# totokunda/apex-studio

Measured on AMD Instinct MI355X. Metric: denoise_steps_per_sec, higher is better.
Workload: dtype bf16; 1 GPU; flux-dev-1024x1024 denoise step (19 double + 38 single MM-DiT blocks, S_img 4096 + S_txt 512, B=1, no CFG) + FlowMatch-Euler step; clips_in_flight=1, parallelism=clip-per-gpu x1

## Files before the change

### apex-studio_amd/build.py

```python
from __future__ import annotations

import hashlib
import os
import shutil
import subprocess
import sys

PKG_DIR = os.path.dirname(os.path.abspath(__file__))
CSRC = os.path.join(PKG_DIR, "csrc")
LIB_NAME = "libapex_mi355.so"
LIB_PATH = os.path.join(PKG_DIR, LIB_NAME)
SOURCES = ["runtime.hip", "gemm.hip", "attention.hip", "attention_masked.hip", "attention_varlen.hip", "attention_dual.hip", "attention_wide.hip", "elementwise.hip", "dequant_gguf.hip",
           "conv.hip", "gemm_fp8.hip", "gemm_mxfp4.hip", "gemm_mxfp6.hip"]
ARCH = "gfx950"


def _hipcc() -> str:
    for cand in (os.environ.get("HIPCC"), shutil.which("hipcc"), "/opt/rocm/bin/hipcc"):
        if cand and os.path.exists(cand):
            return cand
    raise RuntimeError("hipcc not found (set HIPCC or install ROCm)")


FLAGS = ["-O3", "-std=c++17", "-fPIC", "-Wno-unused-result"]
if os.environ.get("APEXMI_DEBUG", "0") not in ("", "0"):
    FLAGS.append("-DAPEXMI_DEBUG")


NO_SPILL = {"attention.hip": ["attn_fwd_d128_w64_kernel", "attn_fwd_d128_w64r_kernel", "attn_fwd_d128_w64_band_kernel"],
            "attention_masked.hip": ["attn_masked_kernel", "attn_window_map_kernel"],
            "attention_varlen.hip": ["attn_varlen_kernel", "attn_varlen_vt_kernel"], "attention_dual.hip": ["attn_dual_kernel"], "attention_wide.hip": ["attn_wide_kernel"],
            "gemm_fp8.hip": ["gemm_fp8_kernel"], "gemm_mxfp4.hip": ["gemm_mxfp4_kernel"], "gemm_mxfp6.hip": ["gemm_mxfp6_kernel"],
            "elementwise.hip": ["ln_modulate_quant_kernel", "ln_modulate_wave_quant_kernel"]}
REMARKS = "-Rpass-analysis=kernel-resource-usage"


def parse_resource_remarks(text: str) -> dict:
    import re
    out, cur = {}, None
    for line in text.splitlines():
        m = re.search(r"remark:\s+Function Name: (\S+)", line)
        if m:
            cur = out.setdefault(m.group(1), {})
            continue
        m = re.search(r"remark:\s+([A-Za-z ]+?)(?: \[[^\]]*\])?: (\d+)", line)
        if m and cur is not None:
            cur[m.group(1).strip()] = int(m.group(2))
    return out


def check_no_spill(src: str, remarks: str, complete: bool = False) -> None:
    res = parse_resource_remarks(remarks)
    wanted = NO_SPILL.get(src, [])
    found = [want for want in wanted if any(want in k for k in res)]
    for want in wanted:
        hits = {k: v for k, v in res.items() if want in k}
        if not hits:
            if found and not complete:
                continue
            raise RuntimeError(f"build: no resource remark for kernel '{want}' of {src} — the spill check cannot run")
        for k, v in hits.items():
            bad = {f: v.get(f, -1) for f in ("ScratchSize", "SGPRs Spill", "VGPRs Spill") if v.get(f, -1) != 0}
            if bad:
                raise RuntimeError(f"build: {k} ({src}) has a hand-fixed register map and must not spill, but the compiler "
                                   f"reports {bad} (VGPRs {v.get('VGPRs')}, AGPRs {v.get('AGPRs')}, SGPRs {v.get('TotalSGPRs')}): "
                                   f"this hipcc allocates differently from the one the map was written against")


def _digest(paths: list[str], extra: str = "") -> str:
    h = hashlib.sha256(extra.encode())
    for p in paths:
        with open(p, "rb") as f:
            h.update(hashlib.sha256(f.read()).digest())
    return h.hexdigest()


def _stale(target: str, digest: str) -> bool:
    stamp = target + ".sha256"
    if not (os.path.exists(target) and os.path.exists(stamp)):
        return True
    with open(stamp) as f:
        return f.read().strip() != digest


def _stamp(target: str, digest: str) -> None:
    with open(target + ".sha256", "w") as f:
        f.write(digest + "\n")


def build(force: bool = False, verbose: bool = True) -> str:
    hipcc = _hipcc()
    headers = [os.path.join(CSRC, "common.h"),
               os.path.join(PKG_DIR, "..", "include", "apexmi.h")]
    headers += sorted(os.path.join(CSRC, f) for f in os.listdir(CSRC) if f.endswith((".inc", ".h")) and f != "common.h")
    objs = []
    jobs = []
    for src in SOURCES:
        sp = os.path.join(CSRC, src)
        op = os.path.join(CSRC, src.replace(".hip", ".o"))
        objs.append(op)
        dg = _digest([sp] + headers, " ".join(FLAGS + ([REMARKS + ":checked"] if src in NO_SPILL else []) + [ARCH]))
        if force or _stale(op, dg):
            cmd = [hipcc, f"--offload-arch={ARCH}", *FLAGS, *([REMARKS] if src in NO_SPILL else []), "-c", sp, "-o", op]
            if verbose:
                print("[build]", " ".join(cmd), flush=True)
            jobs.append((subprocess.Popen(cmd, stderr=subprocess.PIPE if src in NO_SPILL else None, text=True), cmd, op, dg, src))
    for proc, cmd, op, dg, src in jobs:
        err = proc.communicate()[1]
        if err:
            rest = [l for l in err.splitlines() if "kernel-resource-usage" not in l and not l.lstrip().startswith(("|", "^"))
                    and not l.strip()[:1].isdigit() and not l.startswith("In file included from")]
            if rest and verbose:
                print("\n".join(rest), file=sys.stderr, flush=True)
        if proc.returncode != 0:
            if err:
                print(err[-4000:], file=sys.stderr)
            raise subprocess.CalledProcessError(proc.returncode, cmd)
        if src in NO_SPILL:
            check_no_spill(src, err or "", complete=True)
        _stamp(op, dg)
    dg = _digest(objs, ARCH)
    if force or _stale(LIB_PATH, dg):
        cmd = [hipcc, f"--offload-arch={ARCH}", "-shared", "-fPIC", "-o", LIB_PATH] + objs
        if verbose:
            print("[build]", " ".join(cmd), flush=True)
        subprocess.check_call(cmd)
        _stamp(LIB_PATH, dg)
    return LIB_PATH


if __name__ == "__main__":
    build(force="--force" in sys.argv)
    print(LIB_PATH)
```

### apex-studio_amd/csrc/gemm.hip

```cpp
#include "common.h"

#include <cstring>
#include <type_traits>

namespace {

#ifndef APEXMI_GEMM_TRACE
#define APEXMI_GEMM_TRACE 0
#endif
#define PP_BAR()                               \
    do {                                       \
        __builtin_amdgcn_sched_barrier(0);     \
        __builtin_amdgcn_s_barrier();          \
        __builtin_amdgcn_sched_barrier(0);     \
    } while (0)
#define PP_SYNC()                                                                   \
    do {                                                                            \
        asm volatile("s_waitcnt lgkmcnt(0)" ::: "memory");                          \
        PP_BAR();                                                                   \
    } while (0)
#define VMCNT(n) asm volatile("s_waitcnt vmcnt(" #n ")" ::: "memory")
constexpr int BK = 64;
constexpr int GROUP_M = 6;
constexpr int EPI_GATE_RES_F32 = 7;
constexpr int MAX_GROUPS = 4;

struct GemmProblem {
    const bf16_t* A;
    const bf16_t* W;
    const bf16_t* bias;
    bf16_t* C;
    const float* gate;
    const bf16_t* R;
    int64_t lda, ldw, ldc, ldr;
    int M, N, nm, nn, tile0, gelu;
    int qkv, row0;
    const bf16_t* nq;
    const bf16_t* nk;
};
struct QkvShared {
    bf16_t* qo;
    bf16_t* ko;
    bf16_t* vt;
    const float* rope;
    int S_out, Skp, inner;
    float eps;
    const float* rope_pairs;
};
struct GemmGroup {
    GemmProblem p[MAX_GROUPS];
    int count, K, total, group_m;
    int batch;
    int64_t bsA, bsW, bsC_bytes;
    QkvShared qs;
    unsigned long long* clk;
#if APEXMI_GEMM_TRACE
    unsigned long long* trace;
#endif
    int wpacked;
};

template <int BM_, int BN_, int WM_, int WN_, int SCHED_>
struct Cfg {
    static constexpr int BM = BM_, BN = BN_, WM = WM_, WN = WN_;
    static constexpr int SCHED = SCHED_;
    static constexpr bool PP = SCHED_ == 1;
    static constexpr int NW = WM * WN, NT = NW * 64;
    static constexpr int TM = BM / WM / 32, TN = BN / WN / 32;
    static constexpr int A_BYTES = BM * BK * 2, W_BYTES = BN * BK * 2;
    static constexpr int STAGE = A_BYTES + W_BYTES;
    static constexpr int LDS = SCHED_ == 8 ? 5 * 32768 : 2 * STAGE;
    static constexpr int A_LD = BM * 8 / NT, W_LD = BN * 8 / NT;
    static constexpr int OCC = (LDS <= 80 * 1024 && NT == 256) ? 2 : (NT == 512 ? 2 : 1);
};
using CFG_128 = Cfg<128, 128, 2, 2, 0>;
using CFG_256 = Cfg<256, 256, 2, 4, 0>;
using CFG_128E = Cfg<128, 128, 2, 4, 0>;
using CFG_256P = Cfg<256, 256, 2, 4, 1>;
using CFG_256W = Cfg<256, 256, 2, 2, 4>;
using CFG_256P16 = Cfg<256, 256, 2, 4, 5>;
using CFG_256R = Cfg<256, 256, 2, 4, 7>;
using CFG_256R5 = Cfg<256, 256, 2, 4, 8>;

APEXMI_DEVICE float act_f(float x, int mode) {
    if (mode == 1) return gelu_tanh_f(x);
    if (mode == 2) return 0.5f * x * (1.0f + erff(x * 0.70710678118654752f));
    if (mode == 4) return x_sigmoid_log2(x, (1.702f * 1.4426950408889634f) * x);
    return silu_f(x);
}
template <int ACT>
APEXMI_DEVICE float act_c(float x) {
    if constexpr (ACT == 0) return x;
    else return act_f(x, ACT);
}
#define APEXMI_ACT_DISPATCH(mode, ...)                                    \
    switch (mode) {                                                       \
        case 1: { constexpr int ACT = 1; __VA_ARGS__; } break;            \
        case 2: { constexpr int ACT = 2; __VA_ARGS__; } break;            \
        case 3: { constexpr int ACT = 3; __VA_ARGS__; } break;            \
        case 4: { constexpr int ACT = 4; __VA_ARGS__; } break;            \
        default: { constexpr int ACT = 0; __VA_ARGS__; } break;           \
    }
inline int act_mode(int epilogue) {
    return epilogue == APEXMI_EPI_BIAS_GELU ? 1 : epilogue == APEXMI_EPI_BIAS_GELU_ERF ? 2 : epilogue == APEXMI_EPI_BIAS_SILU ? 3 : epilogue == APEXMI_EPI_BIAS_QUICK_GELU ? 4 : 0;
}

APEXMI_DEVICE void swap_pair(u32x2& a, u32x2& b) {
#pragma unroll
    for (int i = 0; i < 2; ++i) {
        auto r = __builtin_amdgcn_permlane32_swap(a[i], b[i], false, false);
        a[i] = r[0];
        b[i] = r[1];
    }
}

template <int EPI, int TM, int ACT = 0>
APEXMI_DEVICE void store_ntile(const f32x16 (&acc)[TM], const GemmProblem& P, int N, const int (&m)[TM],
                               int nbase, int hi) {
    float bs[4][4];
    f32x4 gt[4];
#pragma unroll
    for (int g = 0; g < 4; ++g) {
        const int n = min(nbase + 8 * g + 4 * hi, N - 4);
        u32x2 b = {0u, 0u};
        if (P.bias != nullptr) b = *(const u32x2*)(P.bias + n);
        bs[g][0] = bf16_lo(b[0]);
        bs[g][1] = bf16_hi(b[0]);
        bs[g][2] = bf16_lo(b[1]);
        bs[g][3] = bf16_hi(b[1]);
        if (EPI == APEXMI_EPI_BIAS_GATE_RES || EPI == EPI_GATE_RES_F32) gt[g] = *(const f32x4*)(P.gate + n);
    }
    if (EPI == APEXMI_EPI_BIAS_F32 || EPI == EPI_GATE_RES_F32) {
        float* Cf = (float*)P.C;
        const float* Rf = (const float*)P.R;
#pragma unroll
        for (int mt = 0; mt < TM; ++mt)
#pragma unroll
            for (int g = 0; g < 4; ++g) {
                const int n = nbase + 8 * g + 4 * hi;
                if (m[mt] >= 0 && n < N) {
                    float o[4];
#pragma unroll
                    for (int j = 0; j < 4; ++j) {
                        o[j] = acc[mt][4 * g + j] + bs[g][j];
                        o[j] = act_c<ACT>(o[j]);
                    }
                    if (EPI == EPI_GATE_RES_F32) {
                        const f32x4 r = *(const f32x4*)(Rf + (int64_t)m[mt] * P.ldr + n);
#pragma unroll
                        for (int j = 0; j < 4; ++j) o[j] = r[j] + gt[g][j] * o[j];
                    }
                    *(f32x4*)(Cf + (int64_t)m[mt] * P.ldc + n) = f32x4{o[0], o[1], o[2], o[3]};
                }
            }
        return;
    }
    u32x4 rr[TM][2];
    if (EPI == APEXMI_EPI_BIAS_GATE_RES) {
#pragma unroll
        for (int mt = 0; mt < TM; ++mt)
#pragma unroll
            for (int pr = 0; pr < 2; ++pr) {
                const int nst = min(nbase + 8 * (2 * pr + hi), N - 8);
                rr[mt][pr] = *(const u32x4*)(P.R + (int64_t)max(m[mt], 0) * P.ldr + nst);
            }
    }
#pragma unroll
    for (int mt = 0; mt < TM; ++mt)
#pragma unroll
        for (int pr = 0; pr < 2; ++pr) {
            const int g0 = 2 * pr;
            const int nst = nbase + 8 * (g0 + hi);
            float v[2][4];
#pragma unroll
            for (int q = 0; q < 2; ++q)
#pragma unroll
                for (int j = 0; j < 4; ++j) {
                    v[q][j] = acc[mt][4 * (g0 + q) + j] + bs[g0 + q][j];
                    v[q][j] = act_c<ACT>(v[q][j]);
                }
            if (EPI == APEXMI_EPI_BIAS_GATE_RES) {
                u32x2 ra = {rr[mt][pr][0], rr[mt][pr][1]}, rb = {rr[mt][pr][2], rr[mt][pr][3]};
                swap_pair(ra, rb);
#pragma unroll
                for (int q = 0; q < 2; ++q) {
                    const u32x2 r2 = q ? rb : ra;
                    v[q][0] = bf16_lo(r2[0]) + gt[g0 + q][0] * v[q][0];
                    v[q][1] = bf16_hi(r2[0]) + gt[g0 + q][1] * v[q][1];
                    v[q][2] = bf16_lo(r2[1]) + gt[g0 + q][2] * v[q][2];
                    v[q][3] = bf16_hi(r2[1]) + gt[g0 + q][3] * v[q][3];
                }
            }
            u32x2 oa = {pack_bf16(v[0][0], v[0][1]), pack_bf16(v[0][2], v[0][3])};
            u32x2 ob = {pack_bf16(v[1][0], v[1][1]), pack_bf16(v[1][2], v[1][3])};
            swap_pair(oa, ob);
            if (m[mt] >= 0 && nst < N) {
                const u32x4 o = {oa[0], oa[1], ob[0], ob[1]};
                *(u32x4*)(P.C + (int64_t)m[mt] * P.ldc + nst) = o;
            }
        }
}


typedef __attribute__((ext_vector_type(4))) float f32x4_t;

APEXMI_DEVICE float sum_xor16(float x) {
    auto r = __builtin_amdgcn_permlane16_swap(__float_as_uint(x), __float_as_uint(x), false, false);
    return __uint_as_float(r[0]) + __uint_as_float(r[1]);
}
APEXMI_DEVICE void swap16(uint32_t& a, uint32_t& b) {
    auto r = __builtin_amdgcn_permlane16_swap(a, b, false, false);
    a = r[0];
    b = r[1];
}

template <int EPI, int MT, int ACT = 0>
APEXMI_DEVICE void store_slab16(const f32x4_t (&x)[MT], const f32x4_t (&y)[MT], const GemmProblem& P, int N,
                                const int (&m)[MT], int nbase, int g, const u32x4* rr_pre = nullptr) {
    float bs[2][4];
    f32x4 gt[2];
#pragma unroll
    for (int t = 0; t < 2; ++t) {
        const int n = min(nbase + 16 * t + 4 * g, N - 4);
        u32x2 b = {0u, 0u};
        if (P.bias != nullptr) b = *(const u32x2*)(P.bias + n);
        bs[t][0] = bf16_lo(b[0]);
        bs[t][1] = bf16_hi(b[0]);
        bs[t][2] = bf16_lo(b[1]);
        bs[t][3] = bf16_hi(b[1]);
        if (EPI == APEXMI_EPI_BIAS_GATE_RES || EPI == EPI_GATE_RES_F32) gt[t] = *(const f32x4*)(P.gate + n);
    }
    if (EPI == APEXMI_EPI_BIAS_F32 || EPI == EPI_GATE_RES_F32) {
        float* Cf = (float*)P.C;
        const float* Rf = (const float*)P.R;
        constexpr int CH = MT < 4 ? MT : 4;
#pragma unroll
        for (int m0 = 0; m0 < MT; m0 += CH) {
            f32x4 rr[CH][2];
            if (EPI == EPI_GATE_RES_F32) {
#pragma unroll
                for (int c = 0; c < CH; ++c)
#pragma unroll
                    for (int t = 0; t < 2; ++t)
                        if (m0 + c < MT)
                            rr[c][t] = *(const f32x4*)(Rf + (int64_t)max(m[m0 + c < MT ? m0 + c : 0], 0) * P.ldr + min(nbase + 16 * t + 4 * g, N - 4));
            }
#pragma unroll
            for (int c = 0; c < CH; ++c)
#pragma unroll
                for (int t = 0; t < 2; ++t) {
                    if (m0 + c >= MT) continue;
                    const int mt = m0 + c < MT ? m0 + c : 0;
                    const int n = nbase + 16 * t + 4 * g;
                    const f32x4_t& a = t ? y[mt] : x[mt];
                    if (m[mt] >= 0 && n < N) {
                        float o[4];
#pragma unroll
                        for (int j = 0; j < 4; ++j) {
                            o[j] = a[j] + bs[t][j];
                            o[j] = act_c<ACT>(o[j]);
                        }
                        if (EPI == EPI_GATE_RES_F32) {
#pragma unroll
                            for (int j = 0; j < 4; ++j) o[j] = rr[c][t][j] + gt[t][j] * o[j];
                        }
                        *(f32x4*)(Cf + (int64_t)m[mt] * P.ldc + n) = f32x4{o[0], o[1], o[2], o[3]};
                    }
                }
        }
        return;
    }
    const int nst = nbase + 16 * (g & 1) + 8 * (g >> 1);
    u32x4 rr[MT];
    if (EPI == APEXMI_EPI_BIAS_GATE_RES) {
#pragma unroll
        for (int mt = 0; mt < MT; ++mt)
            rr[mt] = rr_pre ? rr_pre[mt] : *(const u32x4*)(P.R + (int64_t)max(m[mt], 0) * P.ldr + min(nst, N - 8));
    }
#pragma unroll
    for (int mt = 0; mt < MT; ++mt) {
        float v[2][4];
#pragma unroll
        for (int j = 0; j < 4; ++j) {
            v[0][j] = x[mt][j] + bs[0][j];
            v[1][j] = y[mt][j] + bs[1][j];
            v[0][j] = act_c<ACT>(v[0][j]);
            v[1][j] = act_c<ACT>(v[1][j]);
        }
        if (EPI == APEXMI_EPI_BIAS_GATE_RES) {
            uint32_t r0 = rr[mt][0], r1 = rr[mt][1], r2 = rr[mt][2], r3 = rr[mt][3];
            swap16(r0, r2);
            swap16(r1, r3);
            const uint32_t ra[2][2] = {{r0, r1}, {r2, r3}};
#pragma unroll
            for (int t = 0; t < 2; ++t) {
                v[t][0] = bf16_lo(ra[t][0]) + gt[t][0] * v[t][0];
                v[t][1] = bf16_hi(ra[t][0]) + gt[t][1] * v[t][1];
                v[t][2] = bf16_lo(ra[t][1]) + gt[t][2] * v[t][2];
                v[t][3] = bf16_hi(ra[t][1]) + gt[t][3] * v[t][3];
            }
        }
        uint32_t x0 = pack_bf16(v[0][0], v[0][1]), x1 = pack_bf16(v[0][2], v[0][3]);
        uint32_t y0 = pack_bf16(v[1][0], v[1][1]), y1 = pack_bf16(v[1][2], v[1][3]);
        swap16(x0, y0);
        swap16(x1, y1);
        if (m[mt] >= 0 && nst < N) {
            const u32x4 o = {x0, x1, y0, y1};
            *(u32x4*)(P.C + (int64_t)m[mt] * P.ldc + nst) = o;
        }
    }
}

#ifndef APEXMI_QK_ABL
#define APEXMI_QK_ABL 0
#endif
template <int MT = 8, int WROWS = 128>
APEXMI_DEVICE void qkv_epilogue16(f32x4_t (&acc16)[4][MT], const GemmProblem& P, const QkvShared& Q, int M, int m0, int n0,
                                  int wave, int wm, int wn, int lane, char* smem) {
    const int g = lane >> 4, c = lane & 15;
    const int which = n0 / Q.inner;
    const int ncol0 = n0 - which * Q.inner;
    float bs[2][4];
    auto load_bias = [&](int p) {
#pragma unroll
        for (int t = 0; t < 2; ++t) {
            u32x2 b = {0u, 0u};
            if (P.bias != nullptr) b = *(const u32x2*)(P.bias + n0 + wn * 64 + p * 32 + 16 * t + 4 * g);
            bs[t][0] = bf16_lo(b[0]);
            bs[t][1] = bf16_hi(b[0]);
            bs[t][2] = bf16_lo(b[1]);
            bs[t][3] = bf16_hi(b[1]);
        }
    };
    auto rounded = [&](int p, int mt) -> u32x4 {
        const f32x4_t& x = acc16[2 * p][mt];
        const f32x4_t& y = acc16[2 * p + 1][mt];
        uint32_t x0 = pack_bf16(x[0] + bs[0][0], x[1] + bs[0][1]), x1 = pack_bf16(x[2] + bs[0][2], x[3] + bs[0][3]);
        uint32_t y0 = pack_bf16(y[0] + bs[1][0], y[1] + bs[1][1]), y1 = pack_bf16(y[2] + bs[1][2], y[3] + bs[1][3]);
        swap16(x0, y0);
        swap16(x1, y1);
        return u32x4{x0, x1, y0, y1};
    };
    const int cw = 16 * (g & 1) + 8 * (g >> 1);
    __syncthreads();
    if (which == 2) {
        constexpr int NPASS = (2 * WROWS * 512 > 160 * 1024) ? 2 : 1;
        constexpr int ROWS = NPASS == 1 ? 2 * WROWS : WROWS;
        bf16_t* tile = (bf16_t*)smem;
        const int tid = wave * 64 + lane;
#pragma unroll
        for (int pass = 0; pass < NPASS; ++pass) {
            if (NPASS == 2 && pass == 1) __syncthreads();
            if (NPASS == 1 || wm == pass) {
#pragma unroll
                for (int p = 0; p < 2; ++p) {
                    load_bias(p);
#pragma unroll
                    for (int mt = 0; mt < MT; ++mt) {
                        const int r = (NPASS == 1 ? wm * WROWS : 0) + mt * 16 + c;
                        const int dch = (wn * 64 + p * 32 + cw) >> 3;
                        *(u32x4*)(tile + r * 256 + (((dch + (r >> 3) + 4 * (r & 7)) & 31) << 3)) = rounded(p, mt);
                    }
                }
            }
            __syncthreads();
            const int mp = m0 + (NPASS == 1 ? 0 : pass * WROWS);
            if (((P.row0 | M) & 7) != 0) {
                for (int i = 0; i < ROWS / 2; ++i) {
                    const int idx = i * 512 + tid;
                    const int r = idx % ROWS, d = idx / ROWS;
                    const bf16_t e = tile[r * 256 + ((((d >> 3) + (r >> 3) + 4 * (r & 7)) & 31) << 3) + (d & 7)];
                    const int h = (ncol0 + d) >> 7, dd = (ncol0 + d) & 127;
                    if (mp + r < M) Q.vt[((int64_t)h * 128 + dd) * Q.Skp + P.row0 + mp + r] = e;
                }
                continue;
            }
#pragma unroll 4
            for (int i = 0; i < ROWS / 16; ++i) {
                const int idx = i * 512 + tid;
                const int sc = idx & 7, d = (idx >> 3) & 255, sc_hi = idx >> 11;
                const int s8 = (sc_hi * 8 + sc) * 8;
                uint32_t w[4];
#pragma unroll
                for (int j = 0; j < 8; ++j) {
                    const int r = s8 + j;
                    const uint32_t e = tile[r * 256 + ((((d >> 3) + (r >> 3) + 4 * (r & 7)) & 31) << 3) + (d & 7)];
                    if (j & 1) w[j >> 1] |= e << 16;
                    else w[j >> 1] = e;
                }
                const int h = (ncol0 + d) >> 7, dd = (ncol0 + d) & 127;
                if (mp + s8 < M)
                    *(u32x4*)(Q.vt + ((int64_t)h * 128 + dd) * Q.Skp + P.row0 + mp + s8) = u32x4{w[0], w[1], w[2], w[3]};
            }
        }
        return;
    }
    float* red = (float*)smem;
#pragma unroll
    for (int p = 0; p < ((APEXMI_QK_ABL & 4) ? 0 : 2); ++p) {
        load_bias(p);
#pragma unroll
        for (int mt = 0; mt < MT; ++mt) {
            float x[8];
            unpack8(rounded(p, mt), x);
            float sq = 0.0f;
#pragma unroll
            for (int j = 0; j < 8; ++j) sq += x[j] * x[j];
            red[(wave * 2 * MT + p * MT + mt) * 64 + lane] = sq;
        }
    }
    __syncthreads();
    const bf16_t* nw = which ? P.nk : P.nq;
    const int h = (ncol0 >> 7) + (wn >> 1);
    bf16_t* dst_base = (which ? Q.ko : Q.qo) + (int64_t)h * Q.S_out * 128;
    auto rinv_of = [&](int mt) -> float {
        const float a0 = red[(wave * 2 * MT + mt) * 64 + lane] + red[((wave ^ 1) * 2 * MT + mt) * 64 + lane];
        const float a1 = red[(wave * 2 * MT + MT + mt) * 64 + lane] + red[((wave ^ 1) * 2 * MT + MT + mt) * 64 + lane];
        float sq = a0 + a1;
        sq = sum_xor16(sq);
        sq = sum_xor32(sq);
        return rsqrtf(sq * (1.0f / 128) + Q.eps);
    };
    float rinv[MT > 8 ? 1 : MT];
    if constexpr (MT <= 8) {
#pragma unroll
        for (int mt = 0; mt < MT; ++mt) rinv[mt] = rinv_of(mt);
    }
    if constexpr (!(APEXMI_QK_ABL & 64)) {
        if (Q.rope_pairs != nullptr) {
            constexpr int NIT = 2 * MT, NS = 5;
            constexpr int RED_BYTES = 8 * 2 * MT * 64 * 4;
            char* ring = smem + RED_BYTES + wave * (NS * 2048);
            const unsigned ring_lane = (unsigned)(uintptr_t)(__attribute__((address_space(3))) char*)ring + (unsigned)lane * 16u;
            auto issue = [&](int it) {
                const int p = it / MT, mt = it % MT;
                const int d = (wn & 1) * 64 + p * 32 + cw;
                int m = m0 + wm * WROWS + mt * 16 + c;
                asm volatile("" : "+v"(m));
                const int srow = P.row0 + min(m, M - 1);
                const float* cp = Q.rope_pairs + (int64_t)srow * 64 + (d >> 1);
                char* dst = ring + (it % NS) * 2048;
                glds16(cp, dst);
                glds16(cp + (int64_t)Q.S_out * 64, dst + 1024);
            };
#pragma unroll
            for (int it = 0; it < NS - 1; ++it) issue(it);
            float* wtab = (float*)(smem + RED_BYTES + 8 * NS * 2048) + wave * 1024 + lane * 8;
            float wv[MT > 8 ? 1 : 8];
            if constexpr (MT > 8) {
                if (nw != nullptr) {
#pragma unroll
                    for (int p = 0; p < 2; ++p) {
                        float w8[8];
                        unpack8(*(const u32x4*)(nw + (wn & 1) * 64 + p * 32 + cw), w8);
                        *(f32x4*)(wtab + p * 512) = f32x4{w8[0], w8[1], w8[2], w8[3]};
                        *(f32x4*)(wtab + p * 512 + 4) = f32x4{w8[4], w8[5], w8[6], w8[7]};
                    }
                }
            }
            auto body = [&](auto IT) {
                constexpr int it = decltype(IT)::value;
                if constexpr (it < NIT) {
                    constexpr int p = it / MT, mt = it % MT;
                    constexpr int later = (NIT - 1 - it) < (NS - 1) ? (NIT - 1 - it) : (NS - 1);
                    if constexpr (it + NS - 1 < NIT) issue(it + NS - 1);
                    const int d = (wn & 1) * 64 + p * 32 + cw;
                    if constexpr (mt == 0) {
                        load_bias(p);
                        if constexpr (MT <= 8) {
                            if (nw != nullptr) unpack8(*(const u32x4*)(nw + d), wv);
                        }
                    }
                    float x[8], y[8];
                    unpack8(rounded(p, mt), x);
                    if (nw != nullptr) {
                        if constexpr (MT > 8) {
                            const float ri = rinv_of(mt);
                            const f32x4 w0 = *(const f32x4*)(wtab + p * 512), w1 = *(const f32x4*)(wtab + p * 512 + 4);
#pragma unroll
                            for (int j = 0; j < 4; ++j) {
                                x[j] = x[j] * ri * w0[j];
                                x[j + 4] = x[j + 4] * ri * w1[j];
                            }
                        } else {
                            const float ri = rinv[MT > 8 ? 0 : mt];
#pragma unroll
                            for (int j = 0; j < 8; ++j) x[j] = x[j] * ri * wv[MT > 8 ? 0 : j];
                        }
                    }
                    f32x4 cq, sq4;
                    asm volatile("s_waitcnt vmcnt(%3)\n\t"
                                 "ds_read_b128 %0, %2 offset:%4\n\t"
                                 "ds_read_b128 %1, %2 offset:%5\n\t"
                                 "s_waitcnt lgkmcnt(0)"
                                 : "=&v"(cq), "=&v"(sq4)
                                 : "v"(ring_lane), "n"(2 * later), "n"((it % NS) * 2048), "n"((it % NS) * 2048 + 1024)
                                 : "memory");
#pragma unroll
                    for (int q = 0; q < 4; ++q) {
                        y[2 * q] = fmaf(x[2 * q], cq[q], -(x[2 * q + 1] * sq4[q]));
                        y[2 * q + 1] = fmaf(x[2 * q + 1], cq[q], x[2 * q] * sq4[q]);
                    }
                    int m = m0 + wm * WROWS + mt * 16 + c;
                    asm volatile("" : "+v"(m));
                    const int srow = P.row0 + min(m, M - 1);
                    if (m < M)
                        *(u32x4*)(dst_base + (int64_t)srow * 128 + d) =
                            u32x4{pack_bf16(y[0], y[1]), pack_bf16(y[2], y[3]), pack_bf16(y[4], y[5]), pack_bf16(y[6], y[7])};
                    __builtin_amdgcn_sched_barrier(0);
                }
            };
#define APEXMI_QK_IT(i) body(std::integral_constant<int, (i)>{});
            APEXMI_QK_IT(0) APEXMI_QK_IT(1) APEXMI_QK_IT(2) APEXMI_QK_IT(3) APEXMI_QK_IT(4) APEXMI_QK_IT(5)
            APEXMI_QK_IT(6) APEXMI_QK_IT(7) APEXMI_QK_IT(8) APEXMI_QK_IT(9) APEXMI_QK_IT(10) APEXMI_QK_IT(11)
            APEXMI_QK_IT(12) APEXMI_QK_IT(13) APEXMI_QK_IT(14) APEXMI_QK_IT(15) APEXMI_QK_IT(16) APEXMI_QK_IT(17)
            APEXMI_QK_IT(18) APEXMI_QK_IT(19) APEXMI_QK_IT(20) APEXMI_QK_IT(21) APEXMI_QK_IT(22) APEXMI_QK_IT(23)
#undef APEXMI_QK_IT
            static_assert(NIT <= 24, "the unrolled call list above covers 24 iterations");
            static_assert(MT > 8 ? RED_BYTES + 8 * NS * 2048 + 8 * 4096 <= 160 * 1024 : RED_BYTES + 8 * NS * 2048 <= 128 * 1024,
                          "sums + ring (+ weights) must fit the tile's LDS");
            return;
        }
    }
#pragma unroll
    for (int p = 0; p < ((APEXMI_QK_ABL & 32) ? 0 : 2); ++p) {
        const int d = (wn & 1) * 64 + p * 32 + cw;
        load_bias(p);
        float wv[8];
        if (nw != nullptr) unpack8(*(const u32x4*)(nw + d), wv);
#pragma unroll
        for (int mt = 0; mt < MT; ++mt) {
            const int m = m0 + wm * WROWS + mt * 16 + c;
            const int srow = P.row0 + min(m, M - 1);
            float x[8], y[8];
            unpack8(rounded(p, mt), x);
            if (nw != nullptr) {
                const float ri = (APEXMI_QK_ABL & 8) ? 1.0f : MT > 8 ? rinv_of(mt) : rinv[MT > 8 ? 0 : mt];
#pragma unroll
                for (int j = 0; j < 8; ++j) x[j] = x[j] * ri * wv[j];
            }
            const float* cp = Q.rope + (int64_t)srow * 128 + d;
            const float* sp = Q.rope + (int64_t)Q.S_out * 128 + (int64_t)srow * 128 + d;
            float cs[8], sn[8];
            if constexpr (APEXMI_QK_ABL & 1) {
#pragma unroll
                for (int j = 0; j < 8; ++j) cs[j] = 1.f, sn[j] = 0.5f;
            } else {
                const f32x4 c0 = *(const f32x4*)cp, c1 = *(const f32x4*)(cp + 4);
                const f32x4 s0 = *(const f32x4*)sp, s1 = *(const f32x4*)(sp + 4);
#pragma unroll
                for (int j = 0; j < 4; ++j) {
                    cs[j] = c0[j];
                    cs[j + 4] = c1[j];
                    sn[j] = s0[j];
                    sn[j + 4] = s1[j];
                }
            }
#pragma unroll
            for (int q = 0; q < 4; ++q) {
                y[2 * q] = fmaf(x[2 * q], cs[2 * q], -(x[2 * q + 1] * sn[2 * q]));
                y[2 * q + 1] = fmaf(x[2 * q + 1], cs[2 * q + 1], x[2 * q] * sn[2 * q + 1]);
            }
            if ((APEXMI_QK_ABL & 2) ? (y[0] + y[3] + y[5] == 12345.678f) : (m < M))
                *(u32x4*)(dst_base + (int64_t)srow * 128 + d) =
                    u32x4{pack_bf16(y[0], y[1]), pack_bf16(y[2], y[3]), pack_bf16(y[4], y[5]), pack_bf16(y[6], y[7])};
            if (!(APEXMI_QK_ABL & 16) && (MT > 8 || (mt & 1))) __builtin_amdgcn_sched_barrier(0);
        }
    }
}

#if APEXMI_GEMM_TRACE
#define APEXMI_TRACE_END()                                                                                   \
    do {                                                                                                     \
        if (G.trace != nullptr) {                                                                            \
            __builtin_amdgcn_sched_barrier(0);                                                               \
            const unsigned long long t_st = __builtin_amdgcn_s_memrealtime();                                \
            asm volatile("s_waitcnt vmcnt(0)" ::: "memory");                                                 \
            const unsigned long long t_ack = __builtin_amdgcn_s_memrealtime();                               \
            if (tid == 0) {                                                                                  \
                unsigned long long* o = G.trace + (size_t)blockIdx.x * 8;                                    \
                o[0] = __builtin_amdgcn_s_getreg((31 << 11) | (0 << 6) | 4);               \
                o[1] = __builtin_amdgcn_s_getreg((31 << 11) | (0 << 6) | 20);             \
                o[2] = tr_in;                                                                                \
                o[3] = tr_l0;                                                                                \
                o[4] = tr_l1;                                                                                \
                o[5] = t_st;                                                                                 \
                o[6] = t_ack;                                                                                \
                o[7] = (unsigned long long)s;                                                                \
            }                                                                                                \
        }                                                                                                    \
    } while (0)
#else
#define APEXMI_TRACE_END() do { } while (0)
#endif

struct TileCoord {
    int pm, pn;
};
__device__ __forceinline__ TileCoord tile_coord(int s, int nm, int nn, int group_m) {
    const int width = group_m * nn;
    const int first_m = (s / width) * group_m;
    const int gsz = min(nm - first_m, group_m);
    return TileCoord{first_m + (s % width) % gsz, (s % width) / gsz};
}

__device__ __forceinline__ const char* uniform_ptr(const char* p) {
    const uint64_t u = (uint64_t)p;
    const uint32_t hi = __builtin_amdgcn_readfirstlane((uint32_t)(u >> 32)), lo = __builtin_amdgcn_readfirstlane((uint32_t)u);
    return (const char*)(((uint64_t)hi << 32) | lo);
}
#pragma clang diagnostic push
#pragma clang diagnostic ignored "-Winline-asm"
__device__ __forceinline__ void glds16_s(const char* sbase, uint32_t voff, uint32_t la) {
    asm volatile("s_mov_b32 m0, %2\n\ts_nop 0\n\tglobal_load_lds_dwordx4 %0, %1"
                 :: "v"(voff), "s"(sbase), "s"(la) : "memory", "m0");
}
#pragma clang diagnostic pop

struct KRange {
    int kt0, kt1;
};
template <typename CFG, int EPI>
__device__ __forceinline__ void gemm_tile(const GemmGroup& G, char* smem, int s, const KRange& kr) {
    constexpr int BM = CFG::BM, BN = CFG::BN, TM = CFG::TM, TN = CFG::TN;

#if APEXMI_GEMM_TRACE
    unsigned long long tr_in = 0, tr_l0 = 0, tr_l1 = 0;
    if (G.trace != nullptr) tr_in = __builtin_amdgcn_s_memrealtime();
#endif
    int tid_ = threadIdx.x;
    asm volatile("" : "+v"(tid_));
    const int tid = tid_;
    const int lane = tid & 63;
    const int wave = __builtin_amdgcn_readfirstlane(tid >> 6);
    const int wm = wave / CFG::WN, wn = wave % CFG::WN;
    const int l31 = lane & 31, hi = lane >> 5;

    int gi = 0;
#pragma unroll
    for (int i = 1; i < MAX_GROUPS; ++i)
        if (i < G.count && s >= G.p[i].tile0) gi = i;
    GemmProblem P = G.p[gi];
    if (G.batch > 1) {
        const int64_t z = blockIdx.y;
        P.A += z * G.bsA;
        P.W += z * G.bsW;
        P.C = (bf16_t*)((char*)P.C + z * G.bsC_bytes);
    }
    s -= P.tile0;
    const int N = P.N, M = P.M;
    const TileCoord tc = tile_coord(s, P.nm, P.nn, G.group_m);
    const int pm = tc.pm, pn = tc.pn;
    const int m0 = pm * BM, n0 = pn * BN;

    const char* a_src[CFG::A_LD];
    const char* w_src[CFG::W_LD];
#pragma unroll
    for (int i = 0; i < CFG::A_LD; ++i) {
        const int p = (i * CFG::NW + wave) * 64 + lane;
        const int row = p >> 3, c = (p & 7) ^ ((row >> 1) & 7);
        a_src[i] = (const char*)(P.A + (int64_t)min(m0 + row, M - 1) * P.lda + c * 8);
    }
#pragma unroll
    for (int i = 0; i < CFG::W_LD; ++i) {
        const int p = (i * CFG::NW + wave) * 64 + lane;
        const int row = p >> 3, c = (p & 7) ^ ((row >> 1) & 7);
        w_src[i] = (const char*)(P.W + (int64_t)min(n0 + row, N - 1) * P.ldw + c * 8);
    }

    f32x16 acc[TN][TM];
#pragma unroll
    for (int i = 0; i < TN; ++i)
#pragma unroll
        for (int j = 0; j < TM; ++j)
#pragma unroll
            for (int r = 0; r < 16; ++r) acc[i][j][r] = 0.0f;

    f32x4_t acc16[4][8];
    if constexpr (CFG::SCHED == 5 || CFG::SCHED >= 7) {
#pragma unroll
        for (int i = 0; i < 4; ++i)
#pragma unroll
            for (int j = 0; j < 8; ++j) {
                acc16[i][j] = f32x4_t{0.f, 0.f, 0.f, 0.f};
                asm volatile("" : "+v"(acc16[i][j]));
            }
    }
    const int nkt_all = G.K / BK;
    const int nkt = (CFG::SCHED == 5) ? kr.kt1 - kr.kt0 : nkt_all;
    unsigned long long clk_c0 = 0, clk_r0 = 0;
    if (G.clk != nullptr) {
        clk_c0 = __builtin_readcyclecounter();
        clk_r0 = __builtin_amdgcn_s_memrealtime();
    }
#if APEXMI_GEMM_TRACE
    if (G.trace != nullptr) tr_l0 = __builtin_amdgcn_s_memrealtime();
#endif

    int a_off[TM], a_sw[TM], w_off[TN], w_sw[TN];
#pragma unroll
    for (int t = 0; t < TM; ++t) {
        const int r = wm * (BM / CFG::WM) + t * 32 + l31;
        a_off[t] = r * 128;
        a_sw[t] = (r >> 1) & 7;
    }
#pragma unroll
    for (int t = 0; t < TN; ++t) {
        const int r = wn * (BN / CFG::WN) + t * 32 + l31;
        w_off[t] = r * 128;
        w_sw[t] = (r >> 1) & 7;
    }

    if constexpr (CFG::SCHED == 0) {
        const char* const a_p = (const char*)(P.A + (int64_t)min(m0, M - 1) * P.lda);
        const char* const w_p = (const char*)(P.W + (int64_t)min(n0, N - 1) * P.ldw);
        const char* const a_u = uniform_ptr(a_p);
        const char* const w_u = uniform_ptr(w_p);
        uint32_t a_o[CFG::A_LD], w_o[CFG::W_LD];
#pragma unroll
        for (int i = 0; i < CFG::A_LD; ++i) a_o[i] = (uint32_t)(a_src[i] - a_u);
#pragma unroll
        for (int i = 0; i < CFG::W_LD; ++i) w_o[i] = (uint32_t)(w_src[i] - w_u);
        const uint32_t smem_lds0 = __builtin_amdgcn_readfirstlane((uint32_t)(uintptr_t)(__attribute__((address_space(3))) void*)smem);
        auto stage = [&](int buf, int kt) {
            const uint32_t base = smem_lds0 + buf * CFG::STAGE + wave * 1024;
            const char* ga = a_u + (int64_t)kt * (BK * 2);
            const char* gw = w_u + (int64_t)kt * (BK * 2);
#pragma unroll
            for (int i = 0; i < CFG::A_LD; ++i) glds16_s(ga, a_o[i], base + i * (CFG::NW * 1024));
#pragma unroll
            for (int i = 0; i < CFG::W_LD; ++i) glds16_s(gw, w_o[i], base + CFG::A_BYTES + i * (CFG::NW * 1024));
        };
        stage(0, 0);
        for (int kt = 0; kt < nkt; ++kt) {
            asm volatile("s_waitcnt vmcnt(0)" ::: "memory");
            __syncthreads();
            if (kt + 1 < nkt) stage((kt + 1) & 1, kt + 1);
            const char* As = smem + (kt & 1) * CFG::STAGE;
            const char* Ws = As + CFG::A_BYTES;
#pragma unroll
            for (int ks = 0; ks < 4; ++ks) {
                const int c = ks * 2 + hi;
                bf16x8 af[TM], wf[TN];
#pragma unroll
                for (int t = 0; t < TM; ++t) af[t] = *(const bf16x8*)(As + a_off[t] + ((c ^ a_sw[t]) << 4));
#pragma unroll
                for (int t = 0; t < TN; ++t) wf[t] = *(const bf16x8*)(Ws + w_off[t] + ((c ^ w_sw[t]) << 4));
#pragma unroll
                for (int nt = 0; nt < TN; ++nt)
#pragma unroll
                    for (int mt = 0; mt < TM; ++mt)
                        acc[nt][mt] = __builtin_amdgcn_mfma_f32_32x32x16_bf16(wf[nt], af[mt], acc[nt][mt], 0, 0, 0);
            }
        }
    } else if constexpr (CFG::SCHED == 4) {
        static_assert(CFG::SCHED != 4 || (TM == 4 && TN == 4 && CFG::NW == 4), "SCHED 4 is written for 2x2 waves of 128x128");
        bf16x8 fa[2][4], fw[2][4];
        const int rows_a = min(M - m0, BM), rows_w = min(N - n0, BN);
        auto rsrc_a = __builtin_amdgcn_make_buffer_rsrc((void*)(P.A + (int64_t)m0 * P.lda), 0,
                                                        (int)(((int64_t)(rows_a - 1) * P.lda + G.K) * 2), 0x00020000);
        auto rsrc_w = __builtin_amdgcn_make_buffer_rsrc((void*)(P.W + (int64_t)n0 * P.ldw), 0,
                                                        (int)(((int64_t)(rows_w - 1) * P.ldw + G.K) * 2), 0x00020000);
        const int sw_src = ((lane & 7) ^ (4 * (wave & 1) + (lane >> 4))) * 16;
        const int voff_a = (lane >> 3) * (int)P.lda * 2 + sw_src;
        const int voff_w = (lane >> 3) * (int)P.ldw * 2 + sw_src;
        const int sa = (int)P.lda * 2 * 8, sw = (int)P.ldw * 2 * 8;
        const int krot = (G.K * 2) % 8192 == 0 ? (int)(blockIdx.x & 7) * (nkt >> 3) : 0;
        auto dma1 = [&](int slot, int kt_, int i) {
            int kt = kt_ + krot;
            kt = kt >= nkt ? kt - nkt : kt;
            char* base = smem + slot * CFG::STAGE + wave * 1024;
            if (i < 8)
                __builtin_amdgcn_raw_ptr_buffer_load_lds(rsrc_a, (__attribute__((address_space(3))) void*)(base + i * 4096), 16, voff_a,
                                                         (i * 4 + wave) * sa + kt * (BK * 2), 0, 0);
            else
                __builtin_amdgcn_raw_ptr_buffer_load_lds(rsrc_w, (__attribute__((address_space(3))) void*)(base + CFG::A_BYTES + (i - 8) * 4096), 16,
                                                         voff_w, ((i - 8) * 4 + wave) * sw + kt * (BK * 2), 0, 0);
        };
        auto rd1 = [&](int slot, int ks, int b, int j) {
            const char* As = smem + slot * CFG::STAGE;
            const char* Ws = As + CFG::A_BYTES;
            const int c = ks * 2 + hi;
            if (j == 0) fw[b][0] = *(const bf16x8*)(Ws + w_off[0] + ((c ^ w_sw[0]) << 4));
            else if (j <= 4) fa[b][j - 1] = *(const bf16x8*)(As + a_off[j - 1] + ((c ^ a_sw[j - 1]) << 4));
            else fw[b][j - 4] = *(const bf16x8*)(Ws + w_off[j - 4] + ((c ^ w_sw[j - 4]) << 4));
        };
        auto mma1 = [&](int b, int i) {
            acc[i >> 2][i & 3] =
                __builtin_amdgcn_mfma_f32_32x32x16_bf16(fw[b][i >> 2], fa[b][i & 3], acc[i >> 2][i & 3], 0, 0, 0);
        };
#define W4_FENCE() __builtin_amdgcn_sched_barrier(0)
        constexpr int ROT = 0;
        constexpr int STEP = 2;
        auto period = [&](int kt, auto has_dma, auto has_next) {
            constexpr bool DMA = decltype(has_dma)::value, NEXT = decltype(has_next)::value;
            const int cur = kt & 1, nxt = cur ^ 1;
            asm volatile("s_waitcnt vmcnt(0) lgkmcnt(0)" ::: "memory");
            W4_FENCE();
            __builtin_amdgcn_s_barrier();
            W4_FENCE();
#pragma unroll
            for (int s = 0; s < (NEXT ? 64 : 16); ++s) {
                const int q = s >> 4, i = s & 15;
                mma1((q + 1) & 1, i);
                if (NEXT && i < 8) rd1(nxt, q, q & 1, i);
                if (DMA && s >= ROT && (s - ROT) % STEP == 0 && (s - ROT) / STEP < 16) dma1(cur, kt + 2, (s - ROT) / STEP);
                W4_FENCE();
            }
        };
#pragma unroll
        for (int i = 0; i < 16; ++i) dma1(0, 0, i);
        if (nkt > 1) {
#pragma unroll
            for (int i = 0; i < 16; ++i) dma1(1, 1, i);
            asm volatile("s_waitcnt vmcnt(16)" ::: "memory");
        } else {
            asm volatile("s_waitcnt vmcnt(0)" ::: "memory");
        }
        W4_FENCE();
        __builtin_amdgcn_s_barrier();
        W4_FENCE();
#pragma unroll
        for (int j = 0; j < 8; ++j) rd1(0, 0, 0, j);
        W4_FENCE();
#pragma unroll
        for (int s = 0; s < 48; ++s) {
            const int q = s >> 4, i = s & 15;
            mma1(q & 1, i);
            if (i < 8) rd1(0, q + 1, (q + 1) & 1, i);
            W4_FENCE();
        }
        int kt = 0;
        for (; kt + 2 < nkt; ++kt) period(kt, std::true_type{}, std::true_type{});
        if (kt + 1 < nkt) {
            period(kt, std::false_type{}, std::true_type{});
            ++kt;
        }
        period(kt, std::false_type{}, std::false_type{});
#undef W4_FENCE
    } else if constexpr (CFG::SCHED >= 7) {
        const int l15 = lane & 15, g4 = lane >> 4;
        const int swz = (g4 ^ (l15 >> 2)) << 4;
        const int rd_a = (wm * 128 + l15) * 64 + swz;
        const int rd_w = 16384 + (wn * 64 + l15) * 64 + swz;
        const char* base_a = (const char*)(P.A + (int64_t)m0 * P.lda);
        const char* base_w = (const char*)(P.W + (int64_t)n0 * P.ldw);
        unsigned off[4];
        int dst[4];
#pragma unroll
        for (int j = 0; j < 2; ++j) {
            const int pc = wave + 8 * j;
            const int row = pc * 16 + (lane >> 2);
            const int c = (lane & 3) ^ ((row >> 2) & 3);
            off[j] = (unsigned)((min(m0 + row, M - 1) - m0) * (int)P.lda * 2 + c * 16);
            off[2 + j] = (unsigned)((min(n0 + row, N - 1) - n0) * (int)P.ldw * 2 + c * 16);
            dst[j] = pc * 1024;
            dst[2 + j] = 16384 + pc * 1024;
        }
        constexpr int RD_ = CFG::SCHED == 8 ? 4 : 3;
        constexpr int NSLOT = RD_ + 1;
        auto dma = [&](int st, int slot) {
            char* base = smem + slot * 32768;
            const char* ka = base_a + (int64_t)st * 64;
            const char* kw = base_w + (int64_t)st * 64;
#pragma unroll
            for (int j = 0; j < 2; ++j) glds16(ka + off[j], base + dst[j]);
#pragma unroll
            for (int j = 2; j < 4; ++j) glds16(kw + off[j], base + dst[j]);
        };
        bf16x8 fa[2][8], fw[2][4];
#define RING_DSR(dstreg, addr, offs) asm volatile("ds_read_b128 %0, %1 offset:%2" : "=v"(dstreg) : "v"(addr), "i"(offs) : "memory")
#define RING_RD(slotidx, set)                              \
    do {                                                   \
        const int slot_ = (slotidx) * 32768;               \
        const int aw_ = slot_ + rd_w, aa_ = slot_ + rd_a;  \
        RING_DSR(fw[set][0], aw_, 0);                      \
        RING_DSR(fw[set][1], aw_, 1024);                   \
        RING_DSR(fw[set][2], aw_, 2048);                   \
        RING_DSR(fw[set][3], aw_, 3072);                   \
        RING_DSR(fa[set][0], aa_, 0);                      \
        RING_DSR(fa[set][1], aa_, 1024);                   \
        RING_DSR(fa[set][2], aa_, 2048);                   \
        RING_DSR(fa[set][3], aa_, 3072);                   \
        RING_DSR(fa[set][4], aa_, 4096);                   \
        RING_DSR(fa[set][5], aa_, 5120);                   \
        RING_DSR(fa[set][6], aa_, 6144);                   \
        RING_DSR(fa[set][7], aa_, 7168);                   \
    } while (0)
#define RING_WAIT(n, set)                                                                                                    \
    asm volatile("s_waitcnt lgkmcnt(" #n ")"                                                                                 \
                 : "+v"(fw[set][0]), "+v"(fw[set][1]), "+v"(fw[set][2]), "+v"(fw[set][3]), "+v"(fa[set][0]), "+v"(fa[set][1]), \
                   "+v"(fa[set][2]), "+v"(fa[set][3]), "+v"(fa[set][4]), "+v"(fa[set][5]), "+v"(fa[set][6]), "+v"(fa[set][7]) \
                 :                                                                                                           \
                 : "memory")
#define RING_MMA(set)                                                                                                      \
    do {                                                                                                                   \
        __builtin_amdgcn_s_setprio(1);                                                                                     \
        _Pragma("unroll") for (int u = 0; u < 4; ++u) _Pragma("unroll") for (int t = 0; t < 8; ++t) acc16[u][t] =          \
            __builtin_amdgcn_mfma_f32_16x16x32_bf16(fw[set][u], fa[set][t], acc16[u][t], 0, 0, 0);                         \
        __builtin_amdgcn_s_setprio(0);                                                                                     \
    } while (0)
#define RING_FENCE() __builtin_amdgcn_sched_barrier(0)
#define RING_VM(n) asm volatile("s_waitcnt vmcnt(" #n ")" ::: "memory")
#define RING_BAR() __builtin_amdgcn_s_barrier()
#define RING_STEP(st_, set, RD, DMA)                                        \
    do {                                                                    \
        RING_FENCE();                                                       \
        if (RD) RING_RD(s_rd, (set) ^ 1);                                   \
        RING_FENCE();                                                       \
        if (DMA) dma((st_) + RD_, s_dma);                                   \
        RING_FENCE();                                                       \
        if (DMA) {                                                          \
            if (RD_ == 3) RING_VM(4);                                       \
            else RING_VM(8);                                                \
        } else {                                                            \
            RING_VM(0);                                                     \
        }                                                                   \
        RING_FENCE();                                                       \
        RING_BAR();                                                         \
        RING_FENCE();                                                       \
        RING_MMA(set);                                                      \
        if (RD) RING_WAIT(0, (set) ^ 1);                                    \
        RING_FENCE();                                                       \
        RING_BAR();                                                         \
        RING_FENCE();                                                       \
        s_rd = s_rd + 1 == NSLOT ? 0 : s_rd + 1;                            \
        s_dma = s_dma + 1 == NSLOT ? 0 : s_dma + 1;                         \
    } while (0)
        const int ns = nkt * 2;
#pragma unroll
        for (int i = 0; i < RD_; ++i)
            if (i < ns) dma(i, i);
        if (ns >= 4 && RD_ == 4) RING_VM(8);
        else if (ns >= 3) RING_VM(4);
        else RING_VM(0);
        RING_FENCE();
        __builtin_amdgcn_s_barrier();
        RING_FENCE();
        RING_RD(0, 0);
        RING_WAIT(0, 0);
        RING_FENCE();
        if (wm == 1) RING_BAR();
        RING_FENCE();
        int s_rd = 1, s_dma = RD_ % NSLOT;
        int st = 0;
        for (; st + 1 + RD_ < ns; st += 2) {
            RING_STEP(st, 0, true, true);
            RING_STEP(st + 1, 1, true, true);
        }
        if (st + 4 <= ns) {
            if constexpr (RD_ == 3) RING_STEP(st, 0, true, true);
            else RING_STEP(st, 0, true, false);
            RING_STEP(st + 1, 1, true, false);
            st += 2;
        }
        RING_STEP(st, 0, true, false);
        RING_STEP(st + 1, 1, false, false);
        RING_FENCE();
        if (wm == 0) RING_BAR();
        RING_FENCE();
#undef RING_VM
#undef RING_BAR
#undef RING_STEP
#undef RING_MMA
#undef RING_RD
#undef RING_FENCE
#undef RING_DSR
#undef RING_WAIT
    } else if constexpr (CFG::SCHED == 5) {
        const int l15 = lane & 15, g4 = lane >> 4;
        const int sw16 = (l15 >> 1) & 7;
        int a16[8], w16[4];
#pragma unroll
        for (int t = 0; t < 8; ++t) a16[t] = (wm * 128 + t * 16 + l15) * 128;
#pragma unroll
        for (int t = 0; t < 4; ++t) w16[t] = (wn * 64 + t * 16 + l15) * 128;
        const int ch16[2] = {((0 + g4) ^ sw16) << 4, ((4 + g4) ^ sw16) << 4};
        bf16x8 af[4][2], wf[2][2][2];
        auto rd_a = [&](const char* As, int half) {
#pragma unroll
            for (int t = 0; t < 4; ++t)
#pragma unroll
                for (int ks = 0; ks < 2; ++ks) af[t][ks] = *(const bf16x8*)(As + a16[half * 4 + t] + ch16[ks]);
        };
        auto rd_w = [&](const char* Ws, int nt) {
#pragma unroll
            for (int u = 0; u < 2; ++u)
#pragma unroll
                for (int ks = 0; ks < 2; ++ks) wf[nt][u][ks] = *(const bf16x8*)(Ws + w16[nt * 2 + u] + ch16[ks]);
        };
        auto mma = [&](int half, int nt) {
            __builtin_amdgcn_s_setprio(1);
#pragma unroll
            for (int ks = 0; ks < 2; ++ks)
#pragma unroll
                for (int u = 0; u < 2; ++u)
#pragma unroll
                    for (int t = 0; t < 4; ++t)
                        acc16[nt * 2 + u][half * 4 + t] = __builtin_amdgcn_mfma_f32_16x16x32_bf16(
                            wf[nt][u][ks], af[t][ks], acc16[nt * 2 + u][half * 4 + t], 0, 0, 0);
            __builtin_amdgcn_s_setprio(0);
        };
        const char* ra_src[2][2];
        const char* rw_src[2][2];
        int ra_row[2][2], rw_row[2][2];
#pragma unroll
        for (int reg = 0; reg < 2; ++reg)
#pragma unroll
            for (int j = 0; j < 2; ++j) {
                const int q = j * 8 + wave;
                const int ra0 = (q < 8 ? q * 8 : 128 + (q - 8) * 8) + reg * 64;
                const int rw0 = (q >> 2) * 64 + reg * 32 + (q & 3) * 8;
                const int ra = ra0 + (lane >> 3), rw = rw0 + (lane >> 3);
                ra_src[reg][j] = (G.wpacked & 2)
                    ? (const char*)(P.A + ((int64_t)pm * nkt_all * 256 + ra) * 64 + (((lane & 7) ^ ((ra >> 1) & 7)) * 8))
                    : (const char*)(P.A + (int64_t)min(m0 + ra, M - 1) * P.lda + (((lane & 7) ^ ((ra >> 1) & 7)) * 8));
                rw_src[reg][j] = (G.wpacked & 1)
                    ? (const char*)(P.W + ((int64_t)pn * nkt_all * 256 + rw) * 64 + (((lane & 7) ^ ((rw >> 1) & 7)) * 8))
                    : (const char*)(P.W + (int64_t)min(n0 + rw, N - 1) * P.ldw + (((lane & 7) ^ ((rw >> 1) & 7)) * 8));
                ra_row[reg][j] = ra0;
                rw_row[reg][j] = rw0;
            }
        const int64_t w_kstep = (G.wpacked & 1) ? 256 * 128 : BK * 2;
        const int64_t a_kstep = (G.wpacked & 2) ? 256 * 128 : BK * 2;
        const char* const a_base_u = uniform_ptr((G.wpacked & 2) ? (const char*)(P.A + (int64_t)pm * nkt_all * 256 * 64)
                                                                 : (const char*)(P.A + (int64_t)min(m0, M - 1) * P.lda));
        const char* const w_base_u = uniform_ptr((G.wpacked & 1) ? (const char*)(P.W + (int64_t)pn * nkt_all * 256 * 64)
                                                                 : (const char*)(P.W + (int64_t)min(n0, N - 1) * P.ldw));
        uint32_t ra_off[2][2], rw_off[2][2];
#pragma unroll
        for (int reg = 0; reg < 2; ++reg)
#pragma unroll
            for (int j = 0; j < 2; ++j) {
                ra_off[reg][j] = (uint32_t)(ra_src[reg][j] - a_base_u);
                rw_off[reg][j] = (uint32_t)(rw_src[reg][j] - w_base_u);
            }
        const uint32_t smem_lds = __builtin_amdgcn_readfirstlane((uint32_t)(uintptr_t)(__attribute__((address_space(3))) void*)smem);
        auto stage_a = [&](int buf, int kt, int reg) {
            const uint32_t base = smem_lds + buf * CFG::STAGE;
            const char* gb = a_base_u + (int64_t)kt * a_kstep;
#pragma unroll
            for (int j = 0; j < 2; ++j) glds16_s(gb, ra_off[reg][j], base + ra_row[reg][j] * 128);
        };
        auto stage_w = [&](int buf, int kt, int reg) {
            const uint32_t base = smem_lds + buf * CFG::STAGE + CFG::A_BYTES;
            const char* gb = w_base_u + (int64_t)kt * w_kstep;
#pragma unroll
            for (int j = 0; j < 2; ++j) glds16_s(gb, rw_off[reg][j], base + rw_row[reg][j] * 128);
        };
        stage_a(0, 0, 0);
        stage_w(0, 0, 0);
        stage_w(0, 0, 1);
        stage_a(0, 0, 1);
        VMCNT(0);
        PP_BAR();
        if (wm == 1) PP_BAR();
        auto ktile = [&](int kt, auto more_c) {
            constexpr bool more = decltype(more_c)::value;
            const char* As = smem + (kt & 1) * CFG::STAGE;
            const char* Ws = As + CFG::A_BYTES;
            const int nb = (kt + 1) & 1;
            rd_a(As, 0);
            rd_w(Ws, 0);
            if constexpr (more) { stage_a(nb, kt + 1, 0); VMCNT(4); } else { VMCNT(2); }
            PP_SYNC();
            mma(0, 0);
            PP_BAR();
            rd_w(Ws, 1);
            if constexpr (more) { stage_w(nb, kt + 1, 0); VMCNT(4); } else { VMCNT(0); }
            PP_SYNC();
            mma(0, 1);
            PP_BAR();
            rd_a(As, 1);
            if constexpr (more) { stage_w(nb, kt + 1, 1); VMCNT(4); }
            PP_SYNC();
            mma(1, 1);
            PP_BAR();
            if constexpr (more) { stage_a(nb, kt + 1, 1); VMCNT(4); }
            PP_SYNC();
            mma(1, 0);
            PP_BAR();
        };
        for (int kt = 0; kt + 1 < nkt; ++kt) ktile(kt, std::true_type{});
        if (nkt > 0) ktile(nkt - 1, std::false_type{});
        if (wm == 0) PP_BAR();
    } else {
        static_assert(!CFG::PP || (TM == 4 && TN == 2), "ping-pong schedule is written for 128x64 wave tiles");
        bf16x8 af[2][4], wf[4];
        auto rd_a = [&](const char* As, int half) {
#pragma unroll
            for (int t = 0; t < 2; ++t)
#pragma unroll
                for (int ks = 0; ks < 4; ++ks)
                    af[t][ks] = *(const bf16x8*)(As + a_off[half * 2 + t] + (((ks * 2 + hi) ^ a_sw[half * 2 + t]) << 4));
        };
        auto rd_w = [&](const char* Ws, int nt) {
#pragma unroll
            for (int ks = 0; ks < 4; ++ks)
                wf[ks] = *(const bf16x8*)(Ws + w_off[nt] + (((ks * 2 + hi) ^ w_sw[nt]) << 4));
        };
        auto mma = [&](int half, int nt) {
            __builtin_amdgcn_s_setprio(1);
#pragma unroll
            for (int ks = 0; ks < 4; ++ks)
#pragma unroll
                for (int t = 0; t < 2; ++t)
                    acc[nt][half * 2 + t] =
                        __builtin_amdgcn_mfma_f32_32x32x16_bf16(wf[ks], af[t][ks], acc[nt][half * 2 + t], 0, 0, 0);
            __builtin_amdgcn_s_setprio(0);
        };

        const char* ra_src[2][2];
        const char* rw_src[2][2];
        int ra_lds[2][2], rw_lds[2][2];
#pragma unroll
        for (int reg = 0; reg < 2; ++reg)
#pragma unroll
            for (int j = 0; j < 2; ++j) {
                const int q = j * 8 + wave;
                const int ra0 = (q < 8 ? q * 8 : 128 + (q - 8) * 8) + reg * 64;
                const int rw0 = (q >> 2) * 64 + reg * 32 + (q & 3) * 8;
                const int ra = ra0 + (lane >> 3), rw = rw0 + (lane >> 3);
                ra_src[reg][j] = (const char*)(P.A + (int64_t)min(m0 + ra, M - 1) * P.lda + (((lane & 7) ^ ((ra >> 1) & 7)) * 8));
                rw_src[reg][j] = (const char*)(P.W + (int64_t)min(n0 + rw, N - 1) * P.ldw + (((lane & 7) ^ ((rw >> 1) & 7)) * 8));
                ra_lds[reg][j] = ra0 * 128;
                rw_lds[reg][j] = CFG::A_BYTES + rw0 * 128;
            }
        auto stage_a = [&](int buf, int kt, int reg) {
            char* base = smem + buf * CFG::STAGE;
            const int64_t koff = (int64_t)kt * (BK * 2);
#pragma unroll
            for (int j = 0; j < 2; ++j) glds16(ra_src[reg][j] + koff, base + ra_lds[reg][j]);
        };
        auto stage_w = [&](int buf, int kt, int reg) {
            char* base = smem + buf * CFG::STAGE;
            const int64_t koff = (int64_t)kt * (BK * 2);
#pragma unroll
            for (int j = 0; j < 2; ++j) glds16(rw_src[reg][j] + koff, base + rw_lds[reg][j]);
        };

        stage_a(0, 0, 0);
        stage_w(0, 0, 0);
        stage_w(0, 0, 1);
        stage_a(0, 0, 1);
        VMCNT(0);
        PP_BAR();
        if (wm == 1) PP_BAR();
        for (int kt = 0; kt < nkt; ++kt) {
            const char* As = smem + (kt & 1) * CFG::STAGE;
            const char* Ws = As + CFG::A_BYTES;
            const bool more = kt + 1 < nkt;
            const int nb = (kt + 1) & 1;
            rd_a(As, 0);
            rd_w(Ws, 0);
            if (more) stage_a(nb, kt + 1, 0);
            if (more) { VMCNT(4); } else { VMCNT(2); }
            PP_SYNC();
            mma(0, 0);
            PP_BAR();
            rd_w(Ws, 1);
            if (more) stage_w(nb, kt + 1, 0);
            if (more) { VMCNT(4); } else { VMCNT(0); }
            PP_SYNC();
            mma(0, 1);
            PP_BAR();
            rd_a(As, 1);
            if (more) stage_w(nb, kt + 1, 1);
            if (more) VMCNT(4);
            PP_SYNC();
            mma(1, 1);
            PP_BAR();
            rd_w(Ws, 0);
            if (more) stage_a(nb, kt + 1, 1);
            if (more) VMCNT(4);
            PP_SYNC();
            mma(1, 0);
            PP_BAR();
        }
        if (wm == 0) PP_BAR();
    }

#if APEXMI_GEMM_TRACE
    if (G.trace != nullptr) {
        __builtin_amdgcn_sched_barrier(0);
        tr_l1 = __builtin_amdgcn_s_memrealtime();
        __builtin_amdgcn_sched_barrier(0);
    }
#endif
    if (G.clk != nullptr) {
        const unsigned long long c1 = __builtin_readcyclecounter(), r1 = __builtin_amdgcn_s_memrealtime();
        if (tid == 0) {
            atomicAdd(G.clk, c1 - clk_c0);
            atomicAdd(G.clk + 1, r1 - clk_r0);
        }
    }

    if constexpr (CFG::SCHED == 5 || CFG::SCHED >= 7) {
        if constexpr (EPI == APEXMI_EPI_BIAS) {
            if (P.qkv) {
                qkv_epilogue16(acc16, P, G.qs, M, m0, n0, wave, wm, wn, lane, smem);
                APEXMI_TRACE_END();
                return;
            }
        }
        int mrow16[8];
#pragma unroll
        for (int mt = 0; mt < 8; ++mt) {
            mrow16[mt] = m0 + wm * 128 + mt * 16 + (lane & 15);
            if (mrow16[mt] >= M) mrow16[mt] = -1;
        }
        if constexpr (EPI == APEXMI_EPI_BIAS_GATE_RES) {
            u32x4 rr2[2][8];
            const int g = lane >> 4;
#pragma unroll
            for (int p = 0; p < 2; ++p) {
                const int nst = n0 + wn * 64 + p * 32 + 16 * (g & 1) + 8 * (g >> 1);
#pragma unroll
                for (int mt = 0; mt < 8; ++mt)
                    rr2[p][mt] = *(const u32x4*)(P.R + (int64_t)max(mrow16[mt], 0) * P.ldr + min(nst, N - 8));
            }
#pragma unroll
            for (int p = 0; p < 2; ++p)
                store_slab16<EPI, 8, 0>(acc16[2 * p], acc16[2 * p + 1], P, N, mrow16, n0 + wn * 64 + p * 32, g, rr2[p]);
        } else {
            APEXMI_ACT_DISPATCH((EPI == APEXMI_EPI_BIAS || EPI == APEXMI_EPI_BIAS_F32) ? P.gelu : 0,
                                _Pragma("unroll") for (int p = 0; p < 2; ++p)
                                    store_slab16<EPI, 8, ACT>(acc16[2 * p], acc16[2 * p + 1], P, N, mrow16, n0 + wn * 64 + p * 32, lane >> 4));
        }
        APEXMI_TRACE_END();
        return;
    }
    int mrow[TM];
#pragma unroll
    for (int mt = 0; mt < TM; ++mt) {
        mrow[mt] = m0 + wm * (BM / CFG::WM) + mt * 32 + l31;
        if (mrow[mt] >= M) mrow[mt] = -1;
    }
    APEXMI_ACT_DISPATCH((EPI == APEXMI_EPI_BIAS || EPI == APEXMI_EPI_BIAS_F32) ? P.gelu : 0,
                        _Pragma("unroll") for (int nt = 0; nt < TN; ++nt)
                            store_ntile<EPI, TM, ACT>(acc[nt], P, N, mrow, n0 + wn * (BN / CFG::WN) + nt * 32, hi));
}

template <typename CFG, int EPI>
__global__ __launch_bounds__(CFG::NT, CFG::OCC) void gemm_bf16_kernel(const GemmGroup G) {
    extern __shared__ __attribute__((aligned(16))) char smem[];
    const int nkt = G.K / BK;
    const KRange kr{0, nkt};
    gemm_tile<CFG, EPI>(G, smem, xcd_remap(blockIdx.x, G.total), kr);
}

__global__ __launch_bounds__(256) void split_bf16x3_kernel(const float* __restrict__ x, int64_t ldx, int64_t M, int K,
                                                            bf16_t* __restrict__ out, int64_t ldo) {
    const int kc = K >> 3;
    const int64_t idx = (int64_t)blockIdx.x * 256 + threadIdx.x;
    if (idx >= M * kc) return;
    const int64_t m = idx / kc;
    const int c = (int)(idx % kc) * 8;
    float v[8], h[8], md[8], lo[8];
    load8<float>(x + m * ldx + c, v);
#pragma unroll
    for (int j = 0; j < 8; ++j) {
        h[j] = bf16_to_f32(f32_to_bf16(v[j]));
        const float r1 = v[j] - h[j];
        md[j] = bf16_to_f32(f32_to_bf16(r1));
        lo[j] = r1 - md[j];
    }
    bf16_t* o = out + m * ldo + c;
    store8<bf16_t>(o, h);
    store8<bf16_t>(o + K, md);
    store8<bf16_t>(o + 2 * (int64_t)K, lo);
}

constexpr int XBM = 288, XBN = 192;
constexpr int X_A_BYTES = XBM * BK * 2, X_W_BYTES = XBN * BK * 2, X_STAGE = X_A_BYTES + X_W_BYTES, X_LDS = 2 * X_STAGE;

template <int EPI, int MT, int ACT = 0>
APEXMI_DEVICE void store_single16(const f32x4_t (&x)[MT], const GemmProblem& P, int N, const int (&m)[MT], int nb, int g,
                                  const u32x2* rr_pre) {
    const int nl = min(nb + 4 * g, N - 4);
    float bs[4] = {0.f, 0.f, 0.f, 0.f};
    if (P.bias != nullptr) {
        const u32x2 b = *(const u32x2*)(P.bias + nl);
        bs[0] = bf16_lo(b[0]);
        bs[1] = bf16_hi(b[0]);
        bs[2] = bf16_lo(b[1]);
        bs[3] = bf16_hi(b[1]);
    }
    f32x4 gt = {0.f, 0.f, 0.f, 0.f};
    if (EPI == APEXMI_EPI_BIAS_GATE_RES) gt = *(const f32x4*)(P.gate + nl);
#pragma unroll
    for (int mt = 0; mt < MT; ++mt) {
        float v[4];
#pragma unroll
        for (int j = 0; j < 4; ++j) v[j] = act_c<ACT>(x[mt][j] + bs[j]);
        if (EPI == APEXMI_EPI_BIAS_GATE_RES) {
            const u32x2 r = rr_pre[mt];
            v[0] = bf16_lo(r[0]) + gt[0] * v[0];
            v[1] = bf16_hi(r[0]) + gt[1] * v[1];
            v[2] = bf16_lo(r[1]) + gt[2] * v[2];
            v[3] = bf16_hi(r[1]) + gt[3] * v[3];
        }
        if (m[mt] >= 0 && nb + 4 * g < N)
            *(u32x2*)(P.C + (int64_t)m[mt] * P.ldc + nb + 4 * g) = u32x2{pack_bf16(v[0], v[1]), pack_bf16(v[2], v[3])};
    }
}

template <int EPI>
__global__ __launch_bounds__(512, 2) void gemm_bf16_x288_kernel(const GemmGroup G) {
    extern __shared__ __attribute__((aligned(16))) char smem[];
    const int tid = threadIdx.x;
    const int lane = tid & 63;
    const int wave = __builtin_amdgcn_readfirstlane(tid >> 6);
    const int wm = wave >> 2, wn = wave & 3;

    int s = xcd_remap(blockIdx.x, G.total);
    int gi = 0;
#pragma unroll
    for (int i = 1; i < MAX_GROUPS; ++i)
        if (i < G.count && s >= G.p[i].tile0) gi = i;
    const GemmProblem P = G.p[gi];
    s -= P.tile0;
    const int N = P.N, M = P.M;
    const TileCoord tc = tile_coord(s, P.nm, P.nn, G.group_m);
    const int m0 = tc.pm * XBM, n0 = tc.pn * XBN;

    const char* src[8];
    int dst[8];
#pragma unroll
    for (int j = 0; j < 8; ++j) {
        int row0;
        bool isw = false;
        if (j < 3) {
            isw = true;
            row0 = (j * 8 + wave) * 8;
        } else if (j < 5) {
            const int q = (j - 3) * 8 + wave;
            row0 = q < 6 ? q * 8 : q < 12 ? 144 + (q - 6) * 8 : (q - 12) * 8;
        } else {
            const int q = (j - 5) * 8 + wave;
            row0 = q < 6 ? 48 + q * 8 : q < 12 ? 192 + (q - 6) * 8 : q < 18 ? 96 + (q - 12) * 8 : 240 + (q - 18) * 8;
        }
        const int row = row0 + (lane >> 3);
        const int c = (lane & 7) ^ ((row >> 1) & 7);
        src[j] = isw ? (const char*)(P.W + (int64_t)min(n0 + row, N - 1) * P.ldw + c * 8)
                     : (const char*)(P.A + (int64_t)min(m0 + row, M - 1) * P.lda + c * 8);
        dst[j] = (isw ? X_A_BYTES : 0) + row0 * 128;
    }
    auto stage = [&](int buf, int kt, int j) { glds16(src[j] + (int64_t)kt * (BK * 2), smem + buf * X_STAGE + dst[j]); };

    f32x4_t acc[3][9];
#pragma unroll
    for (int i = 0; i < 3; ++i)
#pragma unroll
        for (int j = 0; j < 9; ++j) acc[i][j] = f32x4_t{0.f, 0.f, 0.f, 0.f};

    const int nkt = G.K / BK;
    unsigned long long clk_c0 = 0, clk_r0 = 0;
    if (G.clk != nullptr) {
        clk_c0 = __builtin_readcyclecounter();
        clk_r0 = __builtin_amdgcn_s_memrealtime();
    }

    const int l15 = lane & 15, g4 = lane >> 4;
    const int sw16 = (l15 >> 1) & 7;
    const int a_base = (wm * 144 + l15) * 128, w_base = X_A_BYTES + (wn * 48 + l15) * 128;
    const int ch16[2] = {((0 + g4) ^ sw16) << 4, ((4 + g4) ^ sw16) << 4};
    bf16x8 af[3][2], wf[3][2];
    auto rd_a = [&](const char* St, int grp) {
#pragma unroll
        for (int t = 0; t < 3; ++t)
#pragma unroll
            for (int ks = 0; ks < 2; ++ks) af[t][ks] = *(const bf16x8*)(St + a_base + (grp * 3 + t) * 2048 + ch16[ks]);
    };
    auto rd_w = [&](const char* St) {
#pragma unroll
        for (int t = 0; t < 3; ++t)
#pragma unroll
            for (int ks = 0; ks < 2; ++ks) wf[t][ks] = *(const bf16x8*)(St + w_base + t * 2048 + ch16[ks]);
    };
    auto mma = [&](int grp) {
        __builtin_amdgcn_s_setprio(1);
#pragma unroll
        for (int ks = 0; ks < 2; ++ks)
#pragma unroll
            for (int nt = 0; nt < 3; ++nt)
#pragma unroll
                for (int t = 0; t < 3; ++t)
                    acc[nt][grp * 3 + t] =
                        __builtin_amdgcn_mfma_f32_16x16x32_bf16(wf[nt][ks], af[t][ks], acc[nt][grp * 3 + t], 0, 0, 0);
        __builtin_amdgcn_s_setprio(0);
    };
#pragma unroll
    for (int j = 0; j < 8; ++j) stage(0, 0, j);
    VMCNT(0);
    PP_BAR();
    if (wm == 1) PP_BAR();
    for (int kt = 0; kt < nkt; ++kt) {
        const char* St = smem + (kt & 1) * X_STAGE;
        const bool more = kt + 1 < nkt;
        const int nb = (kt + 1) & 1;
        rd_w(St);
        rd_a(St, 0);
        if (more) {
            stage(nb, kt + 1, 0);
            stage(nb, kt + 1, 1);
            stage(nb, kt + 1, 2);
            VMCNT(4);
        } else {
            VMCNT(1);
        }
        PP_SYNC();
        mma(0);
        PP_BAR();
        rd_a(St, 1);
        if (more) {
            stage(nb, kt + 1, 3);
            stage(nb, kt + 1, 4);
            stage(nb, kt + 1, 5);
            VMCNT(6);
        } else {
            VMCNT(0);
        }
        PP_SYNC();
        mma(1);
        PP_BAR();
        rd_a(St, 2);
        if (more) {
            stage(nb, kt + 1, 6);
            stage(nb, kt + 1, 7);
            VMCNT(3);
        }
        PP_SYNC();
        mma(2);
        PP_BAR();
    }
    if (wm == 0) PP_BAR();

    if (G.clk != nullptr) {
        const unsigned long long c1 = __builtin_readcyclecounter(), r1 = __builtin_amdgcn_s_memrealtime();
        if (tid == 0) {
            atomicAdd(G.clk, c1 - clk_c0);
            atomicAdd(G.clk + 1, r1 - clk_r0);
        }
    }

    int mrow[9];
#pragma unroll
    for (int mt = 0; mt < 9; ++mt) {
        mrow[mt] = m0 + wm * 144 + mt * 16 + l15;
        if (mrow[mt] >= M) mrow[mt] = -1;
    }
    const int nbase = n0 + wn * 48;
    if constexpr (EPI == APEXMI_EPI_BIAS_GATE_RES) {
        u32x4 rr[9];
        u32x2 r1[9];
        const int nst = nbase + 16 * (g4 & 1) + 8 * (g4 >> 1);
#pragma unroll
        for (int mt = 0; mt < 9; ++mt) {
            const bf16_t* row = P.R + (int64_t)max(mrow[mt], 0) * P.ldr;
            rr[mt] = *(const u32x4*)(row + min(nst, N - 8));
            r1[mt] = *(const u32x2*)(row + min(nbase + 32 + 4 * g4, N - 4));
        }
        store_slab16<EPI, 9, 0>(acc[0], acc[1], P, N, mrow, nbase, g4, rr);
        store_single16<EPI, 9, 0>(acc[2], P, N, mrow, nbase + 32, g4, r1);
    } else {
        APEXMI_ACT_DISPATCH(P.gelu, store_slab16<EPI, 9, ACT>(acc[0], acc[1], P, N, mrow, nbase, g4);
                            store_single16<EPI, 9, ACT>(acc[2], P, N, mrow, nbase + 32, g4, nullptr));
    }
}

constexpr int YBM = 384, YBN = 256;
constexpr int Y_A_BYTES = YBM * BK * 2, Y_W_BYTES = YBN * BK * 2, Y_STAGE = Y_A_BYTES + Y_W_BYTES, Y_LDS = 2 * Y_STAGE;

template <int EPI, int DIST = 1, int QKV = 0>
__global__ __launch_bounds__(512, 2) void gemm_bf16_x384_kernel(const GemmGroup G) {
    extern __shared__ __attribute__((aligned(16))) char smem[];
    const int tid = threadIdx.x;
    const int lane = tid & 63;
    const int wave = __builtin_amdgcn_readfirstlane(tid >> 6);
    const int wm = wave >> 2, wn = wave & 3;

    int s = xcd_remap(blockIdx.x, G.total);
    int gi = 0;
#pragma unroll
    for (int i = 1; i < MAX_GROUPS; ++i)
        if (i < G.count && s >= G.p[i].tile0) gi = i;
    const GemmProblem P = G.p[gi];
    s -= P.tile0;
    const int N = P.N, M = P.M;
    const TileCoord tc = tile_coord(s, P.nm, P.nn, G.group_m);
    const int m0 = tc.pm * YBM, n0 = tc.pn * YBN;

    const int rows_a = min(M - m0, YBM), rows_w = min(N - n0, YBN);
    auto rsrc_a = __builtin_amdgcn_make_buffer_rsrc((void*)(P.A + (int64_t)m0 * P.lda), 0,
                                                    (int)(((int64_t)(rows_a - 1) * P.lda + G.K) * 2), 0x00020000);
    auto rsrc_w = __builtin_amdgcn_make_buffer_rsrc((void*)(P.W + (int64_t)n0 * P.ldw), 0,
                                                    (int)(((int64_t)(rows_w - 1) * P.ldw + G.K) * 2), 0x00020000);
    const int par = wave & 1, widx = wave >> 1;
    const int sw_src = ((lane & 7) ^ (4 * par + (lane >> 4))) * 16;
    const int voff_a = (lane >> 3) * (int)P.lda * 2 + sw_src;
    const int voff_w = (lane >> 3) * (int)P.ldw * 2 + sw_src;
    const int lda8 = (int)P.lda * 16, ldw8 = (int)P.ldw * 16;
    auto piece_of = [&](int j) -> int {
        if (j < 4) return 2 * (4 * j + widx) + par;
        const int e = 3 * widx + (j < 7 ? j - 4 : j - 7);
        return (e < 6 ? 0 : 24) + (j < 7 ? 0 : 12) + 2 * (e % 6) + par;
    };
    auto stage = [&](int buf, int kt, int j) {
        const int pc = piece_of(j);
        char* dst = smem + buf * Y_STAGE + (j < 4 ? Y_A_BYTES : 0) + pc * 1024;
        if (j < 4)
            __builtin_amdgcn_raw_ptr_buffer_load_lds(rsrc_w, (__attribute__((address_space(3))) void*)dst, 16, voff_w, pc * ldw8 + kt * (BK * 2), 0, 0);
        else
            __builtin_amdgcn_raw_ptr_buffer_load_lds(rsrc_a, (__attribute__((address_space(3))) void*)dst, 16, voff_a, pc * lda8 + kt * (BK * 2), 0, 0);
    };

    f32x4_t acc[4][12];
#pragma unroll
    for (int i = 0; i < 4; ++i)
#pragma unroll
        for (int j = 0; j < 12; ++j) acc[i][j] = f32x4_t{0.f, 0.f, 0.f, 0.f};

    const int nkt = G.K / BK;
    unsigned long long clk_c0 = 0, clk_r0 = 0;
    if (G.clk != nullptr) {
        clk_c0 = __builtin_readcyclecounter();
        clk_r0 = __builtin_amdgcn_s_memrealtime();
    }
#if APEXMI_GEMM_TRACE
    const unsigned long long y_t_in = G.trace != nullptr ? __builtin_amdgcn_s_memrealtime() : 0;
    unsigned long long y_t_loop = 0;
#define Y_TRACE_END(kind)                                                                                   \
    do {                                                                                                    \
        if (G.trace != nullptr) {                                                                           \
            asm volatile("s_waitcnt vmcnt(0)" ::: "memory");                                                \
            __syncthreads();                                                                                \
            if (tid == 0) {                                                                                 \
                unsigned long long* o = G.trace + (size_t)blockIdx.x * 4;                                   \
                o[0] = (unsigned long long)(kind);                                                          \
                o[1] = y_t_in;                                                                              \
                o[2] = y_t_loop;                                                                            \
                o[3] = __builtin_amdgcn_s_memrealtime();                                                    \
            }                                                                                               \
        }                                                                                                   \
    } while (0)
#else
#define Y_TRACE_END(kind) do { } while (0)
#endif

    const int l15 = lane & 15, g4 = lane >> 4;
    const int sw16 = (l15 >> 1) & 7;
    const int a_base = (wm * 192 + l15) * 128, w_base = Y_A_BYTES + (wn * 64 + l15) * 128;
    const int ch16[2] = {((0 + g4) ^ sw16) << 4, ((4 + g4) ^ sw16) << 4};
    bf16x8 af[6], wf[4];
    auto rd_a = [&](const char* St, int h, int ks) {
#pragma unroll
        for (int t = 0; t < 6; ++t) af[t] = *(const bf16x8*)(St + a_base + (h * 6 + t) * 2048 + ch16[ks]);
    };
    auto rd_w = [&](const char* St, int ks) {
#pragma unroll
        for (int t = 0; t < 4; ++t) wf[t] = *(const bf16x8*)(St + w_base + t * 2048 + ch16[ks]);
    };
    auto mma = [&](int h) {
        __builtin_amdgcn_s_setprio(1);
#pragma unroll
        for (int nt = 0; nt < 4; ++nt)
#pragma unroll
            for (int t = 0; t < 6; ++t)
                acc[nt][h * 6 + t] = __builtin_amdgcn_mfma_f32_16x16x32_bf16(wf[nt], af[t], acc[nt][h * 6 + t], 0, 0, 0);
        __builtin_amdgcn_s_setprio(0);
    };
#pragma unroll
    for (int j = 0; j < 10; ++j) stage(0, 0, j);
    VMCNT(0);
    PP_BAR();
    if (wm == 1) PP_BAR();
    auto ktile = [&](int kt, auto more_c) {
        constexpr bool more = decltype(more_c)::value;
        const char* St = smem + (kt & 1) * Y_STAGE;
        const int nb = (kt + 1) & 1;
        rd_w(St, 0);
        rd_a(St, 0, 0);
        if constexpr (more) {
            stage(nb, kt + 1, 0);
            stage(nb, kt + 1, 1);
            if (DIST == 0) {
                stage(nb, kt + 1, 2);
                VMCNT(3);
            } else {
                VMCNT(2);
            }
        } else {
            VMCNT(0);
        }
        PP_SYNC();
        mma(0);
        PP_BAR();
        rd_a(St, 1, 0);
        if constexpr (more) {
            if (DIST != 0) stage(nb, kt + 1, 2);
            stage(nb, kt + 1, 3);
            stage(nb, kt + 1, 4);
            if (DIST == 0) stage(nb, kt + 1, 5);
        }
        PP_SYNC();
        mma(1);
        PP_BAR();
        rd_w(St, 1);
        rd_a(St, 0, 1);
        if constexpr (more) {
            if (DIST != 0) stage(nb, kt + 1, 5);
            stage(nb, kt + 1, 6);
            if (DIST == 0) stage(nb, kt + 1, 7);
        }
        PP_SYNC();
        mma(0);
        PP_BAR();
        rd_a(St, 1, 1);
        if constexpr (more) {
            if (DIST != 0) stage(nb, kt + 1, 7);
            stage(nb, kt + 1, 8);
            stage(nb, kt + 1, 9);
            VMCNT(3);
        }
        PP_SYNC();
        mma(1);
        PP_BAR();
    };
    for (int kt = 0; kt + 1 < nkt; ++kt) ktile(kt, std::true_type{});
    if (nkt > 0) ktile(nkt - 1, std::false_type{});
    if (wm == 0) PP_BAR();

    if (G.clk != nullptr) {
        const unsigned long long c1 = __builtin_readcyclecounter(), r1 = __builtin_amdgcn_s_memrealtime();
        if (tid == 0) {
            atomicAdd(G.clk, c1 - clk_c0);
            atomicAdd(G.clk + 1, r1 - clk_r0);
        }
    }

#if APEXMI_GEMM_TRACE
    if (G.trace != nullptr) y_t_loop = __builtin_amdgcn_s_memrealtime();
#endif
    if constexpr (EPI == APEXMI_EPI_BIAS && QKV == 1) {
        if (P.qkv) {
            qkv_epilogue16<12, 192>(acc, P, G.qs, M, m0, n0, wave, wm, wn, lane, smem);
            Y_TRACE_END(n0 / G.qs.inner);
            return;
        }
    }
    constexpr int MTC = EPI == APEXMI_EPI_BIAS_GATE_RES ? 3 : EPI == EPI_GATE_RES_F32 ? 2 : 6;
#pragma unroll
    for (int h = 0; h < 12 / MTC; ++h) {
        int mrow[MTC];
#pragma unroll
        for (int mt = 0; mt < MTC; ++mt) {
            mrow[mt] = m0 + wm * 192 + (h * MTC + mt) * 16 + l15;
            if (mrow[mt] >= M) mrow[mt] = -1;
        }
#pragma unroll
        for (int p = 0; p < 2; ++p) {
            const int nbase = n0 + wn * 64 + p * 32;
            const f32x4_t(&x)[MTC] = *(const f32x4_t(*)[MTC]) & acc[2 * p][h * MTC];
            const f32x4_t(&y)[MTC] = *(const f32x4_t(*)[MTC]) & acc[2 * p + 1][h * MTC];
            if constexpr (EPI == APEXMI_EPI_BIAS_GATE_RES) {
                u32x4 rr[MTC];
                const int nst = nbase + 16 * (g4 & 1) + 8 * (g4 >> 1);
#pragma unroll
                for (int mt = 0; mt < MTC; ++mt) rr[mt] = *(const u32x4*)(P.R + (int64_t)max(mrow[mt], 0) * P.ldr + min(nst, N - 8));
                store_slab16<EPI, MTC, 0>(x, y, P, N, mrow, nbase, g4, rr);
            } else {
                APEXMI_ACT_DISPATCH(P.gelu, store_slab16<EPI, MTC, ACT>(x, y, P, N, mrow, nbase, g4));
            }
        }
    }
    Y_TRACE_END(3);
}
#undef Y_TRACE_END

int g_group_m = GROUP_M;
#if APEXMI_GEMM_TRACE
uintptr_t g_gemm_trace = 0;
#endif
int g_large_cfg = 7;
int g_force_cfg = 0;
int g_wpacked = 0;
int g_tail_max = 96;
int g_x288 = 0;
int g_x384_group_m = 3;
int g_x384_dist = -1;
int g_x384_qkv = 1;
int g_x384 = 1;
int g_small_max = 112;
int g_tail_split = 2;

int number_tiles(GemmGroup& G, const int* Ms, int BM, int BN) {
    int t = 0;
    for (int i = 0; i < G.count; ++i) {
        G.p[i].M = Ms[i];
        G.p[i].nm = (Ms[i] + BM - 1) / BM;
        G.p[i].nn = (G.p[i].N + BN - 1) / BN;
        G.p[i].tile0 = t;
        t += G.p[i].nm * G.p[i].nn;
    }
    G.total = t;
    G.clk = apexmi_clk_ptr();
#if APEXMI_GEMM_TRACE
    G.trace = (unsigned long long*)g_gemm_trace;
#endif
    G.wpacked = 0;
    return t;
}

template <typename CFG, int EPI>
int launch_cfg(GemmGroup& G, const int* Ms, hipStream_t stream) {
    if constexpr (CFG::SCHED == 0 || CFG::SCHED == 5) {
        for (int i = 0; i < G.count; ++i)
            if (G.p[i].lda > (1 << 22) || G.p[i].ldw > (1 << 22)) {
                apexmi_set_error("gemm_bf16: leading dimensions above 2^22 elements are not supported (lda %lld, ldw %lld)",
                                 (long long)G.p[i].lda, (long long)G.p[i].ldw);
                return 1;
            }
    }
    static uint64_t attr_set = 0;
    APEXMI_SET_ATTR_ONCE(attr_set,
        (void)hipFuncSetAttribute((const void*)gemm_bf16_kernel<CFG, EPI>,
                                  hipFuncAttributeMaxDynamicSharedMemorySize, CFG::LDS));
    const int t = number_tiles(G, Ms, CFG::BM, CFG::BN);
    G.group_m = g_group_m;
    if (CFG::SCHED == 5) G.wpacked = g_wpacked;
    hipLaunchKernelGGL((gemm_bf16_kernel<CFG, EPI>), dim3(t, G.batch), dim3(CFG::NT), CFG::LDS, stream, G);
    return apexmi_check_launch("gemm_bf16");
}

template <int EPI>
int launch_x288(GemmGroup& G, const int* Ms, hipStream_t stream) {
    static uint64_t attr_set = 0;
    APEXMI_SET_ATTR_ONCE(attr_set,
        (void)hipFuncSetAttribute((const void*)gemm_bf16_x288_kernel<EPI>, hipFuncAttributeMaxDynamicSharedMemorySize, X_LDS));
    const int t = number_tiles(G, Ms, XBM, XBN);
    G.group_m = g_group_m;
    hipLaunchKernelGGL((gemm_bf16_x288_kernel<EPI>), dim3(t, 1), dim3(512), X_LDS, stream, G);
    return apexmi_check_launch("gemm_bf16 (288x192)");
}

template <int EPI>
int launch_x384(GemmGroup& G, const int* Ms, hipStream_t stream) {
    static uint64_t attr_set = 0;
    APEXMI_SET_ATTR_ONCE(attr_set,
        (void)hipFuncSetAttribute((const void*)gemm_bf16_x384_kernel<EPI, 0>, hipFuncAttributeMaxDynamicSharedMemorySize, Y_LDS);
        (void)hipFuncSetAttribute((const void*)gemm_bf16_x384_kernel<EPI, 1>, hipFuncAttributeMaxDynamicSharedMemorySize, Y_LDS);
        if constexpr (EPI == APEXMI_EPI_BIAS)
            (void)hipFuncSetAttribute((const void*)gemm_bf16_x384_kernel<EPI, 1, 1>, hipFuncAttributeMaxDynamicSharedMemorySize, Y_LDS));
    const int t = number_tiles(G, Ms, YBM, YBN);
    G.group_m = g_x384_group_m;
    bool any_qkv = false;
    for (int i = 0; i < G.count; ++i) any_qkv |= G.p[i].qkv != 0;
    if constexpr (EPI == APEXMI_EPI_BIAS) {
        if (any_qkv) {
            hipLaunchKernelGGL((gemm_bf16_x384_kernel<EPI, 1, 1>), dim3(t, 1), dim3(512), Y_LDS, stream, G);
            return apexmi_check_launch("gemm_bf16 (384x256, fused q/k/v)");
        }
    }
    const int dist = g_x384_dist >= 0 ? g_x384_dist : (t >= 2048 ? 0 : 1);
    if (dist == 0) hipLaunchKernelGGL((gemm_bf16_x384_kernel<EPI, 0>), dim3(t, 1), dim3(512), Y_LDS, stream, G);
    else hipLaunchKernelGGL((gemm_bf16_x384_kernel<EPI, 1>), dim3(t, 1), dim3(512), Y_LDS, stream, G);
    return apexmi_check_launch("gemm_bf16 (384x256)");
}

inline bool x288_pays(const GemmGroup& G, const int* Ms) {
    int64_t t256 = 0, t288 = 0;
    for (int i = 0; i < G.count; ++i) {
        if (G.p[i].qkv) return false;
        t256 += (int64_t)((Ms[i] + 255) / 256) * ((G.p[i].N + 255) / 256);
        t288 += (int64_t)((Ms[i] + XBM - 1) / XBM) * ((G.p[i].N + XBN - 1) / XBN);
    }
    const double c256 = (double)((t256 + 255) / 256) * 65536.0;
    const double c288 = (double)((t288 + 255) / 256) * (XBM * XBN) * 1.04;
    return c288 < 0.95 * c256;
}

inline bool use_x288(const GemmGroup& G, const int* Ms) {
    if (g_x288 == 0 || G.batch != 1 || G.K % BK != 0 || !(g_force_cfg == 0 || g_force_cfg == 7) || g_large_cfg != 7) return false;
    int64_t mtot = 0;
    int nmax = 0;
    for (int i = 0; i < G.count; ++i) {
        if (G.p[i].qkv) return false;
        mtot += Ms[i];
        nmax = G.p[i].N > nmax ? G.p[i].N : nmax;
    }
    if (g_x288 == 2) return true;
    return G.K >= 256 && mtot >= 1024 && nmax >= 1024 && x288_pays(G, Ms);
}

inline bool x384_pays(const GemmGroup& G, const int* Ms) {
    int64_t t = 0;
    for (int i = 0; i < G.count; ++i) {
        const int64_t nm = (Ms[i] + YBM - 1) / YBM;
        if ((nm * YBM - Ms[i]) * 200 > 3 * (int64_t)Ms[i]) return false;
        t += nm * ((G.p[i].N + YBN - 1) / YBN);
    }
    const int64_t rem = t % 256;
    return t >= 3 * 256 && (rem == 0 || rem >= 154 || t >= 8 * 256);
}
inline bool use_x384(const GemmGroup& G, const int* Ms) {
    if (g_x384 == 0 || G.batch != 1 || G.K % BK != 0 || !(g_force_cfg == 0 || g_force_cfg == 7) || g_large_cfg != 7) return false;
    for (int i = 0; i < G.count; ++i)
        if (G.p[i].qkv || G.p[i].lda > (1 << 21) || G.p[i].ldw > (1 << 21)) return false;
    return g_x384 == 2 || x384_pays(G, Ms);
}

template <int EPI>
int launch_epi(GemmGroup& G, const int* Ms, hipStream_t stream) {
    int cfg = g_force_cfg;
    if constexpr (EPI == APEXMI_EPI_BIAS || EPI == APEXMI_EPI_BIAS_GATE_RES) {
        if (use_x288(G, Ms)) return launch_x288<EPI>(G, Ms, stream);
        if (use_x384(G, Ms)) return launch_x384<EPI>(G, Ms, stream);
    }
    if constexpr (EPI == APEXMI_EPI_BIAS_F32 || EPI == EPI_GATE_RES_F32) {
        if (G.batch == 1 && !use_x288(G, Ms) && use_x384(G, Ms)) return launch_x384<EPI>(G, Ms, stream);
    }
    if (cfg == 0) {
        int64_t mtot = 0;
        int nmax = 0;
        for (int i = 0; i < G.count; ++i) {
            mtot += Ms[i];
            nmax = G.p[i].N > nmax ? G.p[i].N : nmax;
        }
        cfg = (mtot >= 1024 && nmax >= 1024 && G.K >= 256) ? g_large_cfg : 1;
        if ((EPI == APEXMI_EPI_BIAS_GATE_RES || EPI == EPI_GATE_RES_F32) && cfg == 7 && G.batch == 1 && g_small_max > 0) {
            int64_t t256 = 0;
            bool any_qkv = false;
            for (int i = 0; i < G.count; ++i) {
                t256 += (int64_t)((Ms[i] + 255) / 256) * ((G.p[i].N + 255) / 256);
                any_qkv |= G.p[i].qkv != 0;
            }
            if (!any_qkv && t256 <= g_small_max) cfg = 1;
        }
        if (cfg == 6 && G.K % 12288 == 0) cfg = 7;
        if ((cfg == 7 || cfg == 9 || cfg == 10) && g_tail_split && G.count >= 2 && G.batch == 1) {
            int64_t lead = 0;
            for (int i = 0; i + 1 < G.count; ++i)
                lead += (int64_t)((Ms[i] + 255) / 256) * ((G.p[i].N + 255) / 256);
            const int li = G.count - 1;
            const int64_t last = (int64_t)((Ms[li] + 255) / 256) * ((G.p[li].N + 255) / 256);
            if (lead >= 256 && lead % 256 == 0 && last <= g_tail_max) {
                GemmGroup T = G;
                T.count = 1;
                T.p[0] = G.p[li];
                G.count = li;
                if (int rc = (cfg == 9    ? launch_cfg<CFG_256R, EPI>(G, Ms, stream)
                              : cfg == 10 ? launch_cfg<CFG_256R5, EPI>(G, Ms, stream)
                                          : launch_cfg<CFG_256P16, EPI>(G, Ms, stream)))
                    return rc;
                if (g_tail_split == 2) return launch_cfg<CFG_128E, EPI>(T, Ms + li, stream);
                return launch_cfg<CFG_128, EPI>(T, Ms + li, stream);
            }
        }
    }
    switch (cfg) {
        case 1: return launch_cfg<CFG_128, EPI>(G, Ms, stream);
        case 2: return launch_cfg<CFG_256, EPI>(G, Ms, stream);
        case 8: return launch_cfg<CFG_128E, EPI>(G, Ms, stream);
        case 6: return launch_cfg<CFG_256W, EPI>(G, Ms, stream);
        case 7: return launch_cfg<CFG_256P16, EPI>(G, Ms, stream);
        case 9: return launch_cfg<CFG_256R, EPI>(G, Ms, stream);
        case 10: return launch_cfg<CFG_256R5, EPI>(G, Ms, stream);
        default:
            return launch_cfg<CFG_256P, EPI>(G, Ms, stream);
    }
}

int launch_group(GemmGroup& G, const int* Ms, int kind, hipStream_t stream) {
    switch (kind) {
        case APEXMI_EPI_BIAS_GATE_RES: return launch_epi<APEXMI_EPI_BIAS_GATE_RES>(G, Ms, stream);
        case APEXMI_EPI_BIAS_F32: return launch_epi<APEXMI_EPI_BIAS_F32>(G, Ms, stream);
        case EPI_GATE_RES_F32: return launch_epi<EPI_GATE_RES_F32>(G, Ms, stream);
        default: return launch_epi<APEXMI_EPI_BIAS>(G, Ms, stream);
    }
}

int epi_base(int epilogue) { return epilogue & ~APEXMI_EPI_F32_IO; }
bool epi_f32(int epilogue) { return (epilogue & APEXMI_EPI_F32_IO) != 0 || epi_base(epilogue) == APEXMI_EPI_BIAS_F32; }
int epi_kind(int epilogue) {
    const int b = epi_base(epilogue);
    if (epilogue & APEXMI_EPI_F32_IO) return b == APEXMI_EPI_BIAS_GATE_RES ? EPI_GATE_RES_F32 : APEXMI_EPI_BIAS_F32;
    return act_mode(b) ? APEXMI_EPI_BIAS : b;
}

int check_problem(const void* A, int64_t lda, const void* W, int64_t ldw, void* C, int64_t ldc, int M,
                  int N, int K, int epilogue, const float* gate, const void* R, int64_t ldr) {
    APEXMI_REQUIRE(A && W && C, "gemm_bf16: null operand");
    APEXMI_REQUIRE(M > 0 && N > 0 && K > 0, "gemm_bf16: empty problem M=%d N=%d K=%d", M, N, K);
    APEXMI_REQUIRE(K % BK == 0, "gemm_bf16: K=%d must be a multiple of %d", K, BK);
    APEXMI_REQUIRE(N % 8 == 0, "gemm_bf16: N=%d must be a multiple of 8", N);
    APEXMI_REQUIRE(lda % 8 == 0 && ldw % 8 == 0 && ldc % 4 == 0,
                   "gemm_bf16: leading dimensions must keep rows 16-byte aligned");
    APEXMI_REQUIRE(((uintptr_t)A % 16) == 0 && ((uintptr_t)W % 16) == 0 && ((uintptr_t)C % 8) == 0,
                   "gemm_bf16: operands must be 16-byte aligned");
    APEXMI_REQUIRE(epi_base(epilogue) >= 0 && epi_base(epilogue) <= 6 && (epilogue & ~(APEXMI_EPI_F32_IO | 7)) == 0,
                   "gemm_bf16: unknown epilogue %d", epilogue);
    APEXMI_REQUIRE(!epi_f32(epilogue) || ((uintptr_t)C % 16) == 0, "gemm_bf16: f32 output must be 16-byte aligned");
    if (epi_base(epilogue) == APEXMI_EPI_BIAS_GATE_RES) {
        APEXMI_REQUIRE(gate && R, "gemm_bf16: gate/residual epilogue needs gate and R");
        APEXMI_REQUIRE(ldr % 4 == 0 && ((uintptr_t)gate % 16) == 0 && ((uintptr_t)R % (epi_f32(epilogue) ? 16 : 8)) == 0,
                       "gemm_bf16: gate/R alignment");
    }
    return 0;
}

}

extern "C" int apexmi_gemm_bf16(const void* A, int64_t lda, const void* W, int64_t ldw,
                                const void* bias, void* C, int64_t ldc, int M, int N, int K,
                                int epilogue, const float* gate, const void* R, int64_t ldr,
                                apexmi_stream_t stream_) {
    hipStream_t stream = (hipStream_t)stream_;
    if (int rc = check_problem(A, lda, W, ldw, C, ldc, M, N, K, epilogue, gate, R, ldr)) return rc;
    GemmGroup G;
    G.count = 1;
    G.K = K;
    G.batch = 1;
    G.bsA = G.bsW = G.bsC_bytes = 0;
    G.p[0] = GemmProblem{(const bf16_t*)A, (const bf16_t*)W, (const bf16_t*)bias, (bf16_t*)C, gate,
                         (const bf16_t*)R, lda, ldw, ldc, ldr, M, N, 0, 0, 0,
                         act_mode(epi_base(epilogue))};
    ApexmiProfScope prof(0, stream, 2.0 * M * N * (double)K,
                         2.0 * ((double)M * K + (double)N * K + (double)M * N));
    return launch_group(G, &M, epi_kind(epilogue), stream);
}

extern "C" int apexmi_gemm_bf16_batched(const void* A, int64_t lda, int64_t stride_a, const void* W, int64_t ldw,
                                        int64_t stride_w, void* C, int64_t ldc, int64_t stride_c, int batch, int M,
                                        int N, int K, int epilogue, apexmi_stream_t stream_) {
    hipStream_t stream = (hipStream_t)stream_;
    if (int rc = check_problem(A, lda, W, ldw, C, ldc, M, N, K, epilogue, nullptr, nullptr, 0)) return rc;
    APEXMI_REQUIRE(epilogue == APEXMI_EPI_BIAS || epilogue == APEXMI_EPI_BIAS_F32,
                   "gemm_bf16_batched: epilogue %d unsupported (plain bf16 or f32 output only)", epilogue);
    APEXMI_REQUIRE(batch >= 1 && batch <= 65535, "gemm_bf16_batched: batch=%d not in [1, 65535]", batch);
    const int esz = epilogue == APEXMI_EPI_BIAS_F32 ? 4 : 2;
    APEXMI_REQUIRE(stride_a % 8 == 0 && stride_w % 8 == 0 && (stride_c * esz) % 16 == 0,
                   "gemm_bf16_batched: batch strides must keep every element 16-byte aligned");
    APEXMI_REQUIRE(epilogue != APEXMI_EPI_BIAS_F32 || ((uintptr_t)C % 16) == 0, "gemm_bf16_batched: f32 output must be 16-byte aligned");
    GemmGroup G;
    G.count = 1;
    G.K = K;
    G.batch = batch;
    G.bsA = stride_a;
    G.bsW = stride_w;
    G.bsC_bytes = stride_c * esz;
    G.p[0] = GemmProblem{(const bf16_t*)A, (const bf16_t*)W, nullptr, (bf16_t*)C, nullptr, nullptr, lda, ldw, ldc, 0,
                         M, N, 0, 0, 0, 0};
    ApexmiProfScope prof(0, stream, 2.0 * batch * M * N * (double)K,
                         2.0 * batch * ((double)M * K + (double)N * K + (double)M * N));
    return launch_group(G, &M, epi_kind(epilogue), stream);
}

extern "C" int apexmi_gemm_bf16_grouped(int count, const void* const* A, const int64_t* lda,
                                        const void* const* W, const int64_t* ldw,
                                        const void* const* bias, void* const* C, const int64_t* ldc,
                                        const int* M, const int* N, int K, const int* epilogue,
                                        const float* const* gate, const void* const* R,
                                        const int64_t* ldr, apexmi_stream_t stream_) {
    hipStream_t stream = (hipStream_t)stream_;
    APEXMI_REQUIRE(count >= 1 && count <= MAX_GROUPS, "gemm_bf16_grouped: count=%d not in [1,%d]", count, MAX_GROUPS);
    GemmGroup G;
    G.count = count;
    G.K = K;
    G.batch = 1;
    G.bsA = G.bsW = G.bsC_bytes = 0;
    double flops = 0, bytes = 0;
    const int kind = epi_kind(epilogue[0]);
    for (int i = 0; i < count; ++i) {
        APEXMI_REQUIRE(epi_kind(epilogue[i]) == kind,
                       "gemm_bf16_grouped: gate/residual (or float / bf16 output) problems cannot be mixed with the others");
        const float* g = gate ? gate[i] : nullptr;
        const void* r = R ? R[i] : nullptr;
        const int64_t lr = ldr ? ldr[i] : 0;
        if (int rc = check_problem(A[i], lda[i], W[i], ldw[i], C[i], ldc[i], M[i], N[i], K, epilogue[i], g, r, lr))
            return rc;
        G.p[i] = GemmProblem{(const bf16_t*)A[i], (const bf16_t*)W[i], (const bf16_t*)(bias ? bias[i] : nullptr),
                             (bf16_t*)C[i], g, (const bf16_t*)r, lda[i], ldw[i], ldc[i], lr, M[i], N[i], 0, 0, 0,
                             act_mode(epi_base(epilogue[i]))};
        flops += 2.0 * M[i] * N[i] * (double)K;
        bytes += 2.0 * ((double)M[i] * K + (double)N[i] * K + (double)M[i] * N[i]);
    }
    ApexmiProfScope prof(0, stream, flops, bytes);
    return launch_group(G, M, kind, stream);
}

extern "C" int apexmi_gemm_uses_x288(int M, int N, int K) {
    GemmGroup G;
    memset(&G, 0, sizeof(G));
    G.count = 1;
    G.K = K;
    G.batch = 1;
    G.p[0].N = N;
    return (M > 0 && N > 0 && K > 0 && use_x288(G, &M)) ? 1 : 0;
}

extern "C" int apexmi_gemm_qkv_fusable(int64_t m_total, int n_max, int K) {
    return (g_force_cfg == 0 || g_force_cfg == 7 || g_force_cfg == 9 || g_force_cfg == 10) &&
           (g_large_cfg == 7 || g_large_cfg == 9 || g_large_cfg == 10) && m_total >= 1024 && n_max >= 1024 && K >= 256 && K % BK == 0;
}

extern "C" int apexmi_gemm_bf16_grouped_qkv(int count, const void* const* A, const int64_t* lda, const void* const* W,
                                            const int64_t* ldw, const void* const* bias, void* const* C, const int64_t* ldc,
                                            const int* M, const int* N, int K, const int* epilogue, const int* is_qkv,
                                            const void* const* norm_q, const void* const* norm_k, const int* row0, int H,
                                            float eps, const float* rope, void* q_out, void* k_out, void* vt_out, int S_out,
                                            int Skp, apexmi_stream_t stream_) {
    return apexmi_gemm_bf16_grouped_qkv_pairs(count, A, lda, W, ldw, bias, C, ldc, M, N, K, epilogue, is_qkv, norm_q, norm_k, row0, H,
                                              eps, rope, nullptr, q_out, k_out, vt_out, S_out, Skp, stream_);
}

extern "C" int apexmi_gemm_bf16_grouped_qkv_pairs(int count, const void* const* A, const int64_t* lda, const void* const* W,
                                                  const int64_t* ldw, const void* const* bias, void* const* C, const int64_t* ldc,
                                                  const int* M, const int* N, int K, const int* epilogue, const int* is_qkv,
                                                  const void* const* norm_q, const void* const* norm_k, const int* row0, int H,
                                                  float eps, const float* rope, const float* rope_pairs, void* q_out, void* k_out,
                                                  void* vt_out, int S_out, int Skp, apexmi_stream_t stream_) {
    hipStream_t stream = (hipStream_t)stream_;
    APEXMI_REQUIRE(((uintptr_t)rope_pairs % 16) == 0, "gemm_bf16_grouped_qkv: rope_pairs must be 16-byte aligned");
    APEXMI_REQUIRE(count >= 1 && count <= MAX_GROUPS, "gemm_bf16_grouped_qkv: count=%d not in [1,%d]", count, MAX_GROUPS);
    APEXMI_REQUIRE(is_qkv && row0 && rope && q_out && k_out && vt_out && H > 0, "gemm_bf16_grouped_qkv: null argument");
    APEXMI_REQUIRE(H % 2 == 0 && S_out > 0 && Skp >= S_out && Skp % 8 == 0, "gemm_bf16_grouped_qkv: H=%d must be even, Skp=%d a multiple of 8 >= S_out=%d",
                   H, Skp, S_out);
    APEXMI_REQUIRE(((uintptr_t)rope % 16) == 0 && ((uintptr_t)q_out % 16) == 0 && ((uintptr_t)k_out % 16) == 0 && ((uintptr_t)vt_out % 16) == 0,
                   "gemm_bf16_grouped_qkv: rope / outputs must be 16-byte aligned");
    GemmGroup G;
    G.count = count;
    G.K = K;
    G.batch = 1;
    G.bsA = G.bsW = G.bsC_bytes = 0;
    G.qs = QkvShared{(bf16_t*)q_out, (bf16_t*)k_out, (bf16_t*)vt_out, rope, S_out, Skp, H * 128, eps, rope_pairs};
    double flops = 0, bytes = 0;
    int64_t mtot = 0;
    int nmax = 0;
    for (int i = 0; i < count; ++i) {
        APEXMI_REQUIRE(epi_kind(epilogue[i]) == APEXMI_EPI_BIAS, "gemm_bf16_grouped_qkv: bias-class epilogues only (got %d)", epilogue[i]);
        void* c = is_qkv[i] ? q_out : C[i];
        const int64_t lc = is_qkv[i] ? 128 : ldc[i];
        if (int rc = check_problem(A[i], lda[i], W[i], ldw[i], c, lc, M[i], N[i], K, epilogue[i], nullptr, nullptr, 0)) return rc;
        G.p[i] = GemmProblem{(const bf16_t*)A[i], (const bf16_t*)W[i], (const bf16_t*)(bias ? bias[i] : nullptr), (bf16_t*)c,
                             nullptr, nullptr, lda[i], ldw[i], lc, 0, M[i], N[i], 0, 0, 0, act_mode(epi_base(epilogue[i]))};
        if (is_qkv[i]) {
            APEXMI_REQUIRE(N[i] == 3 * H * 128 && epi_base(epilogue[i]) == APEXMI_EPI_BIAS,
                           "gemm_bf16_grouped_qkv: a fused problem has N = 3 H 128 = %d (got %d) and the plain bias epilogue", 3 * H * 128, N[i]);
            APEXMI_REQUIRE(row0[i] >= 0 && row0[i] + M[i] <= S_out,
                           "gemm_bf16_grouped_qkv: rows [%d, %d) must lie inside S_out=%d", row0[i], row0[i] + M[i], S_out);
            const void* nq = norm_q ? norm_q[i] : nullptr;
            const void* nk = norm_k ? norm_k[i] : nullptr;
            APEXMI_REQUIRE(((uintptr_t)nq % 16) == 0 && ((uintptr_t)nk % 16) == 0, "gemm_bf16_grouped_qkv: norm weights must be 16-byte aligned");
            G.p[i].qkv = 1;
            G.p[i].row0 = row0[i];
            G.p[i].nq = (const bf16_t*)nq;
            G.p[i].nk = (const bf16_t*)nk;
        }
        mtot += M[i];
        nmax = N[i] > nmax ? N[i] : nmax;
        flops += 2.0 * M[i] * N[i] * (double)K;
        bytes += 2.0 * ((double)M[i] * K + (double)N[i] * K + (double)M[i] * N[i]);
    }
    APEXMI_REQUIRE(apexmi_gemm_qkv_fusable(mtot, nmax, K),
                   "gemm_bf16_grouped_qkv: needs the 256x256 v_mfma_f32_16x16x32 tiling (gemm.config / gemm.large = 7, >= 1024 rows)");
    ApexmiProfScope prof(0, stream, flops, bytes);
    bool ld_ok = true;
    for (int i = 0; i < count; ++i) ld_ok &= lda[i] <= (1 << 21) && ldw[i] <= (1 << 21);
    if (g_x384 && g_x384_qkv && ld_ok && g_large_cfg == 7 && (g_force_cfg == 0 || g_force_cfg == 7) && (g_x384 == 2 || x384_pays(G, M)))
        return launch_x384<APEXMI_EPI_BIAS>(G, M, stream);
    if (g_large_cfg == 9 || g_force_cfg == 9) return launch_cfg<CFG_256R, APEXMI_EPI_BIAS>(G, M, stream);
    if (g_large_cfg == 10 || g_force_cfg == 10) return launch_cfg<CFG_256R5, APEXMI_EPI_BIAS>(G, M, stream);
    return launch_cfg<CFG_256P16, APEXMI_EPI_BIAS>(G, M, stream);
}

extern "C" int apexmi_split_bf16x3(const float* x, int64_t ldx, int64_t M, int K, void* out, int64_t ldo,
                                   apexmi_stream_t stream_) {
    hipStream_t stream = (hipStream_t)stream_;
    APEXMI_REQUIRE(x && out && M > 0 && K > 0, "split_bf16x3: bad arguments");
    APEXMI_REQUIRE(K % 8 == 0 && ldx % 4 == 0 && ldo % 8 == 0 && ldo >= 3 * (int64_t)K && ((uintptr_t)x % 16) == 0 &&
                       ((uintptr_t)out % 16) == 0,
                   "split_bf16x3: K=%d must be a multiple of 8 and rows 16-byte aligned", K);
    const int64_t n = M * (K / 8);
    ApexmiProfScope prof(5, stream, 0.0, 10.0 * (double)M * K);
    hipLaunchKernelGGL(split_bf16x3_kernel, dim3((unsigned)((n + 255) / 256)), dim3(256), 0, stream, x, ldx, M, K,
                       (bf16_t*)out, ldo);
    return apexmi_check_launch("split_bf16x3");
}

int apexmi_set_gemm_key(const char* key, int value) {
    if (!strcmp(key, "gemm.tail")) g_tail_split = value;
    else if (!strcmp(key, "gemm.tail_max")) g_tail_max = value;
    else if (!strcmp(key, "gemm.group_m")) g_group_m = value > 0 ? value : GROUP_M;
    else if (!strcmp(key, "gemm.large")) g_large_cfg = value;
    else if (!strcmp(key, "gemm.config")) g_force_cfg = value;
    else if (!strcmp(key, "gemm.wpacked")) g_wpacked = value;
    else if (!strcmp(key, "gemm.x288")) g_x288 = value;
    else if (!strcmp(key, "gemm.small_max")) g_small_max = value;
    else if (!strcmp(key, "gemm.x384")) g_x384 = value;
    else if (!strcmp(key, "gemm.x384_dist")) g_x384_dist = value;
    else if (!strcmp(key, "gemm.x384_group_m")) g_x384_group_m = value > 0 ? value : 3;
    else if (!strcmp(key, "gemm.x384_qkv")) g_x384_qkv = value;
#if APEXMI_GEMM_TRACE
    else if (!strcmp(key, "gemm.trace_lo")) g_gemm_trace = (g_gemm_trace & ~(uintptr_t)0xffffffffu) | (uint32_t)value;
    else if (!strcmp(key, "gemm.trace_hi")) g_gemm_trace = (g_gemm_trace & (uintptr_t)0xffffffffu) | ((uintptr_t)(uint32_t)value << 32);
#endif
    else return 1;
    return 0;
}
```

### apex-studio_amd/lib.py

```python
from __future__ import annotations

import ctypes as C
import os

_PKG_DIR = os.path.dirname(os.path.abspath(__file__))
LIB_PATH = os.environ.get("APEX_MI355_LIB") or os.path.join(_PKG_DIR, "libapex_mi355.so")

_lib = None

c_i64p = C.POINTER(C.c_int64)
c_f32p = C.c_void_p
vp = C.c_void_p

SIGNATURES = {
    "apexmi_version": (C.c_int, []),
    "apexmi_last_error": (C.c_char_p, []),
    "apexmi_attn_workspace_bytes": (C.c_size_t, [C.c_int] * 6),
    "apexmi_attn_fwd": (C.c_int, [vp, vp, vp, vp, C.c_int, C.c_int, C.c_int, C.c_int, C.c_int,
                                  c_i64p, c_i64p, c_i64p, c_i64p, C.c_float, C.c_int, vp,
                                  C.c_size_t, vp]),
    "apexmi_attn_fwd_prepared": (C.c_int, [vp, vp, vp, vp, C.c_int, C.c_int, C.c_int, C.c_int,
                                           C.c_int, c_i64p, C.c_float, vp]),
    "apexmi_attn_prepared_workspace_bytes": (C.c_size_t, [C.c_int] * 4),
    "apexmi_attn_fwd_prepared_ws": (C.c_int, [vp, vp, vp, vp, C.c_int, C.c_int, C.c_int, C.c_int,
                                              C.c_int, c_i64p, C.c_float, vp, C.c_size_t, vp]),
    "apexmi_attn_w64_fallbacks": (C.c_int, [C.POINTER(C.c_uint64)]),
    "apexmi_attn_framecausal_workspace_bytes": (C.c_size_t, [C.c_int, C.c_int]),
    "apexmi_attn_fwd_framecausal": (C.c_int, [vp, vp, vp, vp, C.c_int, C.c_int, C.c_int, C.c_int, C.c_int,
                                              c_i64p, c_i64p, c_i64p, c_i64p, C.c_float, vp, C.c_size_t, vp]),
    "apexmi_attn_wide_workspace_bytes": (C.c_size_t, [C.c_int] * 4),
    "apexmi_attn_fwd_wide": (C.c_int, [vp, vp, vp, vp] + [C.c_int] * 5 + [c_i64p] * 4 + [C.c_float, C.c_int, C.c_int, vp, C.c_size_t, vp]),
    "apexmi_attn_wide_auto_splits": (C.c_int, [C.c_int] * 3),
    "apexmi_attn_wide_split_workspace_bytes": (C.c_size_t, [C.c_int] * 6),
    "apexmi_attn_fwd_wide_split": (C.c_int, [vp, vp, vp, vp] + [C.c_int] * 5 + [c_i64p] * 4 + [C.c_float, C.c_int, C.c_int, vp, c_i64p,
                                                                                            C.c_int, vp, C.c_size_t, vp]),
    "apexmi_attn_masked_workspace_bytes": (C.c_size_t, [C.c_int] * 6),
    "apexmi_attn_fwd_masked": (C.c_int, [vp, vp, vp, vp] + [C.c_int] * 6 + [c_i64p] * 4 + [vp, C.c_int, c_i64p, C.c_int,
                                                                                        C.c_float, C.c_int, vp, C.c_size_t, vp]),
    "apexmi_attn_fwd_masked_lse": (C.c_int, [vp, vp, vp, vp, vp] + [C.c_int] * 6 + [c_i64p] * 5 + [vp, C.c_int, c_i64p, C.c_int,
                                                                                                C.c_float, C.c_int, vp, C.c_size_t, vp]),
    "apexmi_attn_merge": (C.c_int, [C.c_int, C.POINTER(vp), C.POINTER(vp), vp, vp] + [C.c_int] * 4 + [c_i64p, c_i64p, C.c_int, vp]),
    "apexmi_attn_varlen_workspace_bytes": (C.c_size_t, [C.c_int] * 4),
    "apexmi_attn_fwd_varlen": (C.c_int, [vp] * 7 + [C.c_int] * 8 + [c_i64p] * 5 + [C.c_int, C.c_float, C.c_int, vp, C.c_size_t, vp]),
    "apexmi_attn_window_map_bytes": (C.c_size_t, [C.c_int, C.c_int]),
    "apexmi_attn_window_map": (C.c_int, [vp, vp] + [C.c_int] * 5 + [vp, C.c_size_t, vp]),
    "apexmi_attn_fwd_window": (C.c_int, [vp, vp, vp, vp] + [C.c_int] * 6 + [c_i64p] * 4 + [vp, vp, C.c_int, C.c_int, C.c_int, vp,
                                                                                        C.c_float, C.c_int, vp, C.c_size_t, vp]),
    "apexmi_attn_fwd_prepared_window": (C.c_int, [vp, vp, vp, vp] + [C.c_int] * 5 + [c_i64p, vp, vp, C.c_int, C.c_int, C.c_int, vp,
                                                                                     C.c_float, vp]),
    "apexmi_attn_fwd_prepared_band": (C.c_int, [vp, vp, vp, vp] + [C.c_int] * 5 + [c_i64p, vp, C.c_int, C.c_float, vp]),
    "apexmi_attn_band_workspace_bytes": (C.c_size_t, [C.c_int] * 4),
    "apexmi_attn_fwd_band": (C.c_int, [vp, vp, vp, vp] + [C.c_int] * 5 + [c_i64p] * 4 + [vp, C.c_int, C.c_float, C.c_int, vp,
                                                                                      C.c_size_t, vp]),
    "apexmi_attn_fwd_prepared_dual": (C.c_int, [vp, vp, vp, C.c_int, C.c_int, vp, vp, C.c_int, C.c_int, vp, C.c_int, C.c_int,
                                                C.c_int, c_i64p, C.c_float, vp]),
    "apexmi_gemm_bf16": (C.c_int, [vp, C.c_int64, vp, C.c_int64, vp, vp, C.c_int64, C.c_int, C.c_int,
                                   C.c_int, C.c_int, vp, vp, C.c_int64, vp]),
    "apexmi_gemm_bf16_grouped": (C.c_int, [C.c_int, C.POINTER(vp), c_i64p, C.POINTER(vp), c_i64p,
                                           C.POINTER(vp), C.POINTER(vp), c_i64p, C.POINTER(C.c_int),
                                           C.POINTER(C.c_int), C.c_int, C.POINTER(C.c_int), C.POINTER(vp),
                                           C.POINTER(vp), c_i64p, vp]),
    "apexmi_gemm_bf16_grouped_qkv": (C.c_int, [C.c_int, C.POINTER(vp), c_i64p, C.POINTER(vp), c_i64p, C.POINTER(vp),
                                               C.POINTER(vp), c_i64p, C.POINTER(C.c_int), C.POINTER(C.c_int), C.c_int,
                                               C.POINTER(C.c_int), C.POINTER(C.c_int), C.POINTER(vp), C.POINTER(vp),
                                               C.POINTER(C.c_int), C.c_int, C.c_float, vp, vp, vp, vp, C.c_int, C.c_int, vp]),
    "apexmi_gemm_bf16_grouped_qkv_pairs": (C.c_int, [C.c_int, C.POINTER(vp), c_i64p, C.POINTER(vp), c_i64p, C.POINTER(vp),
                                                     C.POINTER(vp), c_i64p, C.POINTER(C.c_int), C.POINTER(C.c_int), C.c_int,
                                                     C.POINTER(C.c_int), C.POINTER(C.c_int), C.POINTER(vp), C.POINTER(vp),
                                                     C.POINTER(C.c_int), C.c_int, C.c_float, vp, vp, vp, vp, vp, C.c_int, C.c_int, vp]),
    "apexmi_rope_pairs": (C.c_int, [vp, C.c_int, C.c_int, vp, vp, vp]),
    "apexmi_gemm_qkv_fusable": (C.c_int, [C.c_int64, C.c_int, C.c_int]),
    "apexmi_gemm_uses_x288": (C.c_int, [C.c_int, C.c_int, C.c_int]),
    "apexmi_qk_rms_rope_rows": (C.c_int, [vp, vp, vp, C.c_int64, C.c_int, C.c_int, vp, vp, C.c_float, vp, C.c_int, vp, vp, vp,
                                          C.c_int, C.c_int, C.c_int, vp]),
    "apexmi_qk_rms_rope_rows_f32": (C.c_int, [vp, vp, vp, C.c_int64, C.c_int, C.c_int, vp, vp, C.c_float, vp, C.c_int, vp, vp, vp,
                                              C.c_int, C.c_int, C.c_int, vp]),
    "apexmi_gemm_bf16_batched": (C.c_int, [vp, C.c_int64, C.c_int64, vp, C.c_int64, C.c_int64, vp, C.c_int64, C.c_int64,
                                           C.c_int, C.c_int, C.c_int, C.c_int, C.c_int, vp]),
    "apexmi_attn_bias_workspace_bytes": (C.c_size_t, [C.c_int] * 4),
    "apexmi_attn_fwd_bias": (C.c_int, [vp, C.c_int64, vp, C.c_int64, vp, C.c_int64, vp, C.c_int64, C.c_int, C.c_int,
                                       C.c_int, C.c_int, C.c_int, C.c_float, vp, vp, vp, C.c_int, vp, C.c_size_t, vp]),
    "apexmi_rope_half": (C.c_int, [vp, C.c_int64, C.c_int64, C.c_int, C.c_int, C.c_int, vp, vp, vp]),
    "apexmi_rope_half_f32": (C.c_int, [vp, C.c_int64, C.c_int64, C.c_int, C.c_int, C.c_int, vp, vp, vp]),
    "apexmi_tune_set": (C.c_int, [C.c_char_p, C.c_int]),
    "apexmi_gemv": (C.c_int, [vp, C.c_int64, vp, vp, C.c_int64, vp, C.c_int64, C.c_int, C.c_int,
                              C.c_int, C.c_int, vp]),
    "apexmi_ln_modulate": (C.c_int, [vp, C.c_int64, vp, C.c_int64, C.c_int, C.c_int, vp, vp, vp, vp,
                                     C.c_float, C.c_int, vp]),
    "apexmi_ln_modulate2": (C.c_int, [vp, C.c_int64, vp, C.c_int64, C.c_int, C.c_int, vp, vp, vp, vp,
                                      C.c_float, C.c_int, C.c_int, vp, vp, vp]),
    "apexmi_qkv_prepare": (C.c_int, [vp, vp, vp, C.c_int64, C.c_int, C.c_int, C.c_int, C.c_int, vp, vp,
                                     vp, vp, C.c_float, vp, C.c_int, vp, vp, vp, C.c_int, C.c_int,
                                     C.c_int, vp]),
    "apexmi_v_transpose": (C.c_int, [vp, C.c_int64, C.c_int64, C.c_int, C.c_int, C.c_int, vp, C.c_int,
                                     C.c_int, vp]),
    "apexmi_conv3d_cl": (C.c_int, [vp, vp, vp, vp, vp, vp] + [C.c_int] * 9 + [vp]),
    "apexmi_conv3d_cl_replicate": (C.c_int, [vp, vp, vp, vp, vp, vp] + [C.c_int] * 9 + [vp]),
    "apexmi_conv3d_cl_clips": (C.c_int, [vp, vp, vp, vp, vp, vp] + [C.c_int] * 11 + [vp]),
    "apexmi_conv3d_cl_strided": (C.c_int, [vp, vp, vp, vp, vp, vp] + [C.c_int] * 15 + [vp]),
    "apexmi_conv3d_cl_frames": (C.c_int, [vp, vp, vp, vp, vp, vp] + [C.c_int] * 9 + [vp]),
    "apexmi_conv3d_cl_up2": (C.c_int, [vp, vp, vp, vp, vp, vp] + [C.c_int] * 10 + [vp]),
    "apexmi_conv3d_cl_norm_fusable": (C.c_int, [C.c_int] * 6),
    "apexmi_conv3d_cl_family": (C.c_int, [C.c_int] * 23 + [vp]),
    "apexmi_conv3d_cl_norm": (C.c_int, [vp, vp, vp, vp, vp, vp, vp, C.c_int, vp] + [C.c_int] * 11 + [vp]),
    "apexmi_add_bf16": (C.c_int, [vp, vp, vp, C.c_int64, vp]),
    "apexmi_add_f32": (C.c_int, [vp, vp, vp, C.c_int64, vp]),
    "apexmi_group_mean_bf16": (C.c_int, [vp, vp, C.c_int64, C.c_int, C.c_int, vp]),
    "apexmi_group_mean_f32": (C.c_int, [vp, vp, C.c_int64, C.c_int, C.c_int, vp]),
    "apexmi_rmsnorm_cl": (C.c_int, [vp, vp, vp, C.c_int64, C.c_int, C.c_int, vp]),
    "apexmi_upsample2x_cl": (C.c_int, [vp, vp, C.c_int, C.c_int, C.c_int, C.c_int, vp]),
    "apexmi_time_interleave_cl": (C.c_int, [vp, vp, C.c_int, C.c_int64, C.c_int, vp]),
    "apexmi_conv3d_cl_act": (C.c_int, [vp, vp, vp, vp, vp, vp] + [C.c_int] * 12 + [C.c_float, vp]),
    "apexmi_conv3d_cl_tstrided": (C.c_int, [vp, vp, vp, vp, vp, vp] + [C.c_int] * 12 + [vp]),
    "apexmi_tanh_clamp": (C.c_int, [vp, vp, C.c_int64, C.c_float, vp]),
    "apexmi_pixel_shuffle_clamp": (C.c_int, [vp, vp] + [C.c_int] * 7 + [C.c_float, C.c_float, vp]),
    "apexmi_tanh_clamp_f32": (C.c_int, [vp, vp, C.c_int64, C.c_float, vp]),
    "apexmi_pixel_shuffle_clamp_f32": (C.c_int, [vp, vp] + [C.c_int] * 7 + [C.c_float, C.c_float, vp]),
    "apexmi_groupnorm_workspace_bytes": (C.c_size_t, [C.c_int64, C.c_int]),
    "apexmi_groupnorm_cl": (C.c_int, [vp, vp, vp, vp, C.c_int64, C.c_int, C.c_int, C.c_float, C.c_int, vp,
                                      C.c_size_t, vp]),
    "apexmi_crossfade": (C.c_int, [vp, vp, C.c_int64, C.c_int, C.c_int64, C.c_int64, C.c_int64, C.c_int64,
                                   C.c_int64, vp]),
    "apexmi_timestep_embedding": (C.c_int, [vp, vp, C.c_int, C.c_int, C.c_float, C.c_int, C.c_float,
                                            vp, vp]),
    "apexmi_rope_table_axes": (C.c_int, [vp, C.c_int, C.c_int, C.POINTER(C.c_int), C.c_float, vp, vp]),
    "apexmi_add_bcast_f32": (C.c_int, [vp, vp, vp, C.c_int64, C.c_int64, vp]),
    "apexmi_add_rowvec_bf16": (C.c_int, [vp, C.c_int64, vp, vp, C.c_int64, C.c_int64, C.c_int, vp]),
    "apexmi_add_rowvec_f32": (C.c_int, [vp, C.c_int64, vp, vp, C.c_int64, C.c_int64, C.c_int, vp]),
    "apexmi_frames_to_u8": (C.c_int, [vp, C.c_int64, C.c_int64, C.c_int64, C.c_int64, C.c_int, C.c_int, C.c_int, C.c_int,
                                      vp, vp]),
    "apexmi_mul_bf16": (C.c_int, [vp, vp, vp, C.c_int64, vp]),
    "apexmi_mul_f32": (C.c_int, [vp, vp, vp, C.c_int64, vp]),
    "apexmi_gather_rows_f32": (C.c_int, [vp, C.c_int64, C.c_int64, vp, vp, C.c_int64, C.c_int, vp, C.c_int64,
                                         C.c_int64, C.c_int, vp]),
    "apexmi_attn_fwd_bias_f32": (C.c_int, [vp, C.c_int64, vp, C.c_int64, vp, C.c_int64, vp, C.c_int64, C.c_int, C.c_int,
                                           C.c_int, C.c_int, C.c_int, C.c_float, vp, vp, vp, C.c_int, vp]),
    "apexmi_gather_rows_bf16": (C.c_int, [vp, C.c_int64, C.c_int64, vp, vp, C.c_int64, C.c_int, vp, C.c_int64,
                                          C.c_int64, C.c_int, vp]),
    "apexmi_relpos_bias": (C.c_int, [vp, C.c_int, C.c_int, vp, C.c_int, C.c_int, vp, vp]),
    "apexmi_cast_f32_to_bf16": (C.c_int, [vp, vp, C.c_int64, vp]),
    "apexmi_cast_bf16_to_f32": (C.c_int, [vp, vp, C.c_int64, vp]),
    "apexmi_dequant_fp8_scaled": (C.c_int, [vp, C.c_int, vp, C.c_int64, C.c_int64, C.c_int64, vp, C.c_int64, vp]),
    "apexmi_quant_rows_fp8": (C.c_int, [vp, C.c_int64, C.c_int, C.c_int, vp, C.c_int64, vp, vp]),
    "apexmi_ln_modulate_quant_fp8": (C.c_int, [vp, C.c_int64, C.c_int, vp, C.c_int64, vp, C.c_int64, vp, C.c_int, C.c_int, vp, vp, vp,
                                               vp, C.c_float, C.c_int, C.c_int, vp, vp, vp]),
    "apexmi_gemm_fp8": (C.c_int, [vp, C.c_int64, vp, vp, C.c_int64, C.c_int, vp, C.c_int64, vp, vp, C.c_int64, C.c_int, C.c_int,
                                  C.c_int, C.c_int, vp, vp, C.c_int64, vp]),
    "apexmi_gemm_fp8_lora": (C.c_int, [vp, C.c_int64, vp, vp, C.c_int64, C.c_int, vp, C.c_int64, vp, vp, C.c_int64, C.c_int, C.c_int,
                                       C.c_int, C.c_int, vp, vp, C.c_int64, vp, C.c_int64, vp, C.c_int64, C.c_int, vp]),
    "apexmi_gemm_fp8_grouped": (C.c_int, [C.c_int, C.POINTER(vp), c_i64p, C.POINTER(vp), C.POINTER(vp), c_i64p, C.POINTER(C.c_int),
                                          C.POINTER(vp), c_i64p, C.POINTER(vp), C.POINTER(vp), c_i64p, C.POINTER(C.c_int),
                                          C.POINTER(C.c_int), C.c_int, C.POINTER(C.c_int), C.POINTER(vp), C.POINTER(vp), c_i64p, vp]),
    "apexmi_gemm_fp8_grouped_qkv": (C.c_int, [C.c_int, C.POINTER(vp), c_i64p, C.POINTER(vp), C.POINTER(vp), c_i64p, C.POINTER(C.c_int),
                                              C.POINTER(vp), c_i64p, C.POINTER(vp), C.POINTER(vp), c_i64p, C.POINTER(C.c_int),
                                              C.POINTER(C.c_int), C.c_int, C.POINTER(C.c_int), C.POINTER(vp), C.POINTER(vp), c_i64p,
                                              C.POINTER(C.c_int), C.POINTER(vp), C.POINTER(vp), C.POINTER(C.c_int), C.c_int, C.c_float,
                                              vp, vp, vp, vp, C.c_int, C.c_int, vp]),
    "apexmi_gemm_fp8_grouped_lora": (C.c_int, [C.c_int, C.POINTER(vp), c_i64p, C.POINTER(vp), C.POINTER(vp), c_i64p, C.POINTER(C.c_int),
                                               C.POINTER(vp), c_i64p, C.POINTER(vp), C.POINTER(vp), c_i64p, C.POINTER(C.c_int),
                                               C.POINTER(C.c_int), C.c_int, C.POINTER(C.c_int), C.POINTER(vp), C.POINTER(vp), c_i64p,
                                               C.POINTER(vp), c_i64p, C.POINTER(vp), c_i64p, C.POINTER(C.c_int), vp]),
    "apexmi_gemm_fp8_grouped_qkv_lora": (C.c_int, [C.c_int, C.POINTER(vp), c_i64p, C.POINTER(vp), C.POINTER(vp), c_i64p,
                                                   C.POINTER(C.c_int), C.POINTER(vp), c_i64p, C.POINTER(vp), C.POINTER(vp), c_i64p,
                                                   C.POINTER(C.c_int), C.POINTER(C.c_int), C.c_int, C.POINTER(C.c_int), C.POINTER(vp),
                                                   C.POINTER(vp), c_i64p, C.POINTER(C.c_int), C.POINTER(vp), C.POINTER(vp),
                                                   C.POINTER(C.c_int), C.c_int, C.c_float, vp, vp, vp, vp, C.c_int, C.c_int,
                                                   C.POINTER(vp), c_i64p, C.POINTER(vp), c_i64p, C.POINTER(C.c_int), vp]),
    "apexmi_quant_blocks_mxfp8": (C.c_int, [vp, C.c_int64, C.c_int, C.c_int, vp, C.c_int64, vp, C.c_int64, vp]),
    "apexmi_gemm_fp8_mx": (C.c_int, [vp, C.c_int64, vp, vp, C.c_int64, vp, C.c_int64, C.c_int, vp, C.c_int64, vp, vp, C.c_int64, vp,
                                     C.c_int64, vp, C.c_int64, C.c_int, C.c_int, C.c_int, C.c_int, vp, vp, C.c_int64, vp]),
    "apexmi_gemm_fp8_grouped_mx": (C.c_int, [C.c_int, C.POINTER(vp), c_i64p, C.POINTER(vp), C.POINTER(vp), c_i64p, C.POINTER(C.c_int),
                                             C.POINTER(vp), c_i64p, C.POINTER(vp), C.POINTER(vp), c_i64p, C.POINTER(C.c_int),
                                             C.POINTER(C.c_int), C.c_int, C.POINTER(C.c_int), C.POINTER(vp), C.POINTER(vp), c_i64p,
                                             C.POINTER(vp), c_i64p, C.POINTER(vp), c_i64p, C.POINTER(vp), c_i64p, vp]),
    "apexmi_quant_blocks_mxfp4": (C.c_int, [vp, C.c_int64, C.c_int, C.c_int, vp, C.c_int64, vp, C.c_int64, vp]),
    "apexmi_gemm_mxfp4": (C.c_int, [vp, C.c_int64, vp, C.c_int64, vp, C.c_int64, vp, C.c_int64, vp, vp, C.c_int64, C.c_int, C.c_int,
                                    C.c_int, C.c_int, vp, vp, C.c_int64, vp]),
    "apexmi_gemm_mxfp4_grouped": (C.c_int, [C.c_int, C.POINTER(vp), c_i64p, C.POINTER(vp), c_i64p, C.POINTER(vp), c_i64p, C.POINTER(vp),
                                            c_i64p, C.POINTER(vp), C.POINTER(vp), c_i64p, C.POINTER(C.c_int), C.POINTER(C.c_int), C.c_int,
                                            C.POINTER(C.c_int), C.POINTER(vp), C.POINTER(vp), c_i64p, vp]),
    "apexmi_gemm_mxfp4_grouped_qkv": (C.c_int, [C.c_int, C.POINTER(vp), c_i64p, C.POINTER(vp), c_i64p, C.POINTER(vp), c_i64p,
                                                C.POINTER(vp), c_i64p, C.POINTER(vp), C.POINTER(vp), c_i64p, C.POINTER(C.c_int),
                                                C.POINTER(C.c_int), C.c_int, C.POINTER(C.c_int), C.POINTER(vp), C.POINTER(vp), c_i64p,
                                                C.POINTER(C.c_int), C.POINTER(vp), C.POINTER(vp), C.POINTER(C.c_int), C.c_int, C.c_float,
                                                vp, vp, vp, vp, C.c_int, C.c_int, vp]),
    "apexmi_ln_modulate_quant_mxfp4": (C.c_int, [vp, C.c_int64, C.c_int, vp, C.c_int64, vp, C.c_int64, vp, C.c_int64, C.c_int, C.c_int, vp,
                                                 vp, vp, vp, C.c_float, C.c_int, C.c_int, vp, vp, vp]),
    "apexmi_gemm_mxfp4_mx": (C.c_int, [vp, C.c_int64, vp, C.c_int64, vp, C.c_int64, vp, C.c_int64, vp, vp, C.c_int64, vp, C.c_int64, vp,
                                       C.c_int64, C.c_int, C.c_int, C.c_int, C.c_int, vp, vp, C.c_int64, vp]),
    "apexmi_gemm_mxfp4_grouped_mx": (C.c_int, [C.c_int, C.POINTER(vp), c_i64p, C.POINTER(vp), c_i64p, C.POINTER(vp), c_i64p, C.POINTER(vp),
                                               c_i64p, C.POINTER(vp), C.POINTER(vp), c_i64p, C.POINTER(vp), c_i64p, C.POINTER(vp), c_i64p,
                                               C.POINTER(C.c_int), C.POINTER(C.c_int), C.c_int, C.POINTER(C.c_int), C.POINTER(vp),
                                               C.POINTER(vp), c_i64p, vp]),
    "apexmi_gemm_mxfp4_grouped_qkv_mx": (C.c_int, [C.c_int, C.POINTER(vp), c_i64p, C.POINTER(vp), c_i64p, C.POINTER(vp), c_i64p,
                                                   C.POINTER(vp), c_i64p, C.POINTER(vp), C.POINTER(vp), c_i64p, C.POINTER(vp), c_i64p,
                                                   C.POINTER(vp), c_i64p, C.POINTER(C.c_int), C.POINTER(C.c_int), C.c_int,
                                                   C.POINTER(C.c_int), C.POINTER(vp), C.POINTER(vp), c_i64p, C.POINTER(C.c_int),
                                                   C.POINTER(vp), C.POINTER(vp), C.POINTER(C.c_int), C.c_int, C.c_float, vp, vp, vp, vp,
                                                   C.c_int, C.c_int, vp]),
    "apexmi_quant_blocks_mxfp6": (C.c_int, [vp, C.c_int64, C.c_int, C.c_int, vp, C.c_int64, vp, C.c_int64, vp]),
    "apexmi_gemm_mxfp6": (C.c_int, [vp, C.c_int64, vp, C.c_int64, vp, C.c_int64, vp, C.c_int64, vp, vp, C.c_int64, C.c_int, C.c_int,
                                    C.c_int, C.c_int, vp, vp, C.c_int64, vp]),
    "apexmi_dequant_gguf": (C.c_int, [vp, C.c_int, C.c_int64, C.c_int64, vp, C.c_int64, vp]),
    "apexmi_euler_step": (C.c_int, [vp, vp, vp, C.c_int64, C.c_float, C.c_int, vp]),
    "apexmi_prof_enable": (C.c_int, [C.c_int]),
    "apexmi_prof_read": (C.c_int, [C.POINTER(C.c_double), C.POINTER(C.c_int64), C.POINTER(C.c_double),
                                   C.POINTER(C.c_double)]),
    "apexmi_prof_reset": (C.c_int, []),
    "apexmi_clk_enable": (C.c_int, [C.c_int]),
    "apexmi_clk_read": (C.c_int, [C.POINTER(C.c_uint64), C.POINTER(C.c_uint64)]),
}

for _name in ("apexmi_ln_modulate2", "apexmi_qkv_prepare", "apexmi_rmsnorm_cl", "apexmi_groupnorm_cl",
              "apexmi_time_interleave_cl", "apexmi_crossfade", "apexmi_frames_to_u8"):
    SIGNATURES[_name + "_f32"] = SIGNATURES[_name]
SIGNATURES["apexmi_ln_modulate_f32in"] = SIGNATURES["apexmi_ln_modulate"]
SIGNATURES["apexmi_ln_modulate2_f32in"] = SIGNATURES["apexmi_ln_modulate2"]
SIGNATURES["apexmi_attn_fwd_prepared_f32"] = SIGNATURES["apexmi_attn_fwd_prepared"]
SIGNATURES["apexmi_split_bf16x3"] = (C.c_int, [vp, C.c_int64, C.c_int64, C.c_int, vp, C.c_int64, vp])
SIGNATURES["apexmi_conv3d_cl_f32"] = (C.c_int, [vp, vp, vp, vp, vp, vp] + [C.c_int] * 20 + [C.c_float, vp])

NCLASS = 6
PROF_CLASSES = ("gemm", "attention", "gemv", "ln_modulate", "qkv_prepare", "other")

BF16, F16, F32 = 0, 1, 2
MASK_BOOL = 3
EPI_BIAS, EPI_BIAS_GELU, EPI_BIAS_GATE_RES, EPI_BIAS_F32, EPI_BIAS_GELU_ERF, EPI_BIAS_SILU, EPI_BIAS_QUICK_GELU = 0, 1, 2, 3, 4, 5, 6
EPI_F32_IO = 0x100
GEMV_PRE_SILU, GEMV_POST_SILU, GEMV_POST_GELU, GEMV_ACCUM = 1, 2, 4, 8
ROPE_INTERLEAVED, ROPE_COMPLEX, ROPE_NONE = 0, 1, 2


class ApexMIError(RuntimeError):
    pass


def load():
    global _lib
    if _lib is not None:
        return _lib
    if not os.path.exists(LIB_PATH):
        raise ApexMIError(
            f"{LIB_PATH} is missing: the HIP extension has not been built "
            "(run `python __graft_entry__.py` or apex_studio_amd.build.build()). "
            "There is no CPU fallback for the product path."
        )
    import torch
    if torch.cuda.is_available():
        torch.cuda.init()
    lib = C.CDLL(LIB_PATH)
    for name, (res, args) in SIGNATURES.items():
        fn = getattr(lib, name)
        fn.restype = res
        fn.argtypes = args
    _lib = lib
    return lib


def check(rc: int, what: str = "") -> None:
    if rc != 0:
        msg = load().apexmi_last_error().decode("utf-8", "replace")
        raise ApexMIError(f"{what or 'apexmi'} failed (rc={rc}): {msg}")


def i64x2(vals):
    return (C.c_int64 * 2)(*[int(v) for v in vals])


def i64x3(vals):
    return (C.c_int64 * 3)(*[int(v) for v in vals])


def i64x4(vals):
    return (C.c_int64 * 4)(*[int(v) for v in vals])


def tune_set(key: str, value: int) -> None:
    check(load().apexmi_tune_set(key.encode(), int(value)), "tune_set")


def attn_w64_fallbacks() -> int:
    n = C.c_uint64(0)
    check(load().apexmi_attn_w64_fallbacks(C.byref(n)), "attn_w64_fallbacks")
    return int(n.value)


def prof_enable(on: bool) -> None:
    check(load().apexmi_prof_enable(1 if on else 0))


def clk_enable(on: bool) -> None:
    check(load().apexmi_clk_enable(1 if on else 0), "clk_enable")


def clk_read() -> dict:
    c, r = C.c_uint64(0), C.c_uint64(0)
    check(load().apexmi_clk_read(C.byref(c), C.byref(r)), "clk_read")
    return {"cycles": int(c.value), "ref_ticks": int(r.value), "ghz": (0.1 * c.value / r.value) if r.value else None}


def prof_reset() -> None:
    check(load().apexmi_prof_reset())


def prof_read() -> dict:
    ms = (C.c_double * NCLASS)()
    n = (C.c_int64 * NCLASS)()
    fl = (C.c_double * NCLASS)()
    by = (C.c_double * NCLASS)()
    check(load().apexmi_prof_read(ms, n, fl, by), "prof_read")
    return {
        PROF_CLASSES[i]: {"ms": ms[i], "launches": int(n[i]), "flops": fl[i], "bytes": by[i]}
        for i in range(NCLASS)
    }
```

### include/apexmi.h

```cpp
#ifndef APEXMI_H
#define APEXMI_H

#include <stdint.h>
#include <stddef.h>

#ifdef __cplusplus
extern "C" {
#endif

typedef void* apexmi_stream_t;

#define APEXMI_BF16 0
#define APEXMI_F16 1
#define APEXMI_F32 2
#define APEXMI_MASK_BOOL 3

#define APEXMI_EPI_BIAS 0
#define APEXMI_EPI_BIAS_GELU 1
#define APEXMI_EPI_BIAS_GATE_RES 2
#define APEXMI_EPI_BIAS_GELU_ERF 4
#define APEXMI_EPI_BIAS_QUICK_GELU 6
#define APEXMI_EPI_BIAS_SILU 5
#define APEXMI_EPI_BIAS_F32 3

#define APEXMI_EPI_F32_IO 0x100

#define APEXMI_GEMV_PRE_SILU 1
#define APEXMI_GEMV_POST_SILU 2
#define APEXMI_GEMV_POST_GELU 4
#define APEXMI_GEMV_ACCUM 8

#define APEXMI_ROPE_INTERLEAVED 0
#define APEXMI_ROPE_COMPLEX 1
#define APEXMI_ROPE_NONE 2

int apexmi_version(void);
const char* apexmi_last_error(void);

size_t apexmi_attn_workspace_bytes(int B, int H, int Sq, int Sk, int D, int dtype);
int apexmi_attn_fwd(const void* q, const void* k, const void* v, void* out,
                    int B, int H, int Sq, int Sk, int D,
                    const int64_t q_strides[3], const int64_t k_strides[3],
                    const int64_t v_strides[3], const int64_t o_strides[3],
                    float softmax_scale, int dtype,
                    void* workspace, size_t workspace_bytes, apexmi_stream_t stream);

int apexmi_attn_fwd_prepared(const void* q, const void* k, const void* vt, void* out,
                             int B, int H, int Sq, int Sk, int Skp,
                             const int64_t o_strides[3], float softmax_scale,
                             apexmi_stream_t stream);

size_t apexmi_attn_prepared_workspace_bytes(int B, int H, int Sq, int Sk);
int apexmi_attn_fwd_prepared_ws(const void* q, const void* k, const void* vt, void* out, int B, int H, int Sq, int Sk,
                                int Skp, const int64_t o_strides[3], float softmax_scale, void* workspace,
                                size_t workspace_bytes, apexmi_stream_t stream);

int apexmi_attn_w64_fallbacks(uint64_t* count);

size_t apexmi_attn_framecausal_workspace_bytes(int S, int D);
int apexmi_attn_fwd_framecausal(const void* q, const void* k, const void* v, void* out, int B, int H, int S, int D,
                                int block, const int64_t q_strides[3], const int64_t k_strides[3],
                                const int64_t v_strides[3], const int64_t o_strides[3], float softmax_scale,
                                void* workspace, size_t workspace_bytes, apexmi_stream_t stream);

size_t apexmi_attn_wide_workspace_bytes(int B, int H, int Sk, int D);
int apexmi_attn_fwd_wide(const void* q, const void* k, const void* v, void* out, int B, int H, int Sq, int Sk, int D,
                         const int64_t q_strides[3], const int64_t k_strides[3], const int64_t v_strides[3],
                         const int64_t o_strides[3], float softmax_scale, int dtype, int frame_tokens, void* workspace,
                         size_t workspace_bytes, apexmi_stream_t stream);

int apexmi_attn_wide_auto_splits(int units, int key_tiles, int cus);
size_t apexmi_attn_wide_split_workspace_bytes(int B, int H, int Sq, int Sk, int D, int key_splits);
int apexmi_attn_fwd_wide_split(const void* q, const void* k, const void* v, void* out, int B, int H, int Sq, int Sk, int D,
                               const int64_t q_strides[3], const int64_t k_strides[3], const int64_t v_strides[3],
                               const int64_t o_strides[3], float softmax_scale, int dtype, int frame_tokens, float* lse,
                               const int64_t lse_strides[3], int key_splits, void* workspace, size_t workspace_bytes,
                               apexmi_stream_t stream);

size_t apexmi_attn_masked_workspace_bytes(int B, int Hq, int Hkv, int Sq, int Sk, int D);
int apexmi_attn_fwd_masked(const void* q, const void* k, const void* v, void* out, int B, int Hq, int Hkv, int Sq, int Sk,
                           int D, const int64_t q_strides[3], const int64_t k_strides[3], const int64_t v_strides[3],
                           const int64_t o_strides[3], const void* mask, int mask_dtype, const int64_t mask_strides[4],
                           int is_causal, float softmax_scale, int dtype, void* workspace, size_t workspace_bytes,
                           apexmi_stream_t stream);

int apexmi_attn_fwd_masked_lse(const void* q, const void* k, const void* v, void* out, float* lse, int B, int Hq, int Hkv, int Sq,
                               int Sk, int D, const int64_t q_strides[3], const int64_t k_strides[3],
                               const int64_t v_strides[3], const int64_t o_strides[3], const int64_t lse_strides[3],
                               const void* mask, int mask_dtype, const int64_t mask_strides[4], int is_causal,
                               float softmax_scale, int dtype, void* workspace, size_t workspace_bytes, apexmi_stream_t stream);

int apexmi_attn_merge(int n, const void* const* outs, const float* const* lses, void* out, float* lse_out, int B, int H, int Sq,
                      int D, const int64_t o_strides[3], const int64_t lse_strides[3], int dtype, apexmi_stream_t stream);

size_t apexmi_attn_varlen_workspace_bytes(int Tk, int n, int Hkv, int D);
int apexmi_attn_fwd_varlen(const void* q, const void* k, const void* v, void* out, float* lse, const int* cu_seqlens_q,
                           const int* cu_seqlens_k, int n, int Tq, int Tk, int Hq, int Hkv, int D, int max_seqlen_q,
                           int max_seqlen_k, const int64_t q_strides[2], const int64_t k_strides[2],
                           const int64_t v_strides[2], const int64_t o_strides[2], const int64_t lse_strides[2],
                           int is_causal, float softmax_scale, int dtype, void* workspace, size_t workspace_bytes,
                           apexmi_stream_t stream);

size_t apexmi_attn_window_map_bytes(int Sq, int Sk);
int apexmi_attn_window_map(const void* q_coords, const void* k_coords, int Sq, int Sk, int r0, int r1, int r2, void* map,
                           size_t map_bytes, apexmi_stream_t stream);
int apexmi_attn_fwd_window(const void* q, const void* k, const void* v, void* out, int B, int Hq, int Hkv, int Sq, int Sk,
                           int D, const int64_t q_strides[3], const int64_t k_strides[3], const int64_t v_strides[3],
                           const int64_t o_strides[3], const void* q_coords, const void* k_coords, int r0, int r1, int r2,
                           const void* map, float softmax_scale, int dtype, void* workspace, size_t workspace_bytes,
                           apexmi_stream_t stream);
int apexmi_attn_fwd_prepared_window(const void* q, const void* k, const void* vt, void* out, int B, int H, int Sq, int Sk,
                                    int Skp, const int64_t o_strides[3], const void* q_coords, const void* k_coords, int r0,
                                    int r1, int r2, const void* map, float softmax_scale, apexmi_stream_t stream);

int apexmi_attn_fwd_prepared_band(const void* q, const void* k, const void* vt, void* out, int B, int H, int Sq, int Sk,
                                  int Skp, const int64_t o_strides[3], const void* bands, int Hb, float softmax_scale,
                                  apexmi_stream_t stream);
size_t apexmi_attn_band_workspace_bytes(int B, int H, int Sq, int Sk);
int apexmi_attn_fwd_band(const void* q, const void* k, const void* v, void* out, int B, int H, int Sq, int Sk, int D,
                         const int64_t q_strides[3], const int64_t k_strides[3], const int64_t v_strides[3],
                         const int64_t o_strides[3], const void* bands, int Hb, float softmax_scale, int dtype,
                         void* workspace, size_t workspace_bytes, apexmi_stream_t stream);

int apexmi_attn_fwd_prepared_dual(const void* q, const void* k_t, const void* vt_t, int Sk_t, int Skp_t, const void* k_i,
                                  const void* vt_i, int Sk_i, int Skp_i, void* out, int B, int H, int Sq,
                                  const int64_t o_strides[3], float softmax_scale, apexmi_stream_t stream);

int apexmi_gemm_bf16(const void* A, int64_t lda, const void* W, int64_t ldw, const void* bias,
                     void* C, int64_t ldc, int M, int N, int K, int epilogue,
                     const float* gate, const void* R, int64_t ldr, apexmi_stream_t stream);

int apexmi_gemm_uses_x288(int M, int N, int K);

int apexmi_gemm_bf16_grouped(int count, const void* const* A, const int64_t* lda,
                             const void* const* W, const int64_t* ldw, const void* const* bias,
                             void* const* C, const int64_t* ldc, const int* M, const int* N, int K,
                             const int* epilogue, const float* const* gate, const void* const* R,
                             const int64_t* ldr, apexmi_stream_t stream);

int apexmi_gemm_qkv_fusable(int64_t m_total, int n_max, int K);
int apexmi_gemm_bf16_grouped_qkv(int count, const void* const* A, const int64_t* lda, const void* const* W,
                                 const int64_t* ldw, const void* const* bias, void* const* C, const int64_t* ldc,
                                 const int* M, const int* N, int K, const int* epilogue, const int* is_qkv,
                                 const void* const* norm_q, const void* const* norm_k, const int* row0, int H, float eps,
                                 const float* rope, void* q_out, void* k_out, void* vt_out, int S_out, int Skp,
                                 apexmi_stream_t stream);
int apexmi_gemm_bf16_grouped_qkv_pairs(int count, const void* const* A, const int64_t* lda, const void* const* W,
                                       const int64_t* ldw, const void* const* bias, void* const* C, const int64_t* ldc,
                                       const int* M, const int* N, int K, const int* epilogue, const int* is_qkv,
                                       const void* const* norm_q, const void* const* norm_k, const int* row0, int H, float eps,
                                       const float* rope, const float* rope_pairs, void* q_out, void* k_out, void* vt_out,
                                       int S_out, int Skp, apexmi_stream_t stream);
int apexmi_rope_pairs(const float* rope, int S, int D, float* pairs, int* mismatch, apexmi_stream_t stream);

int apexmi_split_bf16x3(const float* x, int64_t ldx, int64_t M, int K, void* out, int64_t ldo, apexmi_stream_t stream);

int apexmi_gemm_bf16_batched(const void* A, int64_t lda, int64_t stride_a, const void* W, int64_t ldw, int64_t stride_w,
                             void* C, int64_t ldc, int64_t stride_c, int batch, int M, int N, int K, int epilogue,
                             apexmi_stream_t stream);

size_t apexmi_attn_bias_workspace_bytes(int H, int Sq, int Sk, int D);
int apexmi_attn_fwd_bias(const void* q, int64_t ldq, const void* k, int64_t ldk, const void* v, int64_t ldv, void* out,
                         int64_t ldo, int H, int Hkv, int Sq, int Sk, int D, float softmax_scale, const float* bias,
                         const uint8_t* keep, const int* seg, int causal, void* workspace, size_t workspace_bytes,
                         apexmi_stream_t stream);

int apexmi_tune_set(const char* key, int value);

int apexmi_gemv(const void* W, int64_t ldw, const void* bias, const float* x, int64_t ldx,
                float* y, int64_t ldy, int M, int N, int K, int flags, apexmi_stream_t stream);

int apexmi_ln_modulate(const void* x, int64_t ldx, void* out, int64_t ldo, int M, int C,
                       const float* scale, const float* shift, const void* gamma,
                       const void* beta, float eps, int rms, apexmi_stream_t stream);

int apexmi_ln_modulate2(const void* x, int64_t ldx, void* out, int64_t ldo, int M, int C,
                        const float* scale, const float* shift, const void* gamma, const void* beta,
                        float eps, int rms, int split, const float* scale2, const float* shift2,
                        apexmi_stream_t stream);

int apexmi_ln_modulate_f32in(const float* x, int64_t ldx, void* out, int64_t ldo, int M, int C,
                             const float* scale, const float* shift, const void* gamma,
                             const void* beta, float eps, int rms, apexmi_stream_t stream);
int apexmi_ln_modulate2_f32in(const float* x, int64_t ldx, void* out, int64_t ldo, int M, int C,
                              const float* scale, const float* shift, const void* gamma, const void* beta,
                              float eps, int rms, int split, const float* scale2, const float* shift2,
                              apexmi_stream_t stream);

int apexmi_qk_rms_rope_rows(const void* q, const void* k, const void* v, int64_t ld_in, int S, int H, const void* wq, const void* wk,
                            float eps, const float* rope, int rope_mode, void* qo, void* ko, void* vt, int S_out, int Skp,
                            int row0, apexmi_stream_t stream);
int apexmi_qk_rms_rope_rows_f32(const void* q, const void* k, const void* v, int64_t ld_in, int S, int H, const void* wq,
                                const void* wk, float eps, const float* rope, int rope_mode, void* qo, void* ko, void* vt,
                                int S_out, int Skp, int row0, apexmi_stream_t stream);

int apexmi_qkv_prepare(const void* q, const void* k, const void* v, int64_t ld_in,
                       int S, int H, int D, int split,
                       const void* wq, const void* wk, const void* wq2, const void* wk2,
                       float eps, const float* rope, int rope_mode,
                       void* qo, void* ko, void* vt, int S_out, int Skp, int row0,
                       apexmi_stream_t stream);

int apexmi_v_transpose(const void* v, int64_t v_stride_h, int64_t v_stride_s, int S, int H, int D,
                       void* vt, int Skp, int row0, apexmi_stream_t stream);

int apexmi_conv3d_cl(const void* in, const void* w, const void* bias, const void* residual, void* out,
                     const void* zeros, int T, int H, int W, int Cin, int Cout, int Kpad, int kT, int kH,
                     int kW, apexmi_stream_t stream);
int apexmi_conv3d_cl_clips(const void* in, const void* w, const void* bias, const void* residual, void* out, const void* zeros,
                           int T, int H, int W, int Cin, int Cout, int Kpad, int kT, int kH, int kW, int replicate,
                           int clip_frames, apexmi_stream_t stream);

int apexmi_conv3d_cl_up2(const void* in, const void* w, const void* bias, const void* residual, void* out,
                         const void* zeros, int T, int H, int W, int Cin, int Cout, int Kpad, int kT, int kH, int kW,
                         int independent, apexmi_stream_t stream);

int apexmi_conv3d_cl_norm_fusable(int T, int H, int W, int Cin, int Cout, int up);
int apexmi_conv3d_cl_family(int T, int H, int W, int Cin, int Cout, int Kpad, int kT, int kH, int kW, int replicate,
                            int independent, int up, int norm, int clip_frames, int stride_h, int stride_w, int pad_top,
                            int pad_left, int Ho, int Wo, int stride_t, int t_first, int To, int* n_extent);
int apexmi_conv3d_cl_norm(const void* in, const void* w, const void* bias, const void* residual, void* out, void* out_norm,
                          const void* gamma, int silu, const void* zeros, int T, int H, int W, int Cin, int Cout, int Kpad,
                          int kT, int kH, int kW, int independent, int up, apexmi_stream_t stream);

int apexmi_conv3d_cl_act(const void* in, const void* w, const void* bias, const void* residual, void* out,
                         const void* zeros, int T, int H, int W, int Cin, int Cout, int Kpad, int kT, int kH, int kW,
                         int independent, int up, int act, float slope, apexmi_stream_t stream);
int apexmi_tanh_clamp(const void* x, void* y, int64_t n, float inv_scale, apexmi_stream_t stream);
int apexmi_pixel_shuffle_clamp(const void* x, void* y, int T, int H, int W, int Cs, int C, int r, int t0, float lo, float hi,
                               apexmi_stream_t stream);

int apexmi_conv3d_cl_frames(const void* in, const void* w, const void* bias, const void* residual, void* out,
                            const void* zeros, int N, int H, int W, int Cin, int Cout, int Kpad, int kT, int kH, int kW,
                            apexmi_stream_t stream);

int apexmi_conv3d_cl_strided(const void* in, const void* w, const void* bias, const void* residual, void* out,
                             const void* zeros, int T, int H, int W, int Cin, int Cout, int Kpad, int kT, int kH, int kW,
                             int stride_h, int stride_w, int pad_top, int pad_left, int Ho, int Wo,
                             apexmi_stream_t stream);

int apexmi_conv3d_cl_tstrided(const void* in, const void* w, const void* bias, const void* residual, void* out,
                              const void* zeros, int T, int H, int W, int Cin, int Cout, int Kpad, int kT, int kH, int kW,
                              int stride_t, int t_first, int To, apexmi_stream_t stream);

int apexmi_conv3d_cl_replicate(const void* in, const void* w, const void* bias, const void* residual, void* out,
                               const void* zeros, int T, int H, int W, int Cin, int Cout, int Kpad, int kT, int kH,
                               int kW, apexmi_stream_t stream);
int apexmi_rmsnorm_cl(const void* x, void* y, const void* gamma, int64_t P, int C, int silu,
                      apexmi_stream_t stream);
int apexmi_upsample2x_cl(const void* x, void* y, int T, int H, int W, int C, apexmi_stream_t stream);
int apexmi_time_interleave_cl(const void* x, void* y, int T, int64_t HW, int C, apexmi_stream_t stream);
size_t apexmi_groupnorm_workspace_bytes(int64_t P, int C);
int apexmi_groupnorm_cl(const void* x, void* y, const void* gamma, const void* beta, int64_t P, int C, int G,
                        float eps, int silu, void* workspace, size_t workspace_bytes, apexmi_stream_t stream);
int apexmi_crossfade(const void* a, void* b, int64_t outer, int E, int64_t inner, int64_t a_so, int64_t a_se,
                     int64_t b_so, int64_t b_se, apexmi_stream_t stream);

int apexmi_timestep_embedding(const float* t, float* out, int M, int dim, float scale,
                              int flip_sin_to_cos, float downscale_freq_shift, const float* freqs,
                              apexmi_stream_t stream);

int apexmi_rope_table_axes(const float* ids, int S, int n_axes, const int* axes_dim, float theta,
                           float* out, apexmi_stream_t stream);

int apexmi_add_bcast_f32(const float* a, const float* b, float* out, int64_t rows, int64_t n,
                         apexmi_stream_t stream);

int apexmi_add_rowvec_bf16(const void* x, int64_t ldx, const void* v, void* out, int64_t ldo, int64_t rows,
                           int cols, apexmi_stream_t stream);
int apexmi_add_rowvec_f32(const void* x, int64_t ldx, const void* v, void* out, int64_t ldo, int64_t rows,
                           int cols, apexmi_stream_t stream);

int apexmi_add_bf16(const void* a, const void* b, void* out, int64_t n, apexmi_stream_t stream);
int apexmi_add_f32(const void* a, const void* b, void* out, int64_t n, apexmi_stream_t stream);

int apexmi_group_mean_bf16(const void* x, void* out, int64_t P, int C, int gs, apexmi_stream_t stream);

int apexmi_frames_to_u8(const void* video, int64_t stride_c, int64_t stride_t, int64_t stride_h, int64_t stride_w,
                        int C, int T, int H, int W, void* out, apexmi_stream_t stream);

int apexmi_rope_half(void* x, int64_t ldx, int64_t rows, int heads, int head_stride, int D, const float* cos_table,
                     const float* sin_table, apexmi_stream_t stream);

int apexmi_mul_bf16(const void* a, const void* b, void* out, int64_t n, apexmi_stream_t stream);

int apexmi_gather_rows_bf16(const void* table, int64_t ldt, int64_t vocab, const int64_t* ids, const void* pos,
                            int64_t ldp, int period, void* out, int64_t ldo, int64_t rows, int C,
                            apexmi_stream_t stream);

int apexmi_relpos_bias(const void* weight, int num_buckets, int H, const int* bucket, int Sq, int Sk, float* out,
                       apexmi_stream_t stream);

int apexmi_cast_f32_to_bf16(const float* x, void* out, int64_t n, apexmi_stream_t stream);
int apexmi_cast_bf16_to_f32(const void* x, float* out, int64_t n, apexmi_stream_t stream);

int apexmi_dequant_fp8_scaled(const void* w, int format, const void* scale, int64_t scale_count, int64_t rows,
                              int64_t cols, void* out, int64_t ldo, apexmi_stream_t stream);

int apexmi_quant_rows_fp8(const void* a, int64_t lda, int M, int K, void* codes, int64_t ldq, float* scales,
                          apexmi_stream_t stream);

int apexmi_ln_modulate_quant_fp8(const void* x, int64_t ldx, int x_dtype, void* out, int64_t ldo, void* codes, int64_t ldq,
                                 float* scales, int M, int C, const float* scale, const float* shift, const void* gamma,
                                 const void* beta, float eps, int rms, int split, const float* scale2, const float* shift2,
                                 apexmi_stream_t stream);

int apexmi_gemm_fp8(const void* qa, int64_t lda, const float* sa, const void* qw, int64_t ldw, int w_format, const void* sw,
                    int64_t sw_count, const void* bias, void* C, int64_t ldc, int M, int N, int K, int epilogue,
                    const float* gate, const void* R, int64_t ldr, apexmi_stream_t stream);

int apexmi_gemm_fp8_lora(const void* qa, int64_t lda, const float* sa, const void* qw, int64_t ldw, int w_format, const void* sw,
                         int64_t sw_count, const void* bias, void* C, int64_t ldc, int M, int N, int K, int epilogue,
                         const float* gate, const void* R, int64_t ldr, const void* t, int64_t ldt, const void* lb, int64_t ldb,
                         int Rp, apexmi_stream_t stream);

int apexmi_gemm_fp8_grouped(int count, const void* const* qa, const int64_t* lda, const float* const* sa, const void* const* qw,
                            const int64_t* ldw, const int* w_format, const void* const* sw, const int64_t* sw_count,
                            const void* const* bias, void* const* C, const int64_t* ldc, const int* M, const int* N, int K,
                            const int* epilogue, const float* const* gate, const void* const* R, const int64_t* ldr,
                            apexmi_stream_t stream);

int apexmi_gemm_fp8_grouped_qkv(int count, const void* const* qa, const int64_t* lda, const float* const* sa,
                                const void* const* qw, const int64_t* ldw, const int* w_format, const void* const* sw,
                                const int64_t* sw_count, const void* const* bias, void* const* C, const int64_t* ldc, const int* M,
                                const int* N, int K, const int* epilogue, const float* const* gate, const void* const* R,
                                const int64_t* ldr, const int* is_qkv, const void* const* norm_q, const void* const* norm_k,
                                const int* row0, int H, float eps, const float* rope, void* q_out, void* k_out, void* vt_out,
                                int S_out, int Skp, apexmi_stream_t stream);

int apexmi_gemm_fp8_grouped_lora(int count, const void* const* qa, const int64_t* lda, const float* const* sa,
                                 const void* const* qw, const int64_t* ldw, const int* w_format, const void* const* sw,
                                 const int64_t* sw_count, const void* const* bias, void* const* C, const int64_t* ldc, const int* M,
                                 const int* N, int K, const int* epilogue, const float* const* gate, const void* const* R,
                                 const int64_t* ldr, const void* const* t, const int64_t* ldt, const void* const* lb,
                                 const int64_t* ldb, const int* Rp, apexmi_stream_t stream);

int apexmi_gemm_fp8_grouped_qkv_lora(int count, const void* const* qa, const int64_t* lda, const float* const* sa,
                                     const void* const* qw, const int64_t* ldw, const int* w_format, const void* const* sw,
                                     const int64_t* sw_count, const void* const* bias, void* const* C, const int64_t* ldc,
                                     const int* M, const int* N, int K, const int* epilogue, const float* const* gate,
                                     const void* const* R, const int64_t* ldr, const int* is_qkv, const void* const* norm_q,
                                     const void* const* norm_k, const int* row0, int H, float eps, const float* rope, void* q_out,
                                     void* k_out, void* vt_out, int S_out, int Skp, const void* const* t, const int64_t* ldt,
                                     const void* const* lb, const int64_t* ldb, const int* Rp, apexmi_stream_t stream);

int apexmi_quant_blocks_mxfp8(const void* a, int64_t lda, int M, int K, void* codes, int64_t ldq, void* block_scales, int64_t ldbs,
                              apexmi_stream_t stream);

int apexmi_gemm_fp8_mx(const void* qa, int64_t lda, const float* sa, const void* abs, int64_t ldabs, const void* qw, int64_t ldw,
                       int w_format, const void* sw, int64_t sw_count, const void* bias, void* C, int64_t ldc, void* mx_codes,
                       int64_t ldmc, void* mx_scales, int64_t ldms, int M, int N, int K, int epilogue, const float* gate,
                       const void* R, int64_t ldr, apexmi_stream_t stream);

int apexmi_gemm_fp8_grouped_mx(int count, const void* const* qa, const int64_t* lda, const float* const* sa, const void* const* qw,
                               const int64_t* ldw, const int* w_format, const void* const* sw, const int64_t* sw_count,
                               const void* const* bias, void* const* C, const int64_t* ldc, const int* M, const int* N, int K,
                               const int* epilogue, const float* const* gate, const void* const* R, const int64_t* ldr,
                               const void* const* abs, const int64_t* ldabs, void* const* mx_codes, const int64_t* ldmc,
                               void* const* mx_scales, const int64_t* ldms, apexmi_stream_t stream);

int apexmi_quant_blocks_mxfp4(const void* a, int64_t lda, int M, int K, void* codes, int64_t ldq, void* scales, int64_t lds,
                              apexmi_stream_t stream);

int apexmi_gemm_mxfp4(const void* qa, int64_t lda, const void* sa, int64_t ldsa, const void* qw, int64_t ldw, const void* sw,
                      int64_t ldsw, const void* bias, void* C, int64_t ldc, int M, int N, int K, int epilogue, const float* gate,
                      const void* R, int64_t ldr, apexmi_stream_t stream);

int apexmi_gemm_mxfp4_grouped(int count, const void* const* qa, const int64_t* lda, const void* const* sa, const int64_t* ldsa,
                              const void* const* qw, const int64_t* ldw, const void* const* sw, const int64_t* ldsw,
                              const void* const* bias, void* const* C, const int64_t* ldc, const int* M, const int* N, int K,
                              const int* epilogue, const float* const* gate, const void* const* R, const int64_t* ldr,
                              apexmi_stream_t stream);

int apexmi_gemm_mxfp4_grouped_qkv(int count, const void* const* qa, const int64_t* lda, const void* const* sa, const int64_t* ldsa,
                                  const void* const* qw, const int64_t* ldw, const void* const* sw, const int64_t* ldsw,
                                  const void* const* bias, void* const* C, const int64_t* ldc, const int* M, const int* N, int K,
                                  const int* epilogue, const float* const* gate, const void* const* R, const int64_t* ldr,
                                  const int* is_qkv, const void* const* norm_q, const void* const* norm_k, const int* row0, int H,
                                  float eps, const float* rope, void* q_out, void* k_out, void* vt_out, int S_out, int Skp,
                                  apexmi_stream_t stream);

int apexmi_ln_modulate_quant_mxfp4(const void* x, int64_t ldx, int x_dtype, void* out, int64_t ldo, void* codes, int64_t ldq,
                                   void* scales, int64_t lds, int M, int C, const float* scale, const float* shift,
                                   const void* gamma, const void* beta, float eps, int rms, int split, const float* scale2,
                                   const float* shift2, apexmi_stream_t stream);

int apexmi_gemm_mxfp4_mx(const void* qa, int64_t lda, const void* sa, int64_t ldsa, const void* qw, int64_t ldw, const void* sw,
                         int64_t ldsw, const void* bias, void* C, int64_t ldc, void* mx_codes, int64_t ldmc, void* mx_scales,
                         int64_t ldms, int M, int N, int K, int epilogue, const float* gate, const void* R, int64_t ldr,
                         apexmi_stream_t stream);

int apexmi_gemm_mxfp4_grouped_mx(int count, const void* const* qa, const int64_t* lda, const void* const* sa, const int64_t* ldsa,
                                 const void* const* qw, const int64_t* ldw, const void* const* sw, const int64_t* ldsw,
                                 const void* const* bias, void* const* C, const int64_t* ldc, void* const* mx_codes,
                                 const int64_t* ldmc, void* const* mx_scales, const int64_t* ldms, const int* M, const int* N, int K,
                                 const int* epilogue, const float* const* gate, const void* const* R, const int64_t* ldr,
                                 apexmi_stream_t stream);

int apexmi_gemm_mxfp4_grouped_qkv_mx(int count, const void* const* qa, const int64_t* lda, const void* const* sa, const int64_t* ldsa,
                                     const void* const* qw, const int64_t* ldw, const void* const* sw, const int64_t* ldsw,
                                     const void* const* bias, void* const* C, const int64_t* ldc, void* const* mx_codes,
                                     const int64_t* ldmc, void* const* mx_scales, const int64_t* ldms, const int* M, const int* N,
                                     int K, const int* epilogue, const float* const* gate, const void* const* R, const int64_t* ldr,
                                     const int* is_qkv, const void* const* norm_q, const void* const* norm_k, const int* row0, int H,
                                     float eps, const float* rope, void* q_out, void* k_out, void* vt_out, int S_out, int Skp,
                                     apexmi_stream_t stream);

int apexmi_quant_blocks_mxfp6(const void* a, int64_t lda, int M, int K, void* codes, int64_t ldq, void* scales, int64_t lds,
                              apexmi_stream_t stream);

int apexmi_gemm_mxfp6(const void* qa, int64_t lda, const void* sa, int64_t ldsa, const void* qw, int64_t ldw, const void* sw,
                      int64_t ldsw, const void* bias, void* C, int64_t ldc, int M, int N, int K, int epilogue, const float* gate,
                      const void* R, int64_t ldr, apexmi_stream_t stream);

int apexmi_dequant_gguf(const void* blocks, int ggml_type, int64_t rows, int64_t K, void* out, int64_t ldo,
                        apexmi_stream_t stream);

int apexmi_euler_step(const void* sample, const void* model_out, void* out, int64_t n,
                      float dt, int sample_dtype, apexmi_stream_t stream);

int apexmi_ln_modulate2_f32(const void* x, int64_t ldx, void* out, int64_t ldo, int M, int C, const float* scale,
                            const float* shift, const void* gamma, const void* beta, float eps, int rms, int split,
                            const float* scale2, const float* shift2, apexmi_stream_t stream);
int apexmi_qkv_prepare_f32(const void* q, const void* k, const void* v, int64_t ld_in, int S, int H, int D, int split,
                           const void* wq, const void* wk, const void* wq2, const void* wk2, float eps, const float* rope,
                           int rope_mode, void* qo, void* ko, void* vt, int S_out, int Skp, int row0,
                           apexmi_stream_t stream);
int apexmi_attn_fwd_prepared_f32(const void* q, const void* k, const void* vt, void* out, int B, int H, int Sq, int Sk,
                                 int Skp, const int64_t o_strides[3], float softmax_scale, apexmi_stream_t stream);
int apexmi_conv3d_cl_f32(const void* in, const void* w, const void* bias, const void* residual, void* out,
                         const void* zeros, int T, int H, int W, int Cin3, int Cout, int Kpad, int kT, int kH, int kW,
                         int flags, int stride_h, int stride_w, int pad_top, int pad_left, int Ho, int Wo, int stride_t,
                         int t_first, int To, int act, float slope, apexmi_stream_t stream);
int apexmi_rmsnorm_cl_f32(const void* x, void* y, const void* gamma, int64_t P, int C, int silu, apexmi_stream_t stream);
int apexmi_groupnorm_cl_f32(const void* x, void* y, const void* gamma, const void* beta, int64_t P, int C, int G, float eps,
                            int silu, void* workspace, size_t workspace_bytes, apexmi_stream_t stream);
int apexmi_time_interleave_cl_f32(const void* x, void* y, int T, int64_t HW, int C, apexmi_stream_t stream);
int apexmi_crossfade_f32(const void* a, void* b, int64_t outer, int E, int64_t inner, int64_t a_so, int64_t a_se,
                         int64_t b_so, int64_t b_se, apexmi_stream_t stream);
int apexmi_frames_to_u8_f32(const void* video, int64_t stride_c, int64_t stride_t, int64_t stride_h, int64_t stride_w,
                            int C, int T, int H, int W, void* out, apexmi_stream_t stream);
int apexmi_attn_fwd_bias_f32(const float* q, int64_t ldq, const float* k, int64_t ldk, const float* v, int64_t ldv, float* out,
                             int64_t ldo, int H, int Hkv, int Sq, int Sk, int D, float scale, const float* bias,
                             const uint8_t* keep, const int* seg, int causal, apexmi_stream_t stream);
int apexmi_mul_f32(const float* a, const float* b, float* out, int64_t n, apexmi_stream_t stream);
int apexmi_gather_rows_f32(const void* table, int64_t ldt, int64_t vocab, const int64_t* ids, const void* pos, int64_t ldp,
                           int period, float* out, int64_t ldo, int64_t rows, int C, apexmi_stream_t stream);
int apexmi_rope_half_f32(void* x, int64_t ldx, int64_t rows, int heads, int head_stride, int D, const float* cos_, const float* sin_,
                         apexmi_stream_t stream);
int apexmi_group_mean_f32(const void* x, void* out, int64_t P, int C, int gs, apexmi_stream_t stream);
int apexmi_tanh_clamp_f32(const void* x, void* y, int64_t n, float inv_scale, apexmi_stream_t stream);
int apexmi_pixel_shuffle_clamp_f32(const void* x, void* y, int T, int H, int W, int Cs, int C, int r, int t0, float lo, float hi,
                                   apexmi_stream_t stream);

#define APEXMI_NCLASS 6
int apexmi_prof_enable(int on);
int apexmi_prof_read(double ms[APEXMI_NCLASS], int64_t launches[APEXMI_NCLASS],
                     double flops[APEXMI_NCLASS], double bytes[APEXMI_NCLASS]);
int apexmi_prof_reset(void);

int apexmi_clk_enable(int on);
int apexmi_clk_read(uint64_t* cycles, uint64_t* ref_ticks);

#ifdef __cplusplus
}
#endif
#endif
```

Baseline: 16.28 steps/s.

## Add persistent multi-tile GEMM kernels with per-XCD ticket scheduling and prefetch

Adds persistent variants of the 256x256 and 384x256 bf16 GEMM kernels. Each one launches at most one workgroup per CU and pulls further tiles from per-XCD atomic ticket counters, with work stealing across XCDs once its own share runs out. The first K-stage of the next tile is staged into LDS during the current tile's epilogue, hiding per-tile prologue and launch-tail costs. The cost is atomic traffic, extra barriers, a global ticket slot table keyed by stream or graph capture, and tighter register pressure, which is now checked by the no-spill build check.

```diff
diff --git a/apex-studio_amd/build.py b/apex-studio_amd/build.py
--- a/apex-studio_amd/build.py
+++ b/apex-studio_amd/build.py
@@ -30,6 +30,7 @@
 NO_SPILL = {"attention.hip": ["attn_fwd_d128_w64_kernel", "attn_fwd_d128_w64r_kernel", "attn_fwd_d128_w64_band_kernel"],
             "attention_masked.hip": ["attn_masked_kernel", "attn_window_map_kernel"],
             "attention_varlen.hip": ["attn_varlen_kernel", "attn_varlen_vt_kernel"], "attention_dual.hip": ["attn_dual_kernel"], "attention_wide.hip": ["attn_wide_kernel"],
+            "gemm.hip": ["gemm_bf16_multi_kernel", "gemm_bf16_x384_multi_kernel"],
             "gemm_fp8.hip": ["gemm_fp8_kernel"], "gemm_mxfp4.hip": ["gemm_mxfp4_kernel"], "gemm_mxfp6.hip": ["gemm_mxfp6_kernel"],
             "elementwise.hip": ["ln_modulate_quant_kernel", "ln_modulate_wave_quant_kernel"]}
 REMARKS = "-Rpass-analysis=kernel-resource-usage"
diff --git a/apex-studio_amd/csrc/gemm.hip b/apex-studio_amd/csrc/gemm.hip
--- a/apex-studio_amd/csrc/gemm.hip
+++ b/apex-studio_amd/csrc/gemm.hip
@@ -1,7 +1,9 @@
 #include "common.h"
 
 #include <cstring>
+#include <mutex>
 #include <type_traits>
+#include <vector>
 
 namespace {
 
@@ -58,6 +60,7 @@
     unsigned long long* trace;
 #endif
     int wpacked;
+    unsigned* tickets;
 };
 
 template <int BM_, int BN_, int WM_, int WN_, int SCHED_>
@@ -620,8 +623,106 @@
 struct KRange {
     int kt0, kt1;
 };
-template <typename CFG, int EPI>
-__device__ __forceinline__ void gemm_tile(const GemmGroup& G, char* smem, int s, const KRange& kr) {
+
+struct XcdShare {
+    int base, cnt;
+};
+__host__ __device__ inline XcdShare xcd_share(int xcd, int total) {
+    const int q = total >> 3, r = total & 7;
+    return XcdShare{xcd < r ? xcd * (q + 1) : r * (q + 1) + (xcd - r) * q, q + (xcd < r ? 1 : 0)};
+}
+__host__ __device__ inline int ticket_tile(int total, int nwg, int xcd, unsigned v) {
+    const XcdShare sh = xcd_share(xcd, total);
+    const unsigned first = (unsigned)((nwg - xcd + 7) >> 3);
+    return v < (unsigned)sh.cnt - first ? sh.base + (int)(first + v) : -1;
+}
+template <typename L, typename F>
+__host__ __device__ inline int ticket_resolve(int total, int nwg, int xcd, unsigned v, L&& live, F&& fetch_add) {
+    int t = ticket_tile(total, nwg, xcd, v);
+    for (int j = 1; t < 0 && j < 8; ++j) {
+        const int x = (xcd + j) & 7;
+        if (live(x)) t = ticket_tile(total, nwg, x, fetch_add(x));
+    }
+    return t;
+}
+__device__ __forceinline__ const GemmGroup& multi_args() {
+    auto p = (const __attribute__((address_space(4))) GemmGroup*)__builtin_amdgcn_kernarg_segment_ptr();
+    asm volatile("" : "+s"(p));
+    return *(const GemmGroup*)p;
+}
+struct MultiTile {
+    int nxt;
+    unsigned tk;
+};
+__device__ __forceinline__ int multi_lane() {
+    int l;
+    asm volatile("v_mbcnt_lo_u32_b32 %0, -1, 0\n\tv_mbcnt_hi_u32_b32 %0, -1, %0" : "=v"(l));
+    return l;
+}
+__device__ __forceinline__ int multi_xcd() { return (int)(blockIdx.x & 7); }
+__device__ __forceinline__ int multi_nwg() { return (int)gridDim.x; }
+__device__ __forceinline__ unsigned ticket_add(unsigned* head) {
+    return __hip_atomic_fetch_add(head, 1u, __ATOMIC_RELAXED, __HIP_MEMORY_SCOPE_AGENT);
+}
+__device__ __forceinline__ void ticket_fetch(const GemmGroup& G, MultiTile& mt, int wave) {
+    if (wave == 0) {
+        const int l = multi_lane();
+        unsigned* const h = G.tickets + ((multi_xcd() + l) & 7);
+        if (l == 0) mt.tk = ticket_add(h);
+        else if (l < 8) mt.tk = __hip_atomic_load(h, __ATOMIC_RELAXED, __HIP_MEMORY_SCOPE_AGENT);
+    }
+}
+__device__ __forceinline__ int ticket_next(const GemmGroup& G, const MultiTile& mt, char* word, int wave) {
+    if (wave == 0) {
+        const int l = multi_lane();
+        const unsigned long long looks = __ballot(l < 8 && ticket_tile(G.total, multi_nwg(), (multi_xcd() + l) & 7, mt.tk) >= 0);
+        if (l == 0)
+            *(volatile int*)word = ticket_resolve(G.total, multi_nwg(), multi_xcd(), mt.tk,
+                                                  [&](int x) { return ((looks >> ((x - multi_xcd()) & 7)) & 1) != 0; },
+                                                  [&](int x) { return ticket_add(G.tickets + x); });
+    }
+    __syncthreads();
+    const int t = __builtin_amdgcn_readfirstlane(*(volatile int*)word);
+    __syncthreads();
+    return t;
+}
+__device__ __forceinline__ void ticket_leave(const GemmGroup& G, int wave) {
+    if (wave == 0 && multi_lane() == 0 && ticket_add(G.tickets + 8) == (unsigned)multi_nwg() - 1)
+        for (int i = 0; i < 9; ++i) (void)__hip_atomic_exchange(G.tickets + i, 0u, __ATOMIC_RELAXED, __HIP_MEMORY_SCOPE_AGENT);
+}
+__device__ __forceinline__ int problem_of(const GemmGroup& G, int s) {
+    int gi = 0;
+#pragma unroll
+    for (int i = 1; i < MAX_GROUPS; ++i)
+        if (i < G.count && s >= G.p[i].tile0) gi = i;
+    return gi;
+}
+__device__ __forceinline__ void multi_stage0_256(const GemmGroup& G, int s, uint32_t smem_lds, int wave) {
+    int lane = multi_lane();
+    asm volatile("" : "+v"(lane));
+    const GemmProblem& P = G.p[problem_of(G, s)];
+    const TileCoord tc = tile_coord(s - P.tile0, P.nm, P.nn, G.group_m);
+    const int m0 = tc.pm * 256, n0 = tc.pn * 256;
+    const int ma = min(m0, P.M - 1), na = min(n0, P.N - 1);
+    const char* const a_u = uniform_ptr((const char*)(P.A + (int64_t)ma * P.lda));
+    const char* const w_u = uniform_ptr((const char*)(P.W + (int64_t)na * P.ldw));
+    const uint32_t lda2 = (uint32_t)P.lda * 2, ldw2 = (uint32_t)P.ldw * 2;
+#pragma unroll
+    for (int reg = 0; reg < 2; ++reg)
+#pragma unroll
+        for (int j = 0; j < 2; ++j) {
+            const int q = j * 8 + wave;
+            const int ra0 = (q < 8 ? q * 8 : 128 + (q - 8) * 8) + reg * 64;
+            const int rw0 = (q >> 2) * 64 + reg * 32 + (q & 3) * 8;
+            const int ra = ra0 + (lane >> 3), rw = rw0 + (lane >> 3);
+            glds16_s(a_u, (uint32_t)(min(m0 + ra, P.M - 1) - ma) * lda2 + (((lane & 7) ^ ((ra >> 1) & 7)) * 16), smem_lds + ra0 * 128);
+            glds16_s(w_u, (uint32_t)(min(n0 + rw, P.N - 1) - na) * ldw2 + (((lane & 7) ^ ((rw >> 1) & 7)) * 16),
+                     smem_lds + 256 * BK * 2 + rw0 * 128);
+        }
+}
+
+template <typename CFG, int EPI, bool MULTI = false>
+__device__ __forceinline__ void gemm_tile(const GemmGroup& G, char* smem, int s, const KRange& kr, MultiTile* mt = nullptr) {
     constexpr int BM = CFG::BM, BN = CFG::BN, TM = CFG::TM, TN = CFG::TN;
 
 #if APEXMI_GEMM_TRACE
@@ -641,6 +742,11 @@
     for (int i = 1; i < MAX_GROUPS; ++i)
         if (i < G.count && s >= G.p[i].tile0) gi = i;
     GemmProblem P = G.p[gi];
+    if constexpr (MULTI) {
+        const GemmProblem& Ps = G.p[gi];
+        P = GemmProblem{};
+        P.A = Ps.A, P.W = Ps.W, P.lda = Ps.lda, P.ldw = Ps.ldw, P.M = Ps.M, P.N = Ps.N, P.nm = Ps.nm, P.nn = Ps.nn, P.tile0 = Ps.tile0;
+    }
     if (G.batch > 1) {
         const int64_t z = blockIdx.y;
         P.A += z * G.bsA;
@@ -968,6 +1074,7 @@
 #undef RING_DSR
 #undef RING_WAIT
     } else if constexpr (CFG::SCHED == 5) {
+        const int wpk = MULTI ? 0 : G.wpacked;
         const int l15 = lane & 15, g4 = lane >> 4;
         const int sw16 = (l15 >> 1) & 7;
         int a16[8], w16[4];
@@ -1012,20 +1119,20 @@
                 const int ra0 = (q < 8 ? q * 8 : 128 + (q - 8) * 8) + reg * 64;
                 const int rw0 = (q >> 2) * 64 + reg * 32 + (q & 3) * 8;
                 const int ra = ra0 + (lane >> 3), rw = rw0 + (lane >> 3);
-                ra_src[reg][j] = (G.wpacked & 2)
+                ra_src[reg][j] = (wpk & 2)
                     ? (const char*)(P.A + ((int64_t)pm * nkt_all * 256 + ra) * 64 + (((lane & 7) ^ ((ra >> 1) & 7)) * 8))
                     : (const char*)(P.A + (int64_t)min(m0 + ra, M - 1) * P.lda + (((lane & 7) ^ ((ra >> 1) & 7)) * 8));
-                rw_src[reg][j] = (G.wpacked & 1)
+                rw_src[reg][j] = (wpk & 1)
                     ? (const char*)(P.W + ((int64_t)pn * nkt_all * 256 + rw) * 64 + (((lane & 7) ^ ((rw >> 1) & 7)) * 8))
                     : (const char*)(P.W + (int64_t)min(n0 + rw, N - 1) * P.ldw + (((lane & 7) ^ ((rw >> 1) & 7)) * 8));
                 ra_row[reg][j] = ra0;
                 rw_row[reg][j] = rw0;
             }
-        const int64_t w_kstep = (G.wpacked & 1) ? 256 * 128 : BK * 2;
-        const int64_t a_kstep = (G.wpacked & 2) ? 256 * 128 : BK * 2;
-        const char* const a_base_u = uniform_ptr((G.wpacked & 2) ? (const char*)(P.A + (int64_t)pm * nkt_all * 256 * 64)
+        const int64_t w_kstep = (wpk & 1) ? 256 * 128 : BK * 2;
+        const int64_t a_kstep = (wpk & 2) ? 256 * 128 : BK * 2;
+        const char* const a_base_u = uniform_ptr((wpk & 2) ? (const char*)(P.A + (int64_t)pm * nkt_all * 256 * 64)
                                                                  : (const char*)(P.A + (int64_t)min(m0, M - 1) * P.lda));
-        const char* const w_base_u = uniform_ptr((G.wpacked & 1) ? (const char*)(P.W + (int64_t)pn * nkt_all * 256 * 64)
+        const char* const w_base_u = uniform_ptr((wpk & 1) ? (const char*)(P.W + (int64_t)pn * nkt_all * 256 * 64)
                                                                  : (const char*)(P.W + (int64_t)min(n0, N - 1) * P.ldw));
         uint32_t ra_off[2][2], rw_off[2][2];
 #pragma unroll
@@ -1048,10 +1155,12 @@
 #pragma unroll
             for (int j = 0; j < 2; ++j) glds16_s(gb, rw_off[reg][j], base + rw_row[reg][j] * 128);
         };
-        stage_a(0, 0, 0);
-        stage_w(0, 0, 0);
-        stage_w(0, 0, 1);
-        stage_a(0, 0, 1);
+        if constexpr (!MULTI) {
+            stage_a(0, 0, 0);
+            stage_w(0, 0, 0);
+            stage_w(0, 0, 1);
+            stage_a(0, 0, 1);
+        }
         VMCNT(0);
         PP_BAR();
         if (wm == 1) PP_BAR();
@@ -1084,6 +1193,14 @@
         for (int kt = 0; kt + 1 < nkt; ++kt) ktile(kt, std::true_type{});
         if (nkt > 0) ktile(nkt - 1, std::false_type{});
         if (wm == 0) PP_BAR();
+        if constexpr (MULTI) {
+            P = multi_args().p[gi];
+            if (mt->nxt >= 0 && !(EPI == APEXMI_EPI_BIAS && P.qkv)) {
+                const GemmGroup& Gn = multi_args();
+                multi_stage0_256(Gn, mt->nxt, smem_lds, wave);
+                ticket_fetch(Gn, *mt, wave);
+            }
+        }
     } else {
         static_assert(!CFG::PP || (TM == 4 && TN == 2), "ping-pong schedule is written for 128x64 wave tiles");
         bf16x8 af[2][4], wf[4];
@@ -1187,18 +1304,26 @@
         __builtin_amdgcn_sched_barrier(0);
     }
 #endif
-    if (G.clk != nullptr) {
+    const GemmGroup& Ge = MULTI ? multi_args() : G;
+    if (Ge.clk != nullptr) {
         const unsigned long long c1 = __builtin_readcyclecounter(), r1 = __builtin_amdgcn_s_memrealtime();
         if (tid == 0) {
-            atomicAdd(G.clk, c1 - clk_c0);
-            atomicAdd(G.clk + 1, r1 - clk_r0);
+            atomicAdd(Ge.clk, c1 - clk_c0);
+            atomicAdd(Ge.clk + 1, r1 - clk_r0);
         }
     }
 
     if constexpr (CFG::SCHED == 5 || CFG::SCHED >= 7) {
         if constexpr (EPI == APEXMI_EPI_BIAS) {
             if (P.qkv) {
-                qkv_epilogue16(acc16, P, G.qs, M, m0, n0, wave, wm, wn, lane, smem);
+                qkv_epilogue16(acc16, P, Ge.qs, M, m0, n0, wave, wm, wn, lane, smem);
+                if constexpr (MULTI) {
+                    if (mt->nxt >= 0) {
+                        __syncthreads();
+                        multi_stage0_256(Ge, mt->nxt, __builtin_amdgcn_readfirstlane((uint32_t)(uintptr_t)(__attribute__((address_space(3))) void*)smem), wave);
+                        ticket_fetch(Ge, *mt, wave);
+                    }
+                }
                 APEXMI_TRACE_END();
                 return;
             }
@@ -1247,6 +1372,27 @@
     const int nkt = G.K / BK;
     const KRange kr{0, nkt};
     gemm_tile<CFG, EPI>(G, smem, xcd_remap(blockIdx.x, G.total), kr);
+}
+
+template <typename CFG, int EPI>
+__global__ __launch_bounds__(CFG::NT, CFG::OCC) void gemm_bf16_multi_kernel(const GemmGroup G) {
+    static_assert(CFG::SCHED == 5, "the multi-tile form is written for the 256 x 256 ping-pong schedule on 16x16x32");
+    extern __shared__ __attribute__((aligned(16))) char smem[];
+    const int nkt = G.K / BK;
+    const KRange kr{0, nkt};
+    const int wave = __builtin_amdgcn_readfirstlane(threadIdx.x >> 6);
+    MultiTile mt{-1, 0u};
+    int cur = xcd_share(multi_xcd(), G.total).base + (int)(blockIdx.x >> 3);
+    multi_stage0_256(G, cur, __builtin_amdgcn_readfirstlane((uint32_t)(uintptr_t)(__attribute__((address_space(3))) void*)smem), wave);
+    ticket_fetch(G, mt, wave);
+    for (;;) {
+        const GemmGroup& Gt = multi_args();
+        mt.nxt = ticket_next(Gt, mt, smem + CFG::STAGE, wave);
+        gemm_tile<CFG, EPI, true>(Gt, smem, cur, kr, &mt);
+        if (mt.nxt < 0) break;
+        cur = mt.nxt;
+    }
+    ticket_leave(G, wave);
 }
 
 __global__ __launch_bounds__(256) void split_bf16x3_kernel(const float* __restrict__ x, int64_t ldx, int64_t M, int K,
@@ -1472,20 +1618,49 @@
 constexpr int YBM = 384, YBN = 256;
 constexpr int Y_A_BYTES = YBM * BK * 2, Y_W_BYTES = YBN * BK * 2, Y_STAGE = Y_A_BYTES + Y_W_BYTES, Y_LDS = 2 * Y_STAGE;
 
-template <int EPI, int DIST = 1, int QKV = 0>
-__global__ __launch_bounds__(512, 2) void gemm_bf16_x384_kernel(const GemmGroup G) {
-    extern __shared__ __attribute__((aligned(16))) char smem[];
-    const int tid = threadIdx.x;
+__device__ __forceinline__ int x384_piece_of(int j, int par, int widx) {
+    if (j < 4) return 2 * (4 * j + widx) + par;
+    const int e = 3 * widx + (j < 7 ? j - 4 : j - 7);
+    return (e < 6 ? 0 : 24) + (j < 7 ? 0 : 12) + 2 * (e % 6) + par;
+}
+__device__ __forceinline__ void multi_stage0_x384(const GemmGroup& G, int s, char* smem, int wave) {
+    int lane = multi_lane();
+    asm volatile("" : "+v"(lane));
+    const GemmProblem& P = G.p[problem_of(G, s)];
+    const TileCoord tc = tile_coord(s - P.tile0, P.nm, P.nn, G.group_m);
+    const int m0 = tc.pm * YBM, n0 = tc.pn * YBN;
+    const int rows_a = min(P.M - m0, YBM), rows_w = min(P.N - n0, YBN);
+    auto rsrc_a = __builtin_amdgcn_make_buffer_rsrc((void*)(P.A + (int64_t)m0 * P.lda), 0,
+                                                    (int)(((int64_t)(rows_a - 1) * P.lda + G.K) * 2), 0x00020000);
+    auto rsrc_w = __builtin_amdgcn_make_buffer_rsrc((void*)(P.W + (int64_t)n0 * P.ldw), 0,
+                                                    (int)(((int64_t)(rows_w - 1) * P.ldw + G.K) * 2), 0x00020000);
+    const int par = wave & 1, widx = wave >> 1;
+    const int sw_src = ((lane & 7) ^ (4 * par + (lane >> 4))) * 16;
+    const int voff_a = (lane >> 3) * (int)P.lda * 2 + sw_src;
+    const int voff_w = (lane >> 3) * (int)P.ldw * 2 + sw_src;
+#pragma unroll
+    for (int j = 0; j < 10; ++j) {
+        const int pc = x384_piece_of(j, par, widx);
+        char* dst = smem + (j < 4 ? Y_A_BYTES : 0) + pc * 1024;
+        if (j < 4)
+            __builtin_amdgcn_raw_ptr_buffer_load_lds(rsrc_w, (__attribute__((address_space(3))) void*)dst, 16, voff_w, pc * ((int)P.ldw * 16), 0, 0);
+        else
+            __builtin_amdgcn_raw_ptr_buffer_load_lds(rsrc_a, (__attribute__((address_space(3))) void*)dst, 16, voff_a, pc * ((int)P.lda * 16), 0, 0);
+    }
+}
+
+template <int EPI, int DIST, int QKV, bool MULTI = false>
+__device__ __forceinline__ void x384_tile(const GemmGroup& G, char* smem, int s, int tid, MultiTile* mt = nullptr) {
+    if constexpr (MULTI) asm volatile("" : "+v"(tid));
     const int lane = tid & 63;
     const int wave = __builtin_amdgcn_readfirstlane(tid >> 6);
     const int wm = wave >> 2, wn = wave & 3;
 
-    int s = xcd_remap(blockIdx.x, G.total);
     int gi = 0;
 #pragma unroll
     for (int i = 1; i < MAX_GROUPS; ++i)
         if (i < G.count && s >= G.p[i].tile0) gi = i;
-    const GemmProblem P = G.p[gi];
+    GemmProblem P = G.p[gi];
     s -= P.tile0;
     const int N = P.N, M = P.M;
     const TileCoord tc = tile_coord(s, P.nm, P.nn, G.group_m);
@@ -1570,8 +1745,10 @@
                 acc[nt][h * 6 + t] = __builtin_amdgcn_mfma_f32_16x16x32_bf16(wf[nt], af[t], acc[nt][h * 6 + t], 0, 0, 0);
         __builtin_amdgcn_s_setprio(0);
     };
-#pragma unroll
-    for (int j = 0; j < 10; ++j) stage(0, 0, j);
+    if constexpr (!MULTI) {
+#pragma unroll
+        for (int j = 0; j < 10; ++j) stage(0, 0, j);
+    }
     VMCNT(0);
     PP_BAR();
     if (wm == 1) PP_BAR();
@@ -1630,21 +1807,31 @@
     for (int kt = 0; kt + 1 < nkt; ++kt) ktile(kt, std::true_type{});
     if (nkt > 0) ktile(nkt - 1, std::false_type{});
     if (wm == 0) PP_BAR();
-
-    if (G.clk != nullptr) {
+    if constexpr (MULTI) {
+        static_assert(QKV == 0, "x384_tile: no multi-tile form of the fused q/k/v launch");
+        if (mt->nxt >= 0) {
+            const GemmGroup& Gn = multi_args();
+            multi_stage0_x384(Gn, mt->nxt, smem, wave);
+            ticket_fetch(Gn, *mt, wave);
+        }
+    }
+
+    const GemmGroup& Ge = MULTI ? multi_args() : G;
+    if (Ge.clk != nullptr) {
         const unsigned long long c1 = __builtin_readcyclecounter(), r1 = __builtin_amdgcn_s_memrealtime();
         if (tid == 0) {
-            atomicAdd(G.clk, c1 - clk_c0);
-            atomicAdd(G.clk + 1, r1 - clk_r0);
+            atomicAdd(Ge.clk, c1 - clk_c0);
+            atomicAdd(Ge.clk + 1, r1 - clk_r0);
         }
     }
 
 #if APEXMI_GEMM_TRACE
     if (G.trace != nullptr) y_t_loop = __builtin_amdgcn_s_memrealtime();
 #endif
+    if constexpr (MULTI) P = multi_args().p[gi];
     if constexpr (EPI == APEXMI_EPI_BIAS && QKV == 1) {
         if (P.qkv) {
-            qkv_epilogue16<12, 192>(acc, P, G.qs, M, m0, n0, wave, wm, wn, lane, smem);
+            qkv_epilogue16<12, 192>(acc, P, Ge.qs, M, m0, n0, wave, wm, wn, lane, smem);
             Y_TRACE_END(n0 / G.qs.inner);
             return;
         }
@@ -1677,6 +1864,30 @@
     Y_TRACE_END(3);
 }
 #undef Y_TRACE_END
+
+template <int EPI, int DIST = 1, int QKV = 0>
+__global__ __launch_bounds__(512, 2) void gemm_bf16_x384_kernel(const GemmGroup G) {
+    extern __shared__ __attribute__((aligned(16))) char smem[];
+    x384_tile<EPI, DIST, QKV>(G, smem, xcd_remap(blockIdx.x, G.total), threadIdx.x);
+}
+
+template <int EPI, int DIST = 1>
+__global__ __launch_bounds__(512, 2) void gemm_bf16_x384_multi_kernel(const GemmGroup G) {
+    extern __shared__ __attribute__((aligned(16))) char smem[];
+    const int wave = __builtin_amdgcn_readfirstlane(threadIdx.x >> 6);
+    MultiTile mt{-1, 0u};
+    int cur = xcd_share(multi_xcd(), G.total).base + (int)(blockIdx.x >> 3);
+    multi_stage0_x384(G, cur, smem, wave);
+    ticket_fetch(G, mt, wave);
+    for (;;) {
+        const GemmGroup& Gt = multi_args();
+        mt.nxt = ticket_next(Gt, mt, smem + Y_STAGE, wave);
+        x384_tile<EPI, DIST, 0, true>(Gt, smem, cur, wave * 64 + multi_lane(), &mt);
+        if (mt.nxt < 0) break;
+        cur = mt.nxt;
+    }
+    ticket_leave(G, wave);
+}
 
 int g_group_m = GROUP_M;
 #if APEXMI_GEMM_TRACE
@@ -1694,6 +1905,60 @@
 int g_small_max = 112;
 int g_tail_split = 2;
 
+int g_multi = 1;
+
+constexpr int MULTI_SLOTS = 2048, MULTI_STREAMS = 64, MULTI_SLOT_WORDS = 16;
+__device__ unsigned d_gemm_tickets[MULTI_SLOTS * MULTI_SLOT_WORDS];
+std::mutex g_multi_mu;
+hipStream_t g_multi_streams[MULTI_STREAMS];
+int g_multi_nstreams = 0, g_multi_graph_next = MULTI_STREAMS;
+unsigned* multi_slot(hipStream_t stream) {
+    int dev = 0;
+    if (hipGetDevice(&dev) != hipSuccess || dev < 0 || dev >= 64) return nullptr;
+    static unsigned* base[64] = {};
+    std::lock_guard<std::mutex> lk(g_multi_mu);
+    if (base[dev] == nullptr && hipGetSymbolAddress((void**)&base[dev], HIP_SYMBOL(d_gemm_tickets)) != hipSuccess) {
+        (void)hipGetLastError();
+        return nullptr;
+    }
+    hipStreamCaptureStatus cap = hipStreamCaptureStatusNone;
+    if (hipStreamIsCapturing(stream, &cap) != hipSuccess) {
+        (void)hipGetLastError();
+        return nullptr;
+    }
+    int slot = -1;
+    if (cap != hipStreamCaptureStatusNone) {
+        if (g_multi_graph_next < MULTI_SLOTS) slot = g_multi_graph_next++;
+    } else {
+        for (int i = 0; i < g_multi_nstreams && slot < 0; ++i)
+            if (g_multi_streams[i] == stream) slot = i;
+        if (slot < 0 && g_multi_nstreams < MULTI_STREAMS) {
+            slot = g_multi_nstreams;
+            g_multi_streams[g_multi_nstreams++] = stream;
+        }
+    }
+    return slot < 0 ? nullptr : base[dev] + (size_t)slot * MULTI_SLOT_WORDS;
+}
+int multi_cus() {
+    int dev = 0;
+    if (hipGetDevice(&dev) != hipSuccess || dev < 0 || dev >= 64) return 0;
+    static int cus[64] = {};
+    if (cus[dev] == 0 && hipDeviceGetAttribute(&cus[dev], hipDeviceAttributeMultiprocessorCount, dev) != hipSuccess) cus[dev] = 0;
+    return cus[dev];
+}
+constexpr int MULTI_MIN_ROUNDS_X384_BIAS = 12;
+inline bool multi_pays(int tiles, int cus, int min_rounds) { return min_rounds > 0 && tiles >= min_rounds * cus; }
+int multi_wgs(GemmGroup& G, int tiles, hipStream_t stream, int min_rounds) {
+    if (g_multi == 0 || G.batch != 1 || g_wpacked != 0) return 0;
+#if APEXMI_GEMM_TRACE
+    if (g_gemm_trace) return 0;
+#endif
+    const int cus = multi_cus();
+    if (cus <= 0 || !(g_multi == 2 || multi_pays(tiles, cus, min_rounds))) return 0;
+    G.tickets = multi_slot(stream);
+    return G.tickets == nullptr ? 0 : (tiles < cus ? tiles : cus);
+}
+
 int number_tiles(GemmGroup& G, const int* Ms, int BM, int BN) {
     int t = 0;
     for (int i = 0; i < G.count; ++i) {
@@ -1709,6 +1974,7 @@
     G.trace = (unsigned long long*)g_gemm_trace;
 #endif
     G.wpacked = 0;
+    G.tickets = nullptr;
     return t;
 }
 
@@ -1729,6 +1995,16 @@
     const int t = number_tiles(G, Ms, CFG::BM, CFG::BN);
     G.group_m = g_group_m;
     if (CFG::SCHED == 5) G.wpacked = g_wpacked;
+    if constexpr (CFG::SCHED == 5 && (EPI == APEXMI_EPI_BIAS || EPI == APEXMI_EPI_BIAS_GATE_RES)) {
+        if (const int wgs = multi_wgs(G, t, stream, 0)) {
+            static uint64_t attr_set_multi = 0;
+            APEXMI_SET_ATTR_ONCE(attr_set_multi,
+                (void)hipFuncSetAttribute((const void*)gemm_bf16_multi_kernel<CFG, EPI>,
+                                          hipFuncAttributeMaxDynamicSharedMemorySize, CFG::LDS));
+            hipLaunchKernelGGL((gemm_bf16_multi_kernel<CFG, EPI>), dim3(wgs, 1), dim3(CFG::NT), CFG::LDS, stream, G);
+            return apexmi_check_launch("gemm_bf16 (multi-tile)");
+        }
+    }
     hipLaunchKernelGGL((gemm_bf16_kernel<CFG, EPI>), dim3(t, G.batch), dim3(CFG::NT), CFG::LDS, stream, G);
     return apexmi_check_launch("gemm_bf16");
 }
@@ -1763,6 +2039,17 @@
         }
     }
     const int dist = g_x384_dist >= 0 ? g_x384_dist : (t >= 2048 ? 0 : 1);
+    if constexpr (EPI == APEXMI_EPI_BIAS || EPI == APEXMI_EPI_BIAS_GATE_RES) {
+        if (const int wgs = multi_wgs(G, t, stream, EPI == APEXMI_EPI_BIAS ? MULTI_MIN_ROUNDS_X384_BIAS : 0)) {
+            static uint64_t attr_set_multi = 0;
+            APEXMI_SET_ATTR_ONCE(attr_set_multi,
+                (void)hipFuncSetAttribute((const void*)gemm_bf16_x384_multi_kernel<EPI, 0>, hipFuncAttributeMaxDynamicSharedMemorySize, Y_LDS);
+                (void)hipFuncSetAttribute((const void*)gemm_bf16_x384_multi_kernel<EPI, 1>, hipFuncAttributeMaxDynamicSharedMemorySize, Y_LDS));
+            if (dist == 0) hipLaunchKernelGGL((gemm_bf16_x384_multi_kernel<EPI, 0>), dim3(wgs, 1), dim3(512), Y_LDS, stream, G);
+            else hipLaunchKernelGGL((gemm_bf16_x384_multi_kernel<EPI, 1>), dim3(wgs, 1), dim3(512), Y_LDS, stream, G);
+            return apexmi_check_launch("gemm_bf16 (384x256, multi-tile)");
+        }
+    }
     if (dist == 0) hipLaunchKernelGGL((gemm_bf16_x384_kernel<EPI, 0>), dim3(t, 1), dim3(512), Y_LDS, stream, G);
     else hipLaunchKernelGGL((gemm_bf16_x384_kernel<EPI, 1>), dim3(t, 1), dim3(512), Y_LDS, stream, G);
     return apexmi_check_launch("gemm_bf16 (384x256)");
@@ -1997,6 +2284,24 @@
     G.batch = 1;
     G.p[0].N = N;
     return (M > 0 && N > 0 && K > 0 && use_x288(G, &M)) ? 1 : 0;
+}
+
+extern "C" int apexmi_gemm_multi_order(int total, int nwg, const int* asker, int n, int* tile_out) {
+    APEXMI_REQUIRE(asker && tile_out && n >= 0 && nwg >= 1 && nwg <= total, "gemm_multi_order: needs 1 <= nwg <= total");
+    unsigned heads[8] = {};
+    std::vector<char> started(nwg, 0);
+    for (int i = 0; i < n; ++i) {
+        const int b = asker[i];
+        APEXMI_REQUIRE(b >= 0 && b < nwg, "gemm_multi_order: workgroup %d not in [0, %d)", b, nwg);
+        if (!started[b]) {
+            started[b] = 1;
+            tile_out[i] = xcd_share(b & 7, total).base + (b >> 3);
+        } else {
+            tile_out[i] = ticket_resolve(total, nwg, b & 7, heads[b & 7]++, [&](int x) { return ticket_tile(total, nwg, x, heads[x]) >= 0; },
+                                         [&](int x) { return heads[x]++; });
+        }
+    }
+    return 0;
 }
 
 extern "C" int apexmi_gemm_qkv_fusable(int64_t m_total, int n_max, int K) {
@@ -2101,6 +2406,7 @@
     else if (!strcmp(key, "gemm.x384_dist")) g_x384_dist = value;
     else if (!strcmp(key, "gemm.x384_group_m")) g_x384_group_m = value > 0 ? value : 3;
     else if (!strcmp(key, "gemm.x384_qkv")) g_x384_qkv = value;
+    else if (!strcmp(key, "gemm.multi")) g_multi = value;
 #if APEXMI_GEMM_TRACE
     else if (!strcmp(key, "gemm.trace_lo")) g_gemm_trace = (g_gemm_trace & ~(uintptr_t)0xffffffffu) | (uint32_t)value;
     else if (!strcmp(key, "gemm.trace_hi")) g_gemm_trace = (g_gemm_trace & (uintptr_t)0xffffffffu) | ((uintptr_t)(uint32_t)value << 32);
diff --git a/apex-studio_amd/lib.py b/apex-studio_amd/lib.py
--- a/apex-studio_amd/lib.py
+++ b/apex-studio_amd/lib.py
@@ -71,6 +71,7 @@
     "apexmi_rope_pairs": (C.c_int, [vp, C.c_int, C.c_int, vp, vp, vp]),
     "apexmi_gemm_qkv_fusable": (C.c_int, [C.c_int64, C.c_int, C.c_int]),
     "apexmi_gemm_uses_x288": (C.c_int, [C.c_int, C.c_int, C.c_int]),
+    "apexmi_gemm_multi_order": (C.c_int, [C.c_int, C.c_int, C.POINTER(C.c_int), C.c_int, C.POINTER(C.c_int)]),
     "apexmi_qk_rms_rope_rows": (C.c_int, [vp, vp, vp, C.c_int64, C.c_int, C.c_int, vp, vp, C.c_float, vp, C.c_int, vp, vp, vp,
                                           C.c_int, C.c_int, C.c_int, vp]),
     "apexmi_qk_rms_rope_rows_f32": (C.c_int, [vp, vp, vp, C.c_int64, C.c_int, C.c_int, vp, vp, C.c_float, vp, C.c_int, vp, vp, vp,
diff --git a/include/apexmi.h b/include/apexmi.h
--- a/include/apexmi.h
+++ b/include/apexmi.h
@@ -131,6 +131,8 @@
                      const float* gate, const void* R, int64_t ldr, apexmi_stream_t stream);
 
 int apexmi_gemm_uses_x288(int M, int N, int K);
+
+int apexmi_gemm_multi_order(int total, int nwg, const int* asker, int n, int* tile_out);
 
 int apexmi_gemm_bf16_grouped(int count, const void* const* A, const int64_t* lda,
                              const void* const* W, const int64_t* ldw, const void* const* bias,
```

New measurement: 16.28 steps/s. Within noise of the previous version (-0.0%).
